# Forrest-Z/my-lidar-graph-slam

Measured on AMD Instinct MI355X. Metric: scans/sec + p50 scan-match ms, 1081-beam vs 1000×1000@5cm grid, 1/2/4/8 GPU, higher is better.
Workload: dtype f64

## Files before the change

### include/lgs_hip.h

```cpp
#ifndef LGS_HIP_H
#define LGS_HIP_H

#include <stddef.h>
#include <stdint.h>

#ifdef __cplusplus
extern "C" {
#endif

#define LGS_ABI_VERSION 2

#define LGS_OK               0
#define LGS_ERR_INVALID_ARG  1
#define LGS_ERR_HIP          2
#define LGS_ERR_NO_DEVICE    3
#define LGS_ERR_OOM          4
#define LGS_ERR_INTERNAL     5

typedef struct lgs_ctx  lgs_ctx;
typedef struct lgs_grid lgs_grid;
typedef struct lgs_scan lgs_scan;

typedef struct { double x, y, theta; } lgs_pose2d;

typedef struct {
    const double* ranges;
    const double* angles;
    int n;
    lgs_pose2d rel_sensor_pose;
    double min_range, max_range;
} lgs_scan_host;

typedef struct {
    int low_resolution;
    double range_x, range_y, range_theta;
    double scan_range_max;
} lgs_rtcsm_params;

typedef struct {
    double usable_range_min, usable_range_max;
    double hit_and_missed_dist, occupancy_threshold;
    int kernel_size;
    double scaling_factor;
    double standard_deviation;
} lgs_cost_ge_params;

typedef struct {
    int pose_found;
    double normalized_cost;
    lgs_pose2d initial_pose;
    lgs_pose2d estimated_pose;
    double covariance[9];
    double score_max;
    double score_threshold;
    int best_win[3];
    int win[3];
    double steps[3];
    lgs_pose2d best_sensor_pose;
    int64_t coarse_blocks;
    int64_t fine_blocks;
    int guard_hits;
    int fixups;
    int slow_path;
} lgs_rtcsm_summary;

int  lgs_ctx_create(int device, lgs_ctx** out);
void lgs_ctx_destroy(lgs_ctx* ctx);
const char* lgs_ctx_last_error(const lgs_ctx* ctx);
int  lgs_ctx_synchronize(lgs_ctx* ctx);
void* lgs_ctx_stream(lgs_ctx* ctx);
int  lgs_abi_version(void);

#define LGS_OPT_GUARD_EPS     1
#define LGS_OPT_FORCE_DENSE   2
#define LGS_OPT_INJECT_INDEX  3
#define LGS_OPT_GUARD_CAP     4
#define LGS_OPT_PROFILE       5
#define LGS_OPT_PROFILE_MASK  7
#define LGS_OPT_SPIN_SYNC     8
#define LGS_OPT_SKIP_MASK     10
#define LGS_OPT_SUPER_PRUNE   9
#define LGS_OPT_RAY_CHUNK_KEYS 13
#define LGS_OPT_LANES_MIN_BATCH 11
#define LGS_OPT_LINSOLVE_SPLIT 17
#define LGS_OPT_HANDOFF_SPIN_US 18
#define LGS_OPT_PEER_COPY     19
#define LGS_OPT_PRUNE_MIN_SUPER 21
#define LGS_OPT_COOP_TILES    22
#define LGS_OPT_SORT_BARRIER_US 23
#define LGS_OPT_FINE_STAGED   24
#define LGS_OPT_SMALL_WINDOW  25
#define LGS_OPT_POST_RECORDS  26
#define LGS_OPT_FUSED_PLANES  27
#define LGS_OPT_PRIORITY_TAIL 28
#define LGS_OPT_HV_FULL       29
#define LGS_OPT_SPLIT_CHUNKS  30
#define LGS_OPT_DEVICE_HITS   31
#define LGS_OPT_SEED_WIDE     32
#define LGS_OPT_ZERO_TILES    33
#define LGS_OPT_DEVICE_TIMING 34
#define LGS_OPT_LEAN_PROJECT  35
#define LGS_OPT_PGCG_GRID_NODES 36
#define LGS_OPT_FAST_ROWS     37
#define LGS_OPT_POISON_WS     15
int  lgs_ctx_set_option(lgs_ctx* ctx, int option, double value);

int  lgs_debug_item_buffer(lgs_ctx* ctx, int item, int which, void* out, size_t cap, size_t* bytes);

int  lgs_debug_libm(lgs_ctx* ctx, int op, const double* x, int n, double* out);

int  lgs_debug_keysort(lgs_ctx* ctx, const unsigned* keys, unsigned* out, long long n, int lo, int bits);

int  lgs_debug_copy_counters(const lgs_ctx* ctx, long long* direct, long long* staged);

int  lgs_debug_offset_checks(lgs_ctx* ctx, int reset, unsigned long long* out);

typedef struct {
    char name[32];
    int64_t launches;
    double total_ms;
    double algo_bytes;
    double dispatch_ms;
} lgs_kernel_stat;
int  lgs_ctx_kernel_stats(lgs_ctx* ctx, lgs_kernel_stat* out, int cap);
int  lgs_ctx_reset_stats(lgs_ctx* ctx);
int  lgs_ctx_match_counters(lgs_ctx* ctx, int64_t* out4);

int  lgs_grid_create(lgs_ctx* ctx, int w, int h, double min_x, double min_y,
                     double resolution, lgs_grid** out);
int  lgs_grid_wrap(lgs_ctx* ctx, double* device_cells, int w, int h, double min_x,
                   double min_y, double resolution, lgs_grid** out);
void lgs_grid_destroy(lgs_grid* grid);
int  lgs_grid_upload(lgs_ctx* ctx, lgs_grid* grid, const double* host_cells);
int  lgs_grid_upload_patches(lgs_ctx* ctx, lgs_grid* grid, const void* const* patches, int npx, int npy,
                             int patch_size, int cell_bytes, int value_offset);
int  lgs_grid_download(lgs_ctx* ctx, const lgs_grid* grid, double* host_cells);
int  lgs_grid_fill(lgs_ctx* ctx, lgs_grid* grid, double value);
int  lgs_grid_info(const lgs_grid* grid, int* w, int* h, double* min_x, double* min_y,
                   double* resolution);
double* lgs_grid_device_ptr(lgs_grid* grid);

int  lgs_grid_precompute_max(lgs_ctx* ctx, const lgs_grid* in, int win, lgs_grid* out);

int  lgs_scan_create(lgs_ctx* ctx, const lgs_scan_host* host, lgs_scan** out);
void lgs_scan_destroy(lgs_scan* scan);
int  lgs_scan_get(const lgs_scan* scan, int* n, double* ranges, double* angles);
int  lgs_scan_interpolate(lgs_ctx* ctx, const lgs_scan* in, double dist_scans, double dist_threshold_empty,
                          lgs_scan** out);

int  lgs_rtcsm_optimize_pose(lgs_ctx* ctx, const lgs_grid* grid, const lgs_grid* coarse,
                             const lgs_rtcsm_params* params,
                             const lgs_cost_ge_params* cost,
                             const lgs_scan* scan, lgs_pose2d initial_pose,
                             double normalized_score_threshold,
                             lgs_rtcsm_summary* out);
int  lgs_rtcsm_optimize_pose_query(lgs_ctx* ctx, const lgs_grid* grid,
                                   const lgs_rtcsm_params* params,
                                   const lgs_cost_ge_params* cost,
                                   const lgs_scan* scan, lgs_pose2d initial_pose,
                                   lgs_rtcsm_summary* out);
int  lgs_rtcsm_optimize_pose_query_batch(lgs_ctx* ctx, const lgs_grid* const* grids,
                                         const lgs_rtcsm_params* params,
                                         const lgs_cost_ge_params* cost,
                                         const lgs_scan* const* scans,
                                         const lgs_pose2d* initial_poses, int n,
                                         lgs_rtcsm_summary* out);
int  lgs_rtcsm_optimize_pose_batch(lgs_ctx* ctx, const lgs_grid* grid, const lgs_grid* coarse,
                                   const lgs_rtcsm_params* params,
                                   const lgs_cost_ge_params* cost,
                                   const lgs_scan* const* scans, const lgs_pose2d* initial_poses,
                                   int n, double normalized_score_threshold,
                                   lgs_rtcsm_summary* out);
int  lgs_rtcsm_dense_scores(lgs_ctx* ctx, const lgs_grid* grid, const lgs_grid* coarse,
                            const lgs_rtcsm_params* params, const lgs_scan* scan,
                            lgs_pose2d initial_pose, double* coarse_scores,
                            double* fine_scores, int* dims);

typedef struct lgs_map lgs_map;

typedef struct {
    double usable_range_min, usable_range_max;
    double prob_hit, prob_miss;
} lgs_builder_params;

typedef struct {
    double resolution;
    int patch_size;
    int num_patches_x, num_patches_y;
    int num_cells_x, num_cells_y;
    double min_x, min_y;
} lgs_map_geometry;

int  lgs_map_create(lgs_ctx* ctx, double resolution, int patch_size, int num_cells_x,
                    int num_cells_y, double center_x, double center_y, lgs_map** out);
void lgs_map_destroy(lgs_map* map);
int  lgs_map_get_geometry(const lgs_map* map, lgs_map_geometry* out);
int  lgs_map_grid(lgs_map* map, lgs_grid** out);
int  lgs_map_update_scan(lgs_ctx* ctx, lgs_map* map, const lgs_scan* scan, lgs_pose2d robot_pose,
                         const lgs_builder_params* params);
int  lgs_map_construct_from_scans(lgs_ctx* ctx, lgs_map* map, const lgs_scan* const* scans,
                                  const lgs_pose2d* robot_poses, int n,
                                  const lgs_builder_params* params);
int  lgs_map_append_scan(lgs_ctx* ctx, lgs_map* local, lgs_map* latest, const lgs_scan* const* scans,
                         const lgs_pose2d* robot_poses, int n, const lgs_builder_params* params);

int  lgs_debug_map_rebuilds(const lgs_map* m, long long* incremental, long long* full);

int  lgs_maps_construct_from_scans(lgs_ctx* ctx, lgs_map* const* maps, const int* idx_min,
                                   const int* idx_max, int n_maps, const lgs_scan* const* scans,
                                   const lgs_pose2d* robot_poses, int n_nodes,
                                   const lgs_builder_params* params);
int  lgs_map_construct_global(lgs_ctx* ctx, double resolution, int patch_size,
                              const lgs_scan* const* scans, const lgs_pose2d* robot_poses, int n,
                              const lgs_builder_params* params, lgs_map** out);
int  lgs_map_render_gray(lgs_ctx* ctx, const lgs_map* map, uint8_t* image);
int  lgs_map_render_gray_region(lgs_ctx* ctx, const lgs_map* map, int x0, int y0, int w, int h,
                                int flip_rows, uint8_t* image);
int  lgs_map_download_patches(lgs_ctx* ctx, const lgs_map* map, uint8_t* flags);
int  lgs_map_actual_size(lgs_ctx* ctx, const lgs_map* map, int* num_allocated, int* out);
int  lgs_map_download(lgs_ctx* ctx, const lgs_map* map, double* cells, uint32_t* hit_count,
                      uint32_t* miss_count);

int  lgs_cost_greedy_endpoint(lgs_ctx* ctx, const lgs_grid* grid,
// ... 265 lines not shown
```

### my-lidar-graph-slam_amd/csrc/k_bb.hip

```cpp
#include "lgs_internal.hpp"

#include <algorithm>
#include <cfloat>
#include <cstring>
#include <chrono>
#include <cstdio>
#include <cstdlib>
#include <thread>
#include <unordered_map>

using namespace lgs;

namespace lgs {
void launch_precompute(lgs_ctx* ctx, const lgs_grid* in, int win, double* out, const PlaneGeom* planes);
void cost_summaries(lgs_ctx* ctx, const lgs_grid* grid, const lgs_cost_ge_params* cost, lgs_scan* const* scans,
                    const lgs_pose2d* best, int n, lgs_rtcsm_summary* out);
}

namespace {

constexpr int kBBMaxH = 12;
constexpr int kBBBatch = 512;

struct BBItem {
// ... 751 lines not shown
        else
            cost_summaries_gx(ctx, gs.data(), cost, sc.data(), bp.data(), (int)order.size(), tmp.data());
        for (size_t k = 0; k < order.size(); ++k) out[order[k]] = tmp[k];
        order.clear();
    }
    std::stable_sort(order.begin(), order.end(), [&](int a, int b) { return grids[a] < grids[b]; });
    for (size_t k0 = 0; k0 < order.size();) {
        size_t k1 = k0;
        while (k1 < order.size() && grids[order[k1]] == grids[order[k0]]) ++k1;
        std::vector<lgs_scan*> sc;
        std::vector<lgs_pose2d> bp;
        std::vector<lgs_rtcsm_summary> tmp;
        for (size_t k = k0; k < k1; ++k) {
            sc.push_back(scans[order[k]]);
            bp.push_back(best[order[k]]);
            tmp.push_back(out[order[k]]);
        }
        cost_summaries(ctx, grids[order[k0]], cost, sc.data(), bp.data(), (int)sc.size(), tmp.data());
        for (size_t k = k0; k < k1; ++k) out[order[k]] = tmp[k - k0];
        k0 = k1;
    }
    lap(3);
    if (timing) {
        int64_t nodes = 0;
        for (int j = 0; j < n; ++j) nodes += out[j].coarse_blocks;
        std::fprintf(stderr, "bb n=%d nodes=%lld: trig+path %.2f ms, levels %.2f ms, replay %.2f ms, cost %.2f ms\n",
                     n, (long long)nodes, t_ms[0], t_ms[1], t_ms[2], t_ms[3]);
    }
    if (!redo.empty()) {
        std::vector<const lgs_grid*> g2;
        std::vector<const double* const*> p2;
        std::vector<lgs_scan*> s2;
        std::vector<lgs_pose2d> i2;
        for (int j : redo) {
            g2.push_back(grids[j]);
            p2.push_back(pyr[j]);
            s2.push_back(scans[j]);
            i2.push_back(init[j]);
        }
        std::vector<lgs_rtcsm_summary> o2(redo.size());
        run_bb(ctx, p, cost, g2.data(), p2.data(), s2.data(), i2.data(), (int)redo.size(), nthr, o2.data(), true, alt);
        for (size_t k = 0; k < redo.size(); ++k) out[redo[k]] = o2[k];
    }
}

void check_bb(const lgs_bb_params* p, const lgs_cost_ge_params* c)
{
    LGS_REQUIRE(p && c, "null argument");
    LGS_REQUIRE(p->node_height_max >= 0 && p->node_height_max <= kBBMaxH, "node_height_max must be in [0, 12]");
    LGS_REQUIRE(p->range_x >= 0 && p->range_y >= 0 && p->range_theta >= 0, "negative search range");
    LGS_REQUIRE(c->kernel_size >= 0, "negative kernel size");
}

std::vector<std::vector<const double*>> pyramids(lgs_ctx* ctx, const lgs_grid* const* maps, int n_maps, int Hm)
{
    for (int k = 0; k < n_maps; ++k) grid_acquire(ctx, maps[k]);
    size_t total = 0;
    for (int m = 0; m < n_maps; ++m) total += (size_t)(Hm + 1) * align256(sizeof(double) * (size_t)maps[m]->w * maps[m]->h);
    char* base = (char*)ctx->ensure(S_BB2, std::max<size_t>(total, 16));
    std::vector<std::vector<const double*>> out((size_t)n_maps);
    size_t off = 0;
    for (int m = 0; m < n_maps; ++m) {
        for (int h = 0; h <= Hm; ++h) {
            double* d = (double*)(base + off);
            off += align256(sizeof(double) * (size_t)maps[m]->w * maps[m]->h);
            launch_precompute(ctx, maps[m], 1 << h, d, nullptr);
            out[m].push_back(d);
        }
    }
    return out;
}

}

extern "C" int lgs_grid_precompute_pyramid(lgs_ctx* ctx, const lgs_grid* in, int node_height_max,
                                           lgs_grid* const* pyramid)
{
    if (!ctx || !in || !pyramid || node_height_max < 0 || node_height_max > kBBMaxH) return LGS_ERR_INVALID_ARG;
    return guarded(ctx, [&] {
        LGS_HIP_CHECK(hipSetDevice(ctx->device));
        for (int h = 0; h <= node_height_max; ++h) {
            LGS_REQUIRE(pyramid[h] && pyramid[h]->w == in->w && pyramid[h]->h == in->h,
                        "pyramid grids must have the input's size");
            launch_precompute(ctx, in, 1 << h, pyramid[h]->d, nullptr);
        }
        ctx->sync();
    });
}

static int bb_batch_run(lgs_ctx* ctx, const lgs_grid* grid, const lgs_grid* const* pyramid,
                        const lgs_bb_params* params, const lgs_cost_ge_params* cost, CostAlt alt,
                        const lgs_scan* const* scans, const lgs_pose2d* initial, int n, double nthr,
                        lgs_rtcsm_summary* out)
{
    if (!ctx || !grid || !pyramid || !scans || !initial || !out || n < 0) return LGS_ERR_INVALID_ARG;
    if (n == 0) return LGS_OK;
    return guarded(ctx, [&] {
        check_bb(params, cost);
        LGS_REQUIRE(!alt || (long long)grid->w * grid->h < (1LL << 30), "square-error or exact cost: map of 2^30 cells or more");
        std::vector<const double*> pyr;
        for (int h = 0; h <= params->node_height_max; ++h) {
            LGS_REQUIRE(pyramid[h] && pyramid[h]->w == grid->w && pyramid[h]->h == grid->h,
                        "pyramid grids must have the map's size");
            pyr.push_back(pyramid[h]->d);
        }
        std::vector<const double* const*> pp((size_t)n, pyr.data());
        std::vector<const lgs_grid*> grids((size_t)n, grid);
        std::vector<lgs_scan*> sc((size_t)n);
        for (int j = 0; j < n; ++j) {
            LGS_REQUIRE(scans[j] && scans[j]->n >= 1, "empty scan");
            sc[j] = const_cast<lgs_scan*>(scans[j]);
        }
        for (int j0 = 0; j0 < n; j0 += kBBBatch) {
            const int m = std::min(kBBBatch, n - j0);
            run_bb(ctx, params, cost, grids.data() + j0, pp.data() + j0, sc.data() + j0, initial + j0, m, nthr,
                   out + j0, false, alt);
        }
    });
}

extern "C" int lgs_bb_optimize_pose_batch(lgs_ctx* ctx, const lgs_grid* grid, const lgs_grid* const* pyramid,
                                          const lgs_bb_params* params, const lgs_cost_ge_params* cost,
                                          const lgs_scan* const* scans, const lgs_pose2d* initial, int n,
                                          double nthr, lgs_rtcsm_summary* out)
{
    return bb_batch_run(ctx, grid, pyramid, params, cost, CostAlt{}, scans, initial, n, nthr, out);
}

extern "C" int lgs_bb_optimize_pose_batch_cost(lgs_ctx* ctx, const lgs_grid* grid, const lgs_grid* const* pyramid,
                                               const lgs_bb_params* params, const lgs_cost_spec* cost,
                                               const lgs_scan* const* scans, const lgs_pose2d* initial, int n,
                                               double nthr, lgs_rtcsm_summary* out)
{
    CostSel sel;
    if (const int rc = cost_select(cost, &sel)) return rc;
    if (!sel.alt) return lgs_bb_optimize_pose_batch(ctx, grid, pyramid, params, sel.ge, scans, initial, n, nthr, out);
    if (!out || n < 0) return LGS_ERR_INVALID_ARG;
    std::vector<lgs_rtcsm_summary> tmp;
    const int rc0 = guarded(ctx, [&] { tmp.resize((size_t)n); });
    if (rc0 != LGS_OK) return rc0;
    const int rc = bb_batch_run(ctx, grid, pyramid, params, sel.ge, sel.alt, scans, initial, n, nthr, tmp.data());
    if (rc == LGS_OK && n > 0) std::memcpy(out, tmp.data(), sizeof(lgs_rtcsm_summary) * (size_t)n);
    return rc;
}

static int bb_query_run(lgs_ctx* ctx, const lgs_grid* grid, const lgs_bb_params* params,
                        const lgs_cost_ge_params* cost, CostAlt alt, const lgs_scan* scan,
                        lgs_pose2d initial, lgs_rtcsm_summary* out)
{
    if (!ctx || !grid || !scan || !out) return LGS_ERR_INVALID_ARG;
    return guarded(ctx, [&] {
        check_bb(params, cost);
        LGS_REQUIRE(scan->n >= 1, "empty scan");
        LGS_REQUIRE(!alt || (long long)grid->w * grid->h < (1LL << 30), "square-error or exact cost: map of 2^30 cells or more");
        auto pyr = pyramids(ctx, &grid, 1, params->node_height_max);
        const double* const* pp = pyr[0].data();
        lgs_scan* s = const_cast<lgs_scan*>(scan);
        run_bb(ctx, params, cost, &grid, &pp, &s, &initial, 1, DBL_MIN, out, false, alt);
    });
}

extern "C" int lgs_bb_optimize_pose_query(lgs_ctx* ctx, const lgs_grid* grid, const lgs_bb_params* params,
                                          const lgs_cost_ge_params* cost, const lgs_scan* scan,
                                          lgs_pose2d initial, lgs_rtcsm_summary* out)
{
    return bb_query_run(ctx, grid, params, cost, CostAlt{}, scan, initial, out);
// ... 116 lines not shown
```

### my-lidar-graph-slam_amd/csrc/k_rtcsm.hip

```cpp
#include "lgs_internal.hpp"
#include "fast_cell.hpp"
#include "sq_cost_stage.hpp"
#include "ge_cost_device.hpp"

#include <algorithm>
#include <cfloat>
#include <cstring>
#include <map>
#include <mutex>
#include <thread>
#include <type_traits>

using namespace lgs;

namespace lgs {
void launch_precompute(lgs_ctx* ctx, const lgs_grid* in, int win, double* out, const PlaneGeom* planes);
void launch_precompute_jobs(lgs_ctx* ctx, const PrecompJob* d_jobs, int njobs, int maxW, int maxH, int win);
bool precompute_planes_ok(const lgs_grid* in, int win);
void precompute_tile_grid(int maxW, int maxH, int win, int njobs, int* gx, int* gy, int* rows);
}

namespace {


typedef _Float16 SuperT;

constexpr int kMaxBatchItems = 64;
constexpr int kPipe = 16;
constexpr int kPad = 4 * kPipe;

struct MatchItem {
    RtcsmPlan pl;
    CostPlan cp;
    const double* grid;
    const double* ranges;
    const double* angles;
    const double* cmap;
    const SuperT* super;
    const int* negflag;
    int pgen;
    int gen;
    RtcsmRecord* rec;
    int* keepc;
    int2* idx;
    int* cbase;
    int* tedge;
    double* cscore;
    uint8_t* cflag;
    int* list;
    int* segcnt;
    int nseg;
    int* dlist;
    int* nsel;
    int frows;
    double* fval;
    int* fpos;
    double* part_c;
    long long* part_k;
    int nparts;
    double* Lp;
    double* Lc;
    double* seedm;
    int nseedm;
    double* sbound;
    double* poses7;
    int4* cidx;
    double* terms;
    const double* ge_tab;
    double4* btab;
    double2* atab;
    int lean;
    int inject;
    int gcap;
    double geps;
    double fox, foy, fh0;
    float finv_lr;
    int fast;
};
typedef const MatchItem* __restrict__ Items;

struct Blk {
    int x, y, z;
};
__device__ __forceinline__ Blk xcd_block()
{
    const int gx = gridDim.x, gy = gridDim.y, gz = gridDim.z;
    const int nwg = gx * gy * gz;
    const int b = blockIdx.x + gx * (blockIdx.y + gy * blockIdx.z);
    const int xcd = b & 7, q = nwg >> 3, r = nwg & 7;
    const int l = (xcd < r ? xcd * (q + 1) : r * (q + 1) + (xcd - r) * q) + (b >> 3);
    return { __builtin_amdgcn_readfirstlane(l % gx), __builtin_amdgcn_readfirstlane((l / gx) % gy),
             __builtin_amdgcn_readfirstlane(l / (gx * gy)) };
}

struct PlaneJob {
    RtcsmPlan pl;
    const unsigned short* planes16;
    SuperT* super;
    unsigned* zt;
    int* negflag;
// ... 3555 lines not shown
}

void bind_workspace(MatchItem& it, char* base, const ItemLayout& L, int frows)
{
    it.idx = (int2*)(base + L.idx);
    it.cbase = (int*)(base + L.cbase);
    it.cscore = (double*)(base + L.cscore);
    it.cflag = (uint8_t*)(base + L.cflag);
    it.list = (int*)(base + L.list);
    it.segcnt = (int*)(base + L.segcnt);
    it.fval = (double*)(base + L.fval);
    it.fpos = (int*)(base + L.fpos);
    it.part_c = (double*)(base + L.part_c);
    it.part_k = (long long*)(base + L.part_k);
    it.sbound = (double*)(base + L.sbound);
    it.poses7 = (double*)(base + L.poses7);
    it.cidx = (int4*)(base + L.cidx);
    it.terms = (double*)(base + L.terms);
    it.Lp = (double*)(base + L.count);
    it.Lc = (double*)(base + L.count + 64);
    it.nsel = (int*)(base + L.count + 64 + 8 * kSeedCands);
    it.seedm = (double*)(base + L.count + 128);
    it.dlist = (int*)(base + L.dlist);
    it.btab = (double4*)(base + L.btab);
    it.atab = (double2*)(base + L.atab);
    static_assert(64 + 8 * kSeedCands + 4 <= 128, "count block layout");
    it.frows = frows;
    it.nseg = (int)((it.pl.K + kSelSeg - 1) / kSelSeg);
}

inline size_t plane_bytes(const RtcsmPlan& pl)
{
    return align256(sizeof(double) * (size_t)pl.low_res * pl.low_res * (size_t)pl.pstride);
}
inline size_t plane16_bytes(const RtcsmPlan& pl)
{
    return align256(sizeof(unsigned short) * (size_t)pl.low_res * pl.low_res * (size_t)pl.pstride) + 256;
}
inline size_t set_bytes(const RtcsmPlan& pl) { return plane_bytes(pl) + plane16_bytes(pl); }
inline size_t super_bytes(const RtcsmPlan& pl)
{
    if (pl.oct) return align256(4 * (size_t)pl.unit8 * pl.low_res * pl.low_res * (size_t)pl.pstrideO);
    return align256(sizeof(SuperT) * (size_t)pl.low_res * pl.low_res * (size_t)pl.pstride4);
}
double* planes_buffer(lgs_ctx* ctx, const RtcsmPlan& pl, int nsets, bool with_super)
{
    const int b = ctx->bank;
    const size_t bytes = set_bytes(pl) * (size_t)nsets;
    double* D = (double*)ctx->ensure(ctx->banked(S_DECIM), bytes);
    const size_t sbytes = super_bytes(pl) * (size_t)nsets;
    SuperT* S = with_super ? (SuperT*)ctx->ensure(ctx->banked(S_SUPER), sbytes) : nullptr;
    const long long key[4] = { pl.low_res, pl.Wq, pl.Hq, pl.M * 16 + pl.oct * 4 + pl.unit8 };
    if (D != ctx->planes_ptr[b] || std::memcmp(key, ctx->planes_key[b], sizeof(key)) != 0 ||
        nsets > ctx->planes_sets[b] || (with_super && (S != ctx->super_ptr[b] || nsets > ctx->super_sets[b]))) {
        LGS_HIP_CHECK(hipMemsetAsync(D, 0, bytes, ctx->stream));
        ctx->planes_ptr[b] = D;
        ctx->planes_sets[b] = nsets;
        std::memcpy(ctx->planes_key[b], key, sizeof(key));
        ctx->super_ptr[b] = nullptr;
        ctx->super_sets[b] = 0;
        if (with_super) {
            LGS_HIP_CHECK(hipMemsetAsync(S, 0, sbytes, ctx->stream));
            ctx->super_ptr[b] = S;
            ctx->super_sets[b] = nsets;
        }
    }
    return D;
}

struct PlaneSet {
    const lgs_grid* fine = nullptr;
    const lgs_grid* coarse = nullptr;
    const double* cmap = nullptr;
    const SuperT* super = nullptr;
    const int* negflag = nullptr;
    int pgen = 0;
    bool half_copy = false;
    unsigned short* planes16 = nullptr;
};

struct SetJobs {
    size_t jobs_off = 0, njobs = 0, pj_off = 0, npj = 0, dj_off = 0, ndj = 0;
    bool hv = false;
};

inline bool hv_mode(const lgs_ctx* ctx, const RtcsmPlan& lp) { return ctx->fused_planes && lp.oct; }
SuperGeom super_geom(const RtcsmPlan& lp)
{
    SuperGeom g{};
    g.M = lp.M;
    g.Wqp = lp.Wqp;
    g.Wq4 = lp.Wq4;
    g.unit8 = lp.unit8;
    g.Hqp = lp.Hqp;
    g.pstride = lp.pstride;
    g.subO = lp.subO;
    g.pstrideO = lp.pstrideO;
    g.X4lo = (lp.M - kSB) >> 2;
    g.ncol = ((lp.M + lp.Wq - 1) >> 2) - g.X4lo + 1;
    g.qlo = (lp.M - kSB) >> 4;
    g.nqt = ((lp.M + lp.Hq - 1) >> 4) - g.qlo + 1;
    g.lr = lp.low_res;
    return g;
}

void zero_tiles(lgs_ctx* ctx, const RtcsmPlan& lp, const std::vector<PlaneSet>& sets, std::vector<PrecompJob>& jobs,
                const std::vector<int>& job_set, std::vector<PlaneJob>& pj, double* D, SuperT* S, bool need_super)
{
    const int b = ctx->bank, ns = (int)sets.size(), lr = lp.low_res;
    std::vector<unsigned char>& pre_ok = ctx->zt_pre[b];
    std::vector<unsigned char>& hv_ok = ctx->zt_hv[b];
    if ((int)pre_ok.size() < ns) pre_ok.resize(ns, 0);
    if ((int)hv_ok.size() < ns) hv_ok.resize(ns, 0);
    const bool want = ctx->zero_tiles && need_super && lr <= 8 && hv_mode(ctx, lp);
    const bool use_pre = want && !jobs.empty();
    const bool use_hv = want;
    std::vector<unsigned char> pre_now(ns, 0), hv_now(ns, 0);
    int maxW = 0, maxH = 0;
    for (auto& ps : sets)
        if (ps.fine) {
            maxW = std::max(maxW, ps.fine->w);
            maxH = std::max(maxH, ps.fine->h);
        }
    int pgx = 0, pgy = 0, prows = 0;
    if (use_pre) precompute_tile_grid(maxW, maxH, lr, (int)jobs.size(), &pgx, &pgy, &prows);
    const SuperGeom g = super_geom(lp);
    const int nq = ctx->hv_full && lp.unit8 == 2 ? 2 : 1;
    const int hgx = hv_grid_x(g, nq);
    const long long pre_words = use_pre ? (long long)pgx * pgy : 0;
    const long long hv_words = use_hv ? (long long)lr * lr * hgx : 0;
    const long long per_set = pre_words + hv_words;
    if (per_set > 0) {
        unsigned* Z = (unsigned*)ctx->ensure(ctx->banked(S_ZTILE), sizeof(unsigned) * (size_t)(per_set * ns));
        const long long key[12] = { (long long)(uintptr_t)D, (long long)(uintptr_t)S, (long long)(uintptr_t)Z,
                                    lr, lp.Wq, lp.Hq, lp.M * 16 + lp.oct * 4 + lp.unit8, lp.pstride,
                                    pgx, (long long)pgy << 8 | prows, hgx, nq };
        if (std::memcmp(key, ctx->zt_key[b], sizeof(key)) != 0) {
            std::memcpy(ctx->zt_key[b], key, sizeof(key));
            std::fill(pre_ok.begin(), pre_ok.end(), 0);
            std::fill(hv_ok.begin(), hv_ok.end(), 0);
        }
        bool clear = false;
        for (size_t k = 0; k < jobs.size() && use_pre; ++k) {
            const int s = job_set[k];
            const bool ok = pre_ok[s] && ctx->zt_dims[b].size() > (size_t)s &&
                            ctx->zt_dims[b][s] == ((long long)jobs[k].W << 32 | jobs[k].H);
            clear |= !ok;
            jobs[k].zt = Z + per_set * s;
            pre_now[s] = 1;
        }
        for (int s = 0; s < ns && use_hv; ++s) {
            clear |= !hv_ok[s];
            pj[s].zt = Z + per_set * s + pre_words;
            hv_now[s] = 1;
        }
        if (clear) LGS_HIP_CHECK(hipMemsetAsync(Z, 0, sizeof(unsigned) * (size_t)(per_set * ns), ctx->stream));
        if (clear) {
            std::fill(pre_ok.begin(), pre_ok.end(), 0);
            std::fill(hv_ok.begin(), hv_ok.end(), 0);
        }
    }
    if ((int)ctx->zt_dims[b].size() < ns) ctx->zt_dims[b].resize(ns, -1);
    for (int s = 0; s < ns; ++s) {
        pre_ok[s] = pre_now[s];
        if (need_super) hv_ok[s] = hv_now[s];
    }
    for (size_t k = 0; k < jobs.size(); ++k)
        ctx->zt_dims[b][job_set[k]] = ((long long)jobs[k].W << 32 | jobs[k].H);
}

void launch_decimate(const double* coarse, const RtcsmPlan& pl, double* D, hipStream_t st);
SetJobs build_sets(lgs_ctx* ctx, const RtcsmPlan& lp, std::vector<PlaneSet>& sets, bool need_super, Upload& up)
{
    const int ns = (int)sets.size();
    hipStream_t st = ctx->stream;
    const int lr = lp.low_res;
    double* D = planes_buffer(ctx, lp, ns, need_super);
    SuperT* S = need_super ? (SuperT*)ctx->ensure(ctx->banked(S_SUPER), super_bytes(lp) * (size_t)ns) : nullptr;
    int* neg = need_super ? (int*)ctx->ensure(ctx->banked(S_NEGFLAG), sizeof(int) * (size_t)ns) : nullptr;
    const size_t pb = plane_bytes(lp) / sizeof(double), sbb = super_bytes(lp) / sizeof(SuperT);
    const size_t ssz = set_bytes(lp) / sizeof(double);
    std::vector<PrecompJob> jobs;
    std::vector<int> job_set;
    std::vector<PlaneJob> pj;
    std::vector<DecimJob> djobs;
    for (int s = 0; s < ns; ++s) {
        PlaneSet& ps = sets[s];
        ps.cmap = D + ssz * (size_t)s;
        PlaneJob j{};
        j.pl = lp;
        ps.half_copy = need_super;
        if (need_super) {
            ps.planes16 = (unsigned short*)(D + ssz * (size_t)s + pb);
            j.planes16 = ps.planes16;
            j.super = S + sbb * (size_t)s;
            ps.super = j.super;
            ps.negflag = neg + s;
            ps.pgen = ctx->next_stamp();
            j.negflag = neg + s;
            j.pgen = ps.pgen;
        }
        if (ps.fine && precompute_planes_ok(ps.fine, lr)) {
            PrecompJob q{};
            q.in = ps.fine->d;
            q.out = D + ssz * (size_t)s;
            q.W = ps.fine->w;
            q.H = ps.fine->h;
            q.pg = PlaneGeom{ lp.M, lp.Wqp, lp.pstride };
            if (need_super && lr <= 8) {
                q.out16 = ps.planes16;
                q.negflag = neg + s;
                q.pgen = ps.pgen;
                ps.half_copy = false;
            }
            jobs.push_back(q);
            job_set.push_back(s);
        } else if (ps.fine) {
            const size_t cells = (size_t)lp.W * lp.H;
            double* plain = (double*)ctx->ensure(S_COARSE_GRID, sizeof(double) * std::max<size_t>(1, cells));
            launch_precompute(ctx, ps.fine, lr, plain, nullptr);
            launch_decimate(plain, lp, D + ssz * (size_t)s, st);
        } else {
            DecimJob dj{ ps.coarse->d, D + ssz * (size_t)s, need_super ? ps.planes16 : nullptr,
                         need_super ? neg + s : nullptr, ps.pgen };
            djobs.push_back(dj);
            ps.half_copy = false;
        }
        if (need_super) pj.push_back(j);
    }
    zero_tiles(ctx, lp, sets, jobs, job_set, pj, D, S, need_super);
    SetJobs sj;
    sj.njobs = jobs.size();
    sj.jobs_off = jobs.empty() ? 0 : up.append(jobs.data(), jobs.size());
    sj.npj = pj.size();
    sj.pj_off = pj.empty() ? 0 : up.append(pj.data(), pj.size());
    sj.ndj = djobs.size();
    sj.dj_off = djobs.empty() ? 0 : up.append(djobs.data(), djobs.size());
    sj.hv = hv_mode(ctx, lp);
    return sj;
}

void launch_sets(lgs_ctx* ctx, const RtcsmPlan& lp, const std::vector<PlaneSet>& sets, const SetJobs& sj,
                 const Upload& up)
{
    int maxW = 0, maxH = 0;
    for (auto& s : sets)
        if (s.fine) {
            maxW = std::max(maxW, s.fine->w);
            maxH = std::max(maxH, s.fine->h);
        }
    if (sj.njobs)
        launch_precompute_jobs(ctx, up.at<PrecompJob>(sj.jobs_off), (int)sj.njobs, maxW, maxH, lp.low_res);
    if (sj.ndj) {
        const int np = lp.low_res * lp.low_res;
        hipLaunchKernelGGL(k_decimate_jobs, dim3((lp.Wq + 255) / 256, lp.Hq, np * (int)sj.ndj), dim3(256), 0,
                           ctx->stream, up.at<DecimJob>(sj.dj_off), lp.W, lp.H, lp.low_res, lp.Wq, lp.M, lp.Wqp,
                           lp.pstride);
        LGS_HIP_CHECK(hipGetLastError());
    }
    for (const auto& s : sets)
        if (s.half_copy) {
            const long long n = (long long)lp.low_res * lp.low_res * lp.pstride;
            hipLaunchKernelGGL(k_planes16, dim3((unsigned)((n + 255) / 256)), dim3(256), 0, ctx->stream, s.cmap,
                               s.planes16, n, const_cast<int*>(s.negflag), s.pgen);
            LGS_HIP_CHECK(hipGetLastError());
        }
    if (sj.npj && sj.hv) {
        const int np = lp.low_res * lp.low_res;
        const SuperGeom g = super_geom(lp);
        const int nq = ctx->hv_full && lp.unit8 == 2 ? 2 : 1;
        dim3 grid(hv_grid_x(g, nq), 1, np * (int)sj.npj);
        const double cq = (double)np * g.ncol * g.nqt * sj.npj;
        const int tok = ctx->timing_begin(K_SUPER_PLANES, cq * (16.0 * 4.0 * 2.0 + 16.0 * 8.0 * g.unit8));
        if (!ctx->skipped(K_SUPER_PLANES))
        {
            if (nq == 2)
                hipLaunchKernelGGL(HIP_KERNEL_NAME(k_super_hv<2>), grid, dim3(256), 0, ctx->stream,
                                   up.at<PlaneJob>(sj.pj_off), np, g, ctx->dts(tok));
            else
                hipLaunchKernelGGL(HIP_KERNEL_NAME(k_super_hv<1>), grid, dim3(256), 0, ctx->stream,
                                   up.at<PlaneJob>(sj.pj_off), np, g, ctx->dts(tok));
        }
        ctx->timing_end(tok);
        LGS_HIP_CHECK(hipGetLastError());
    } else if (sj.npj) {
        const int np = lp.low_res * lp.low_res;
        const bool lone = sj.npj == 1;
        const int spx = lone ? kSPXLone : kSPX;
        dim3 g((lp.Wqp + spx - 1) / spx, (lp.Hqp + kSPY - 1) / kSPY, np * (int)sj.npj);
        const int tok = ctx->timing_begin(K_SUPER_PLANES, 8.0 * 2.0 * (double)np * lp.pstride * sj.npj);
        if (!ctx->skipped(K_SUPER_PLANES)) {
            if (lone)
                hipLaunchKernelGGL(HIP_KERNEL_NAME(k_super_planes<kSPXLone>), g,
                                   dim3((kSPXLone + 3 + 63) / 64 * 64), 0, ctx->stream, up.at<PlaneJob>(sj.pj_off), np);
            else
                hipLaunchKernelGGL(HIP_KERNEL_NAME(k_super_planes<kSPX>), g, dim3(kSPThreads), 0, ctx->stream,
                                   up.at<PlaneJob>(sj.pj_off), np);
        }
        ctx->timing_end(tok);
        LGS_HIP_CHECK(hipGetLastError());
    }
}

void launch_decimate(const double* coarse, const RtcsmPlan& pl, double* D, hipStream_t st)
{
    dim3 gd((pl.Wq + 255) / 256, pl.Hq, pl.low_res * pl.low_res);
    hipLaunchKernelGGL(k_decimate, gd, dim3(256), 0, st, coarse, pl.W, pl.H, pl.low_res, pl.Wq, pl.M, pl.Wqp,
                       pl.pstride, D);
    LGS_HIP_CHECK(hipGetLastError());
}

inline int fine_grid(int n) { return std::max(64, std::min(1024, 8192 / std::max(n, 1))); }
inline size_t pref_bytes(int nseg) { return sizeof(int) * (size_t)(nseg + 1); }

struct ScanOptions {
    bool dense = false;
    const std::vector<int4>* patches = nullptr;
    const std::vector<int2>* host_idx = nullptr;
    const std::vector<int4>* cost_patches = nullptr;
    bool cost_only = false;
};

void enqueue_cost(lgs_ctx* ctx, const BatchShape& B, Items d_items, const std::vector<MatchItem>& items, int n,
                  int inject)
{
    hipStream_t st = ctx->stream;
    double nbeams = 0.0;
    for (auto& it : items) nbeams += it.cp.N;
    if (B.sq) {
        const int tok_ = ctx->timing_begin(K_COST_SQ, 8.0 * 5.0 * 16.0 * nbeams);
        if (!ctx->skipped(K_COST_SQ)) {
            const size_t lds = cost_sq_lds(items);
            sq_allow_lds(k_cost_sq, lds);
            hipLaunchKernelGGL(k_cost_sq, dim3(n), dim3(kSqThreads), lds, st, d_items, (unsigned)lds, ctx->dts(tok_));
        }
// ... 421 lines not shown
        int cells[4];
        host_cost_cells(cp, scan, P7[pb.first], pb.second, cells);
        cpatch.push_back(make_int4(pb.first * cp.N + pb.second, 0, 0, 0));
        cpatch.push_back(make_int4(cells[0], cells[1], cells[2], cells[3]));
    }
    return true;
}

void finish_summary(const RtcsmPlan& pl, const lgs_scan* scan, lgs_pose2d initial, bool pruned,
                    const RtcsmRecord& rec, lgs_rtcsm_summary* out, bool sq = false)
{
    std::memset(out, 0, sizeof(*out));
    out->pose_found = rec.found;
    out->initial_pose = initial;
    out->score_max = rec.score_max;
    out->score_threshold = pl.thr;
    for (int i = 0; i < 3; ++i) out->best_win[i] = rec.best[i];
    out->win[0] = pl.win_x;
    out->win[1] = pl.win_y;
    out->win[2] = pl.win_t;
    out->steps[0] = pl.step_x;
    out->steps[1] = pl.step_y;
    out->steps[2] = pl.step_t;
    const lgs_pose2d best{ pl.sx + rec.best[0] * pl.step_x, pl.sy + rec.best[1] * pl.step_y,
                           pl.st + rec.best[2] * pl.step_t };
    out->best_sensor_pose = best;
    out->normalized_cost = rec.costs[0] / (double)scan->n;
    out->estimated_pose = move_backward(best, scan->rel);
    const double dl = pl.res, da = 1e-2;
    const double g[3] = { 0.5 * (rec.costs[1] - rec.costs[2]) / dl,
                          0.5 * (rec.costs[3] - rec.costs[4]) / dl,
                          0.5 * (rec.costs[5] - rec.costs[6]) / da };
    for (int i = 0; i < 3; ++i)
        for (int j = 0; j < 3; ++j) out->covariance[3 * i + j] = g[i] * g[j];
    out->covariance[0] += 0.01;
    out->covariance[4] += 0.01;
    out->covariance[8] += 0.01;
    if (sq) {
        sq_covariance(rec.costs + 1, out->covariance);
    }
    out->coarse_blocks = pruned ? (int64_t)rec.coarse_evals : pl.K;
    out->fine_blocks = rec.n_eval;
}

void check_args(const lgs_grid* grid, const lgs_rtcsm_params* p, const lgs_cost_ge_params* c, const lgs_scan* s)
{
    LGS_REQUIRE(grid && p && c && s, "null argument");
    LGS_REQUIRE(p->low_resolution >= 1 && p->low_resolution <= 32, "low_resolution must be in [1, 32]");
    LGS_REQUIRE(p->range_x >= 0 && p->range_y >= 0 && p->range_theta >= 0, "negative search range");
    LGS_REQUIRE(s->n >= 1, "empty scan");
    LGS_REQUIRE(s->n <= 16384, "at most 16384 beams per scan (LDS-staged index rows)");
    LGS_REQUIRE(c->kernel_size >= 0, "negative kernel size");
}

void check_coarse(const lgs_grid* grid, const lgs_grid* coarse)
{
    LGS_REQUIRE(coarse, "null coarse map");
    LGS_REQUIRE(grid->w == coarse->w && grid->h == coarse->h && grid->min_x == coarse->min_x &&
                    grid->min_y == coarse->min_y && grid->res == coarse->res,
                "coarse map must have the fine map's geometry (CreateSameSizeMap)");
}

const char* const kSqDomainError = "square-error cost: an angle lies outside the restated sincos domain";
const char* const kGxDomainError = "exact greedy-endpoint cost: an angle lies outside the restated sincos domain";

struct InFlight {
    std::vector<MatchItem> items;
    BatchShape B;
    std::vector<int> gens;
    std::vector<PlaneSet> sets;
    const lgs_grid* const* grids = nullptr;
    lgs_scan* const* scans = nullptr;
    const lgs_pose2d* init = nullptr;
    lgs_rtcsm_summary* out = nullptr;
    RtcsmRecord* h_rec = nullptr;
    RtcsmRecord* d_rec = nullptr;
    int n = 0, bank = 0;
    long long id = 0;
    bool post = false;
    unsigned* flag = nullptr;
    unsigned post_gen = 0;
    bool sq_err = false;
    bool gx_err = false;
};

bool lean_rows(const lgs_ctx* ctx, const BatchShape& B, const std::vector<MatchItem>& items)
{
    const int n = B.n;
    if (!ctx->lean_project || B.small || !B.pruned || !B.oct || n < ctx->lanes_min_batch || !B.wl.cnt) return false;
    if (ctx->skip_mask) return false;
    if (!(B.fine_lanes && B.fine_staged && ctx->fine_staged)) return false;
    if (!(std::min(ctx->seed_wide, kSeedWide) > kSeedCands)) return false;
    for (const auto& it : items)
        if (it.nparts > kSeedWideMaxParts) return false;
    return true;
}

void launch_matches(lgs_ctx* ctx, const lgs_rtcsm_params* params, const lgs_cost_ge_params* cost,
                    const lgs_grid* const* grids, lgs_scan* const* scans, const lgs_pose2d* init, int n,
                    double nthr, std::vector<PlaneSet>& sets, const int* set_of, lgs_rtcsm_summary* out,
                    InFlight& F, CostAlt alt = {})
{
    const lgs_cost_sq_params* sq = alt.sq;
    LGS_HIP_CHECK(hipSetDevice(ctx->device));
    LGS_REQUIRE(n >= 1 && n <= kMaxBatchItems, "batch of 1..64 matches (run_chunked splits larger ones)");
    std::vector<MatchItem> items((size_t)n);
    BatchShape B;
    B.n = n;
    int Nmax = 1;
    for (int j = 0; j < n; ++j) {
        check_args(grids[j], params, cost, scans[j]);
        grid_acquire(ctx, grids[j]);
        LGS_REQUIRE(grids[j]->w == grids[0]->w && grids[j]->h == grids[0]->h && grids[j]->res == grids[0]->res,
                    "the maps of one batch must share their size and resolution");
        int nv = 0;
        scan_valid_indices(ctx, scans[j], params->scan_range_max, &nv);
        MatchItem& it = items[j];
        std::memset(&it, 0, sizeof(it));
        it.pl = make_plan(grids[j], params, scans[j], init[j], nthr, nv);
        LGS_REQUIRE(it.pl.K <= 7LL * 1024 * 1024, "search window too large (> 7M coarse blocks)");
        it.cp = make_cost_plan(grids[j], cost, scans[j]);
        if (sq) {
            it.cp.min_range = std::max(sq->usable_range_min, scans[j]->min_range);
            it.cp.max_range = std::min(sq->usable_range_max, scans[j]->max_range);
        }
        if (alt.gx) it.ge_tab = ctx->ge_table(cost, grids[j]->res);
        B.Tmax = std::max(B.Tmax, it.pl.T);
        B.NvMax = std::max(B.NvMax, nv);
        Nmax = std::max(Nmax, scans[j]->n);
    }
    for (auto& s : sets)
        if (s.coarse) check_coarse(grids[0], s.coarse);
    const RtcsmPlan& p0 = items[0].pl;
    B.P = p0.P;
    B.nsb2 = p0.nsbx * p0.nsby;
    B.low_res = p0.low_res;
    B.cb = coarse_block(p0);
    B.pair = B.nsb2 <= 32;
    B.chunks = B.pair ? 1 : (B.nsb2 + 63) / 64;
    B.oct = p0.oct != 0;
    B.unit8 = p0.unit8;
    B.nsby = p0.nsby;
    B.pruned = uses_super(ctx, B.NvMax, B.nsb2, false);
    B.lr5 = lr5_path(B.NvMax, B.low_res);
    B.fine_lanes = n >= ctx->lanes_min_batch && B.low_res * B.low_res <= 64 &&
                   B.NvMax <= kFineLanesMaxNv;
    B.frows = (B.lr5 && !B.fine_lanes) ? 5 : 1;
    B.fine_staged = B.fine_lanes && B.low_res == 5;
    for (int j = 0; j < n && B.fine_staged; ++j)
        B.fine_staged = grids[j]->w % 2 == 0 && ((uintptr_t)grids[j]->d & 15) == 0 && grids[j]->w <= 8192 &&
                        grids[j]->h <= 8192;
    B.kernel_size = cost->kernel_size;
    B.sq = sq != nullptr;
    B.gx = alt.gx;
    B.nsegMax = (int)(((long long)B.Tmax * B.P + kSelSeg - 1) / kSelSeg);
    B.small = ctx->small_window && !ctx->force_dense && p0.P == 1 && B.low_res >= 2 && B.low_res <= 7 &&
              B.NvMax <= kSmallMaxNv && n <= kTedgeCtrs;
    for (int j = 0; j < n; ++j) B.small = B.small && grids[j]->w >= B.low_res && grids[j]->h >= 1;
    for (auto& s : sets) B.small = B.small && !s.coarse;
    if (B.small) B.pruned = false;
    if (B.pruned && n >= ctx->lanes_min_batch && B.NvMax <= kListMaxNv && B.Tmax < (1 << 24) && B.nsb2 <= 64) {
        int region = 1;
        for (auto& it : items) region = std::max(region, it.pl.T * it.pl.nsbx * it.pl.nsby);
        int* wl = (int*)ctx->ensure(S_KEEP, sizeof(int) * (size_t)n * (16 + (size_t)region + (size_t)B.Tmax));
        B.wl = WorkList{ wl, wl + 16 * (size_t)n, wl + 16 * (size_t)n + (size_t)region * n, region, B.Tmax };
    }
// ... 45 lines not shown
        it.negflag = s.negflag;
        it.pgen = s.pgen;
        it.gen = gens[j] = ctx->generation = ctx->next_stamp();
        it.rec = d_rec + j;
        it.keepc = B.wl.cnt ? B.wl.cnt + 16 * j : sctr ? sctr + j : nullptr;
        it.nparts = item_nparts(B, it.pl, B.pruned);
        it.nseedm = std::min(ctx->seed_wide, kSeedWide);
        it.inject = ctx->inject_index ? 1 : 0;
        it.geps = ctx->guard_eps;
        it.gcap = ctx->guard_cap;
        set_fast_rows(it, ctx->fast_rows);
    }
    const bool lean = lean_rows(ctx, B, items);
    for (auto& it : items) it.lean = lean ? 1 : 0;
    ctx->dbg.assign((size_t)n, lgs_ctx::DbgItem{});
    for (int j = 0; j < n; ++j) {
        const MatchItem& ij = items[j];
        const RtcsmPlan& q = ij.pl;
        const size_t nidx = (size_t)q.T * std::max(q.Nv, 1) + kPad;
        const void* b[8] = { ij.sbound, ij.part_c, ij.part_k, ij.Lp, ij.tedge, ij.cbase, ij.idx, ij.cscore };
        const size_t sz[8] = { sizeof(double) * (size_t)q.T * B.nsb2, sizeof(double) * (size_t)ij.nparts,
                               sizeof(long long) * (size_t)ij.nparts, 64 + sizeof(double) * kSeedCands,
                               sizeof(int) * (size_t)q.T, sizeof(int) * 2 * nidx,
                               sizeof(int2) * (size_t)q.T * q.Nv, sizeof(double) * (size_t)q.K };
        lgs_ctx::DbgItem& d = ctx->dbg[j];
        for (int k = 0; k < 8; ++k) {
            d.buf[k] = b[k];
            d.bytes[k] = sz[k];
        }
        d.buf[8] = ij.cmap;
        d.bytes[8] = ij.cmap ? plane_bytes(q) : 0;
        d.buf[9] = ij.super;
        d.bytes[9] = ij.super ? super_bytes(q) : 0;
        d.gen = ij.gen;
    }
    const size_t items_off = up.append(items.data(), items.size());
    up.flush();
    if (!B.small) launch_sets(ctx, p0, sets, sj, up);
    struct StreamRestore {
        lgs_ctx* c;
        hipStream_t s;
        ~StreamRestore() { c->stream = s; }
    } restore{ ctx, ctx->stream };
    if (!B.small && ctx->prio_tail && ctx->hi) {
        LGS_HIP_CHECK(hipEventRecord(ctx->split_ev[ctx->bank], ctx->stream));
        LGS_HIP_CHECK(hipStreamWaitEvent(ctx->hi, ctx->split_ev[ctx->bank], 0));
        ctx->stream = ctx->hi;
    }
    enqueue_items(ctx, B, up.at<MatchItem>(items_off), items, ScanOptions{});
    F.post = ctx->post_records;
    if (F.post) {
        static_assert(sizeof(RtcsmRecord) % 16 == 0, "k_post copies 16-byte words");
        F.flag = h_flag;
        F.post_gen = (unsigned)ctx->next_stamp();
        *(volatile unsigned*)h_flag = 0u;
        const int n16 = (int)(rec_bytes / 16);
        const int n2 = ctx->dts_dev ? (int)(kDtsBytes / 16) : 0;
        hipLaunchKernelGGL(k_post, dim3(1), dim3(std::min(kPostThreads, (std::max(n16, n2) + 63) / 64 * 64)), 0,
                           ctx->stream, (const uint4*)d_rec, (uint4*)h_rec, (int)(rec_bytes / 16), h_flag, F.post_gen,
                           (const uint4*)ctx->dts_dev, (uint4*)ctx->dts_host, n2);
        LGS_HIP_CHECK(hipGetLastError());
    } else {
        LGS_HIP_CHECK(hipMemcpyAsync(h_rec, d_rec, rec_bytes, hipMemcpyDeviceToHost, ctx->stream));
        if (ctx->dts_dev)
            LGS_HIP_CHECK(hipMemcpyAsync(const_cast<unsigned long long*>(ctx->dts_host), ctx->dts_dev, kDtsBytes,
                                         hipMemcpyDeviceToHost, ctx->stream));
    }
    hipEvent_t& ev = ctx->bank_ev[ctx->bank];
    if (!ev) LGS_HIP_CHECK(hipEventCreateWithFlags(&ev, hipEventDisableTiming));
    LGS_HIP_CHECK(hipEventRecord(ev, ctx->stream));
    if (ctx->stream != restore.s) LGS_HIP_CHECK(hipStreamWaitEvent(restore.s, ev, 0));
    F.items = std::move(items);
    F.B = B;
    F.gens = std::move(gens);
    F.sets = sets;
    F.grids = grids;
    F.scans = scans;
    F.init = init;
    F.out = out;
    F.h_rec = h_rec;
    F.d_rec = d_rec;
    F.n = n;
    F.bank = ctx->bank;
}

void finish_matches(lgs_ctx* ctx, InFlight& F)
{
    ctx->bank = F.bank;
    if (F.post) {
        volatile unsigned* f = F.flag;
        for (unsigned spins = 1; *f != F.post_gen; ++spins) {
            if (spins % 4096) continue;
            const hipError_t e = hipEventQuery(ctx->bank_ev[F.bank]);
            if (e == hipSuccess && *f != F.post_gen) throw Error(LGS_ERR_INTERNAL, "k_post: completion flag lost");
            if (e != hipSuccess && e != hipErrorNotReady) LGS_HIP_CHECK(e);
        }
        std::atomic_thread_fence(std::memory_order_acquire);
    } else {
        ctx->wait_event(ctx->bank_ev[F.bank]);
    }
    ctx->up_busy[F.bank] = false;
    std::vector<MatchItem>& items = F.items;
    const BatchShape& B = F.B;
    const std::vector<int>& gens = F.gens;
    lgs_scan* const* scans = F.scans;
    const lgs_pose2d* init = F.init;
    lgs_rtcsm_summary* out = F.out;
    RtcsmRecord* h_rec = F.h_rec;
    RtcsmRecord* d_rec = F.d_rec;
    const int n = F.n;
    if (ctx->profile) {
        double coarse_bytes = 0.0;
        for (int j = 0; j < n; ++j) coarse_bytes += 8.0 * items[j].pl.Nv * (double)h_rec[j].coarse_evals;
        for (auto& pt : ctx->pending)
            if (pt.coarse_evals && pt.batch == F.id) {
                pt.algo_bytes = coarse_bytes;
                pt.coarse_evals = false;
            }
        ctx->harvest_upto(F.id);
    }
    const long long saved_batch = ctx->timing_batch;
    ctx->timing_batch = F.id;

    for (int j = 0; j < n; ++j) {
        HostRecord rec(h_rec[j], gens[j]);
        const int guard_hits = rec.guard_count + rec.cost_guard_count;
        int fixups = 0, slow = 0;
        bool pruned = B.pruned;
        ScanOptions opt;
        std::vector<int4> patches, cpatch;
        std::vector<int2> hidx;
        for (int iter = 0; iter < 4; ++iter) {
            bool use_hidx = false, full_cost = false;
            bool rerun = false;
            if (!opt.host_idx && !opt.patches &&
                check_projection_guards(ctx, items[j].pl, scans[j], rec, patches, hidx, use_hidx)) {
                if (use_hidx) opt.host_idx = &hidx;
                else opt.patches = &patches;
                rerun = true;
                fixups = 1;
            }
            if (rec.status & REC_DANGEROUS && !opt.dense) {
                opt.dense = true;
                rerun = true;
                slow = 1;
            }
            if (!rerun && !opt.cost_patches && !B.sq && !B.gx) {
                const CostPlan& cp = items[j].cp;
                if (check_cost_guards(ctx, items[j].pl, cp, scans[j], rec, cpatch, full_cost)) {
                    if (full_cost) {
                        double P7[7][3];
                        host_poses7(items[j].pl, rec.best, P7);
                        cpatch.clear();
                        for (int pi = 0; pi < 7; ++pi)
                            for (int b = 0; b < cp.N; ++b) {
                                const double r = scans[j]->h_ranges[b];
                                if (r >= cp.max_range || r <= cp.min_range) continue;
                                int cells[4];
                                host_cost_cells(cp, scans[j], P7[pi], b, cells);
                                cpatch.push_back(make_int4(pi * cp.N + b, 0, 0, 0));
                                cpatch.push_back(make_int4(cells[0], cells[1], cells[2], cells[3]));
                            }
                    }
                    opt.cost_patches = &cpatch;
                    opt.cost_only = true;
                    rerun = true;
                    fixups = 1;
                }
            }
            if (!rerun) break;
            BatchShape B1 = B;
            B1.n = 1;
            B1.Tmax = items[j].pl.T;
            B1.nsegMax = items[j].nseg;
            B1.pruned = pruned = !B.small && uses_super(ctx, B.NvMax, B.nsb2, opt.dense);
            std::vector<MatchItem> one(1, items[j]);
            one[0].nparts = item_nparts(B1, one[0].pl, B1.pruned);
            one[0].lean = 0;
            const int g = one[0].gen = ctx->generation = ctx->next_stamp();
            if ((size_t)j < ctx->dbg.size()) ctx->dbg[j].gen = g;
            Upload u1(ctx);
            const size_t off = u1.append(one.data(), 1);
            u1.flush();
            enqueue_items(ctx, B1, u1.at<MatchItem>(off), one, opt);
            LGS_HIP_CHECK(hipMemcpyAsync(&h_rec[j], d_rec + j, sizeof(RtcsmRecord), hipMemcpyDeviceToHost,
                                         ctx->stream));
            ctx->sync();
            if (ctx->profile) ctx->harvest_upto(F.id);
            rec = HostRecord(h_rec[j], g);
            if (opt.patches || opt.host_idx) rec.guard_count = 0;
        }
        finish_summary(items[j].pl, scans[j], init[j], pruned, rec, &out[j], B.sq);
        if (B.sq && rec.sq_err) F.sq_err = true;
        if (B.gx)
            for (int k = 0; k < 7; ++k) F.gx_err = F.gx_err || rec.gx_err[k] != 0;
        out[j].guard_hits = guard_hits;
        out[j].fixups = fixups;
        out[j].slow_path = slow;
        ctx->count_matches += 1;
        ctx->count_coarse_blocks += out[j].coarse_blocks;
        ctx->count_coarse_blocks_dense += items[j].pl.K;
        ctx->count_pruned += pruned ? 1 : 0;
    }
    ctx->timing_batch = saved_batch;
    ctx->bank = 0;
}

void run_matches(lgs_ctx* ctx, const lgs_rtcsm_params* params, const lgs_cost_ge_params* cost,
                 const lgs_grid* const* grids, lgs_scan* const* scans, const lgs_pose2d* init, int n,
                 double nthr, std::vector<PlaneSet>& sets, const int* set_of, lgs_rtcsm_summary* out,
                 CostAlt alt = {})
{
    InFlight F;
    ctx->bank = 0;
    launch_matches(ctx, params, cost, grids, scans, init, n, nthr, sets, set_of, out, F, alt);
    finish_matches(ctx, F);
    if (F.sq_err) throw Error(LGS_ERR_INTERNAL, kSqDomainError);
    if (F.gx_err) throw Error(LGS_ERR_INTERNAL, kGxDomainError);
}


constexpr int kMaxBatch = kMaxBatchItems;
constexpr int kSplitMin = 16;
void run_chunked(lgs_ctx* ctx, const lgs_rtcsm_params* params, const lgs_cost_ge_params* cost,
                 const lgs_grid* const* grids, lgs_scan* const* scans, const lgs_pose2d* init, int n,
                 double nthr, const std::vector<PlaneSet>& sets_all, const int* set_of, lgs_rtcsm_summary* out,
                 CostAlt alt = {})
{
    InFlight fl[2];
    bool busy[2] = { false, false };
    bool sq_err = false, gx_err = false;
    int c = 0;
    const int step = (ctx->split_chunks && n <= kMaxBatch && n >= 2 * kSplitMin) ? (n + 1) / 2 : kMaxBatch;
    try {
        for (int j0 = 0; j0 < n; j0 += step, ++c) {
            const int m = std::min(step, n - j0);
            std::vector<PlaneSet> sets;
            std::vector<int> so((size_t)m), remap(sets_all.size(), -1);
            for (int k = 0; k < m; ++k) {
                const int s = set_of[j0 + k];
                if (remap[s] < 0) {
                    remap[s] = (int)sets.size();
                    sets.push_back(sets_all[s]);
                }
                so[k] = remap[s];
            }
            const int b = c & 1;
            ctx->bank = b;
            fl[b] = InFlight{};
            launch_matches(ctx, params, cost, grids + j0, scans + j0, init + j0, m, nthr, sets, so.data(), out + j0,
                           fl[b], alt);
            busy[b] = true;
            if (busy[b ^ 1]) {
                finish_matches(ctx, fl[b ^ 1]);
                busy[b ^ 1] = false;
                sq_err = sq_err || fl[b ^ 1].sq_err;
                gx_err = gx_err || fl[b ^ 1].gx_err;
            }
        }
        const int last = (c - 1) & 1;
        if (busy[last]) {
            finish_matches(ctx, fl[last]);
            busy[last] = false;
            sq_err = sq_err || fl[last].sq_err;
            gx_err = gx_err || fl[last].gx_err;
        }
    } catch (...) {
        ctx->bank = 0;
        throw;
    }
    ctx->bank = 0;
    if (sq_err) throw Error(LGS_ERR_INTERNAL, kSqDomainError);
    if (gx_err) throw Error(LGS_ERR_INTERNAL, kGxDomainError);
}

}

namespace lgs {
void cost_summaries(lgs_ctx* ctx, const lgs_grid* grid, const lgs_cost_ge_params* cost, lgs_scan* const* scans,
                    const lgs_pose2d* best, int n, lgs_rtcsm_summary* out)
{
    if (n <= 0) return;
    grid_acquire(ctx, grid);
    int Nmax = 1;
    for (int j = 0; j < n; ++j) Nmax = std::max(Nmax, scans[j]->n);
    const ItemLayout L = item_layout(1, 1, 1, 1, 1, 64, 1, Nmax);
    char* ws = (char*)ctx->ensure(S_BATCH_WS, L.total * (size_t)n);
    RtcsmRecord* d_rec = (RtcsmRecord*)ctx->ensure(S_RECORDS, sizeof(RtcsmRecord) * (size_t)n);
    RtcsmRecord* h_rec = (RtcsmRecord*)ctx->ensure_pinned(sizeof(RtcsmRecord) * (size_t)n);
    std::vector<MatchItem> items((size_t)n);
    std::vector<double> P7((size_t)n * 21);
    std::vector<int> gens((size_t)n);
    scans_to_device(ctx, scans, n);
    for (int j = 0; j < n; ++j) {
        MatchItem& it = items[j];
        std::memset(&it, 0, sizeof(it));
        bind_workspace(it, ws + L.total * (size_t)j, L, 1);
        it.cp = make_cost_plan(grid, cost, scans[j]);
        it.grid = grid->d;
        it.ranges = scans[j]->d_ranges;
        it.angles = scans[j]->d_angles;
        it.rec = d_rec + j;
        it.gen = gens[j] = ctx->generation = ctx->next_stamp();
        const double x = best[j].x, y = best[j].y, th = best[j].theta, dl = grid->res, da = 1e-2;
        const double v[21] = { x, y, th, x + dl, y + 0.0, th + 0.0, x - dl, y - 0.0, th - 0.0,
                               x + 0.0, y + dl, th + 0.0, x - 0.0, y - dl, th - 0.0,
                               x + 0.0, y + 0.0, th + da, x - 0.0, y - 0.0, th - da };
        std::memcpy(&P7[(size_t)j * 21], v, sizeof(v));
    }
    Upload up(ctx);
    const size_t poff = up.append(P7.data(), P7.size());
    const size_t ioff = up.append(items.data(), items.size());
    char* dev = up.prepare();
    for (int j = 0; j < n; ++j) up.host_at<MatchItem>(ioff)[j].poses7 = (double*)(dev + poff) + 21 * (size_t)j;
    up.copy();
    Items d_items = up.at<MatchItem>(ioff);
    const int ks = cost->kernel_size;
    hipLaunchKernelGGL(KCOST(ks), dim3(7, n), dim3(kCostThreads), cost_lds(items), ctx->stream, d_items,
                       ctx->guard_cap,
                       ctx->guard_eps, ctx->inject_index ? 1 : 0, 0, DevTs{});
    LGS_HIP_CHECK(hipGetLastError());
    LGS_HIP_CHECK(hipMemcpyAsync(h_rec, d_rec, sizeof(RtcsmRecord) * (size_t)n, hipMemcpyDeviceToHost, ctx->stream));
    ctx->sync();
    for (int j = 0; j < n; ++j) {
        HostRecord rec(h_rec[j], gens[j]);
        double p7[7][3];
        std::memcpy(p7, &P7[(size_t)j * 21], sizeof(p7));
        std::vector<int4> cpatch;
        bool full = false;
        out[j].guard_hits += rec.cost_guard_count;
        if (check_cost_guards_p7(ctx, p7, items[j].cp, scans[j], rec, cpatch, full)) {
            const CostPlan& cp = items[j].cp;
            if (full) {
                cpatch.clear();
                for (int pi = 0; pi < 7; ++pi)
                    for (int b = 0; b < cp.N; ++b) {
                        const double r = scans[j]->h_ranges[b];
                        if (r >= cp.max_range || r <= cp.min_range) continue;
                        int cells[4];
                        host_cost_cells(cp, scans[j], p7[pi], b, cells);
                        cpatch.push_back(make_int4(pi * cp.N + b, 0, 0, 0));
                        cpatch.push_back(make_int4(cells[0], cells[1], cells[2], cells[3]));
                    }
            }
            const int np = (int)(cpatch.size() / 2);
            int4* dp = (int4*)ctx->ensure(S_PATCH, sizeof(int4) * std::max<size_t>(cpatch.size(), 1));
            LGS_HIP_CHECK(hipMemcpyAsync(dp, cpatch.data(), sizeof(int4) * cpatch.size(), hipMemcpyHostToDevice,
                                         ctx->stream));
            if (np) hipLaunchKernelGGL(k_cost_patch, dim3((np + 255) / 256), dim3(256), 0, ctx->stream,
                                       items[j].cidx, dp, np);
            hipLaunchKernelGGL(KCOST(ks), dim3(7, 1), dim3(kCostThreads), cost_lds(items), ctx->stream, d_items + j,
                               ctx->guard_cap, ctx->guard_eps, 0, 1, DevTs{});
            LGS_HIP_CHECK(hipGetLastError());
            LGS_HIP_CHECK(hipMemcpyAsync(&h_rec[j], d_rec + j, sizeof(RtcsmRecord), hipMemcpyDeviceToHost,
// ... 406 lines not shown
                    ++qi;
                const lgs_loop_query& Q = queries[qi];
                lgs_loop_result& r = results[ci];
                std::memset(&r, 0, sizeof(r));
                const lgs_rtcsm_summary& s = sums[k];
                r.found = s.pose_found;
                r.start_node_index = Q.local_map_node_index;
                r.end_node_index = candidates[ci].node_index;
                r.start_node_pose = Q.local_map_node_pose;
                r.estimated_pose = s.estimated_pose;
                r.score = s.score_max;
                r.normalized_cost = s.normalized_cost;
                if (s.pose_found) r.relative_pose = inverse_compound(Q.local_map_node_pose, s.estimated_pose);
                std::memcpy(r.covariance, s.covariance, sizeof(r.covariance));
            }
        }
    });
}

extern "C" int lgs_loop_detect_rtcsm(lgs_ctx* ctx, const lgs_rtcsm_params* params,
                                     const lgs_cost_ge_params* cost, double score_threshold,
                                     const lgs_loop_query* queries, int num_queries,
                                     const lgs_loop_candidate* candidates, int num_candidates,
                                     lgs_loop_result* results)
{
    return loop_detect_rtcsm_run(ctx, params, cost, CostAlt{}, score_threshold, queries, num_queries, candidates,
                                 num_candidates, results);
}

extern "C" int lgs_loop_detect_rtcsm_cost(lgs_ctx* ctx, const lgs_rtcsm_params* params, const lgs_cost_spec* cost,
                                          double score_threshold, const lgs_loop_query* queries, int num_queries,
                                          const lgs_loop_candidate* candidates, int num_candidates,
                                          lgs_loop_result* results)
{
    CostSel sel;
    if (const int rc = cost_select(cost, &sel)) return rc;
    if (!sel.alt)
        return lgs_loop_detect_rtcsm(ctx, params, sel.ge, score_threshold, queries, num_queries, candidates,
                                     num_candidates, results);
    if (num_candidates < 0 || (num_candidates > 0 && !results)) return LGS_ERR_INVALID_ARG;
    std::vector<lgs_loop_result> tmp;
    const int rc0 = guarded(ctx, [&] { tmp.resize((size_t)num_candidates); });
    if (rc0 != LGS_OK) return rc0;
    const int rc = loop_detect_rtcsm_run(ctx, params, sel.ge, sel.alt, score_threshold, queries, num_queries,
                                         candidates, num_candidates, tmp.data());
    if (rc == LGS_OK && num_candidates > 0) std::memcpy(results, tmp.data(), sizeof(lgs_loop_result) * tmp.size());
    return rc;
}

namespace {

bool peer_access(int dev, int peer)
{
    if (dev == peer) return true;
    static std::mutex mu;
    static std::map<std::pair<int, int>, bool> known;
    std::lock_guard<std::mutex> lock(mu);
    const auto key = std::make_pair(dev, peer);
    auto it = known.find(key);
    if (it != known.end()) return it->second;
    int can = 0;
    bool ok = hipDeviceCanAccessPeer(&can, dev, peer) == hipSuccess && can;
    if (ok) {
        int cur = 0;
        hipGetDevice(&cur);
        hipSetDevice(dev);
        const hipError_t e = hipDeviceEnablePeerAccess(peer, 0);
        ok = e == hipSuccess || e == hipErrorPeerAccessAlreadyEnabled;
        (void)hipGetLastError();
        hipSetDevice(cur);
    }
    known[key] = ok;
    return ok;
}

lgs_grid* clone_grid(lgs_ctx* ctx, const lgs_grid* src)
{
    lgs_grid* g = nullptr;
    const int rc = lgs_grid_create(ctx, src->w, src->h, src->min_x, src->min_y, src->res, &g);
    if (rc != LGS_OK) throw Error(rc, ctx->last_error);
    const size_t bytes = sizeof(double) * (size_t)src->w * (size_t)src->h;
    try {
        if (bytes) {
            if (src->writer) src->writer->wait();
            if (!ctx->peer_staged && peer_access(ctx->device, src->device)) {
                LGS_HIP_CHECK(hipMemcpyPeerAsync(g->d, ctx->device, src->d, src->device, bytes, ctx->stream));
                ctx->sync();
                ++ctx->copies_direct;
            } else {
                void* pin = nullptr;
                LGS_HIP_CHECK(hipHostMalloc(&pin, bytes));
                hipError_t e = hipMemcpy(pin, src->d, bytes, hipMemcpyDeviceToHost);
                if (e == hipSuccess) e = hipMemcpyAsync(g->d, pin, bytes, hipMemcpyHostToDevice, ctx->stream);
                if (e == hipSuccess) e = hipStreamSynchronize(ctx->stream);
                hipHostFree(pin);
                LGS_HIP_CHECK(e);
                ++ctx->copies_staged;
            }
        }
    } catch (...) {
        lgs_grid_destroy(g);
        throw;
    }
    return g;
}

lgs_scan* clone_scan(lgs_ctx* ctx, const lgs_scan* src)
{
    lgs_scan_host h{};
    h.n = src->n;
    h.ranges = src->h_ranges.data();
    h.angles = src->h_angles.data();
    h.rel_sensor_pose = src->rel;
    h.min_range = src->min_range;
    h.max_range = src->max_range;
    lgs_scan* s = nullptr;
    const int rc = lgs_scan_create(ctx, &h, &s);
    if (rc != LGS_OK) throw Error(rc, ctx->last_error);
    return s;
}

struct LoopShard {
    lgs_ctx* ctx = nullptr;
    int lo = 0, hi = 0;
    std::vector<lgs_loop_query> qs;
    std::vector<lgs_loop_candidate> cs;
    std::vector<lgs_grid*> grids;
    std::vector<lgs_scan*> scans;
    int status = LGS_OK;
    std::string error;

    ~LoopShard()
    {
        for (lgs_grid* g : grids) lgs_grid_destroy(g);
        for (lgs_scan* s : scans) lgs_scan_destroy(s);
    }
    const lgs_grid* own(const lgs_grid* g, std::vector<std::pair<const lgs_grid*, lgs_grid*>>& memo)
    {
        if (!g || g->ctx == ctx) return g;
        for (auto& m : memo)
            if (m.first == g) return m.second;
        grids.push_back(clone_grid(ctx, g));
        memo.push_back({ g, grids.back() });
        return grids.back();
    }
    void prepare(const lgs_loop_query* queries, int num_queries, const lgs_loop_candidate* candidates)
    {
        std::vector<std::pair<const lgs_grid*, lgs_grid*>> memo;
        for (int q = 0; q < num_queries; ++q) {
            const lgs_loop_query& Q = queries[q];
            const int a = std::max(Q.first_candidate, lo), b = std::min(Q.first_candidate + Q.num_candidates, hi);
            if (a >= b) continue;
            lgs_loop_query c = Q;
            c.map = own(Q.map, memo);
            c.coarse = own(Q.coarse, memo);
            c.first_candidate = (int)cs.size();
            c.num_candidates = b - a;
            qs.push_back(c);
            for (int i = a; i < b; ++i) {
                lgs_loop_candidate k = candidates[i];
                if (k.scan->ctx != ctx) {
                    scans.push_back(clone_scan(ctx, k.scan));
                    k.scan = scans.back();
                }
                cs.push_back(k);
            }
// ... 130 lines not shown
```

### my-lidar-graph-slam_amd/csrc/lgs_core.hip

```cpp
#include "lgs_internal.hpp"

#include <atomic>
#include <condition_variable>
#include <cstring>
#include <mutex>
#include <thread>

#include <pthread.h>

using namespace lgs;

void* lgs_ctx::ensure(int slot, size_t bytes)
{
    if (bytes == 0) bytes = 16;
    if (buf_bytes[slot] >= bytes) return buf[slot];
    if (buf[slot]) {
        LGS_HIP_CHECK(hipStreamSynchronize(stream));
        LGS_HIP_CHECK(hipFree(buf[slot]));
        buf[slot] = nullptr;
        buf_bytes[slot] = 0;
    }
    size_t want = bytes + bytes / 4;
    void* p = nullptr;
    hipError_t e = hipMalloc(&p, want);
// ... 419 lines not shown
    int n = 0;
    for (int k = 0; k < K_NUM_KERNELS; ++k) {
        if (ctx->stat_launches[k] == 0) continue;
        if (out && n < cap) {
            std::memset(&out[n], 0, sizeof(out[n]));
            std::strncpy(out[n].name, kKernelNames[k], sizeof(out[n].name) - 1);
            out[n].launches = ctx->stat_launches[k];
            out[n].total_ms = ctx->stat_ms[k];
            out[n].algo_bytes = ctx->stat_bytes[k];
            out[n].dispatch_ms = ctx->stat_disp_ms[k];
        }
        ++n;
    }
    return n;
}

extern "C" size_t lgs_cost_spec_size(void) { return sizeof(lgs_cost_spec); }

extern "C" int lgs_ctx_reset_stats(lgs_ctx* ctx)
{
    if (!ctx) return LGS_ERR_INVALID_ARG;
    return guarded(ctx, [&] {
        ctx->sync();
        ctx->harvest();
        for (int k = 0; k < K_NUM_KERNELS; ++k) {
            ctx->stat_launches[k] = 0;
            ctx->stat_ms[k] = 0;
            ctx->stat_bytes[k] = 0;
            ctx->stat_disp_ms[k] = 0;
        }
        ctx->count_matches = ctx->count_coarse_blocks = ctx->count_coarse_blocks_dense = ctx->count_pruned = 0;
    });
}

extern "C" int lgs_ctx_match_counters(lgs_ctx* ctx, int64_t* out4)
{
    if (!ctx || !out4) return LGS_ERR_INVALID_ARG;
    out4[0] = ctx->count_matches;
    out4[1] = ctx->count_coarse_blocks;
    out4[2] = ctx->count_coarse_blocks_dense;
    out4[3] = ctx->count_pruned;
    return LGS_OK;
}

extern "C" void* lgs_ctx_stream(lgs_ctx* ctx) { return ctx ? (void*)ctx->stream : nullptr; }

extern "C" int lgs_ctx_set_option(lgs_ctx* ctx, int option, double value)
{
    if (!ctx) return LGS_ERR_INVALID_ARG;
    switch (option) {
    case LGS_OPT_GUARD_EPS: ctx->guard_eps = value; return LGS_OK;
    case LGS_OPT_FORCE_DENSE: ctx->force_dense = value != 0.0; return LGS_OK;
    case LGS_OPT_INJECT_INDEX: ctx->inject_index = value != 0.0; return LGS_OK;
    case LGS_OPT_PROFILE:
        ctx->profile = value != 0.0;
        ctx->profile_mask = ~0u;
        return LGS_OK;
    case LGS_OPT_SPIN_SYNC: ctx->spin_sync = value != 0.0; return LGS_OK;
    case LGS_OPT_PROFILE_MASK:
        ctx->profile_mask = (unsigned)value;
        ctx->profile = ctx->profile_mask != 0;
        return LGS_OK;
    case LGS_OPT_SUPER_PRUNE: ctx->super_prune = value != 0.0; return LGS_OK;
    case LGS_OPT_LANES_MIN_BATCH: ctx->lanes_min_batch = (int)value; return LGS_OK;
    case LGS_OPT_RAY_CHUNK_KEYS:
        if (!(value >= 1.0)) return LGS_ERR_INVALID_ARG;
        ctx->ray_chunk_keys = (long long)std::min(value, (double)(1LL << 30));
        return LGS_OK;
    case LGS_OPT_SKIP_MASK: ctx->skip_mask = (unsigned)value; return LGS_OK;
    case LGS_OPT_POISON_WS: ctx->poison_ws = value != 0.0; return LGS_OK;
    case LGS_OPT_PEER_COPY: ctx->peer_staged = value != 0.0; return LGS_OK;
    case LGS_OPT_PRUNE_MIN_SUPER: ctx->prune_min_super = (int)value; return LGS_OK;
    case LGS_OPT_COOP_TILES: ctx->coop_tiles = (long long)value; return LGS_OK;
    case LGS_OPT_FINE_STAGED: ctx->fine_staged = value != 0.0; return LGS_OK;
    case LGS_OPT_SMALL_WINDOW: ctx->small_window = value != 0.0; return LGS_OK;
    case LGS_OPT_POST_RECORDS: ctx->post_records = value != 0.0; return LGS_OK;
    case LGS_OPT_FUSED_PLANES: ctx->fused_planes = value != 0.0; return LGS_OK;
    case LGS_OPT_PRIORITY_TAIL: ctx->prio_tail = value != 0.0; return LGS_OK;
    case LGS_OPT_DEVICE_TIMING: ctx->dev_timing = value != 0.0; return LGS_OK;
    case LGS_OPT_HV_FULL: ctx->hv_full = value != 0.0; return LGS_OK;
    case LGS_OPT_SPLIT_CHUNKS: ctx->split_chunks = value != 0.0; return LGS_OK;
    case LGS_OPT_DEVICE_HITS: ctx->device_hits = value != 0.0; return LGS_OK;
    case LGS_OPT_ZERO_TILES: ctx->zero_tiles = value != 0.0; return LGS_OK;
    case LGS_OPT_LEAN_PROJECT: ctx->lean_project = value != 0.0; return LGS_OK;
    case LGS_OPT_FAST_ROWS: ctx->fast_rows = value != 0.0; return LGS_OK;
    case LGS_OPT_PGCG_GRID_NODES:
        if (!(value >= 0.0)) return LGS_ERR_INVALID_ARG;
        ctx->pg_grid_nodes = (int)std::min(value, 2147483647.0);
        return LGS_OK;
    case LGS_OPT_SEED_WIDE:
        if (!(value >= 0.0 && value <= 16.0)) return LGS_ERR_INVALID_ARG;
        ctx->seed_wide = (int)value;
        return LGS_OK;
    case LGS_OPT_SORT_BARRIER_US:
        if (value < 0) return LGS_ERR_INVALID_ARG;
        ctx->sort_barrier_us = (long long)value;
        return LGS_OK;
    case LGS_OPT_LINSOLVE_SPLIT: ctx->linsolve_split = value != 0.0; return LGS_OK;
    case LGS_OPT_HANDOFF_SPIN_US:
        if (value < 0.0) return LGS_ERR_INVALID_ARG;
        ctx->handoff_spin_us = (long long)value;
        return LGS_OK;
    case LGS_OPT_GUARD_CAP:
        ctx->guard_cap = (int)value;
        if (ctx->guard_cap < 0) ctx->guard_cap = 0;
        if (ctx->guard_cap > kGuardInline) ctx->guard_cap = kGuardInline;
        return LGS_OK;
    default: ctx->last_error = "unknown option"; return LGS_ERR_INVALID_ARG;
    }
}

__global__ void k_fill(double* __restrict__ d, size_t n, double v)
{
    size_t i = (size_t)blockIdx.x * blockDim.x + threadIdx.x;
    size_t stride = (size_t)gridDim.x * blockDim.x;
    for (; i < n; i += stride) d[i] = v;
}

extern "C" int lgs_grid_create(lgs_ctx* ctx, int w, int h, double min_x, double min_y,
                               double res, lgs_grid** out)
{
    if (!ctx || !out) return LGS_ERR_INVALID_ARG;
    *out = nullptr;
    return guarded(ctx, [&] {
        LGS_REQUIRE(w >= 0 && h >= 0 && res > 0.0, "invalid grid geometry");
        LGS_HIP_CHECK(hipSetDevice(ctx->device));
        lgs_grid* g = new lgs_grid();
        g->ctx = ctx;
        g->device = ctx->device;
        g->w = w;
        g->h = h;
        g->min_x = min_x;
        g->min_y = min_y;
        g->res = res;
        g->owned = true;
        size_t bytes = (size_t)w * (size_t)h * sizeof(double);
        if (bytes == 0) bytes = sizeof(double);
        if (hipMalloc(&g->d, bytes) != hipSuccess) {
            delete g;
            throw Error(LGS_ERR_OOM, "hipMalloc failed for grid");
        }
        LGS_HIP_CHECK(hipMemsetAsync(g->d, 0, bytes, ctx->stream));
        ctx->sync();
        *out = g;
    });
}

extern "C" int lgs_grid_wrap(lgs_ctx* ctx, double* dev, int w, int h, double min_x,
                             double min_y, double res, lgs_grid** out)
{
    if (!ctx || !out) return LGS_ERR_INVALID_ARG;
    *out = nullptr;
    return guarded(ctx, [&] {
        LGS_REQUIRE(dev != nullptr && w >= 0 && h >= 0 && res > 0.0, "invalid grid view");
        lgs_grid* g = new lgs_grid();
        g->ctx = ctx;
        g->device = ctx->device;
        g->d = dev;
        g->w = w;
        g->h = h;
        g->min_x = min_x;
        g->min_y = min_y;
        g->res = res;
        g->owned = false;
        *out = g;
    });
}

extern "C" void lgs_grid_destroy(lgs_grid* g)
{
    if (!g || g->map_view) return;
    if (g->owned && g->d) {
        hipSetDevice(g->device);
        hipFree(g->d);
    }
    delete g;
}

extern "C" int lgs_grid_upload(lgs_ctx* ctx, lgs_grid* g, const double* host)
{
    if (!ctx || !g || !host) return LGS_ERR_INVALID_ARG;
    return guarded(ctx, [&] {
        LGS_REQUIRE(!g->map_view, "cannot upload into a map's grid view");
        size_t bytes = (size_t)g->w * (size_t)g->h * sizeof(double);
        if (!bytes) return;
        grid_acquire(ctx, g);
        LGS_HIP_CHECK(hipMemcpyAsync(g->d, host, bytes, hipMemcpyHostToDevice, ctx->stream));
        ctx->sync();
    });
}

namespace {
__global__ __launch_bounds__(256) void k_patch_ingest(double* __restrict__ grid, int W, int H, int ps, int npx,
                                                      const int* __restrict__ slot,
                                                      const unsigned char* __restrict__ cells, int cell_bytes,
                                                      int value_offset)
{
    const int x = blockIdx.x * blockDim.x + threadIdx.x;
    if (x >= W) return;
    for (int y = blockIdx.y; y < H; y += gridDim.y) {
        const int s = slot[(y / ps) * npx + x / ps];
        double v = 0.0;
        if (s >= 0) {
            const size_t c = (size_t)s * ps * ps + (size_t)(y % ps) * ps + (x % ps);
            v = *(const double*)(cells + c * cell_bytes + value_offset);
        }
        grid[(size_t)y * W + x] = v;
    }
}
}

extern "C" int lgs_grid_upload_patches(lgs_ctx* ctx, lgs_grid* g, const void* const* patches, int npx, int npy,
                                       int ps, int cell_bytes, int value_offset)
{
    if (!ctx || !g || (!patches && npx * npy > 0)) return LGS_ERR_INVALID_ARG;
    return guarded(ctx, [&] {
        LGS_REQUIRE(!g->map_view, "cannot upload into a map's grid view");
        LGS_REQUIRE(npx >= 0 && npy >= 0 && ps >= 1, "invalid patch geometry");
        LGS_REQUIRE((long long)npx * ps == g->w && (long long)npy * ps == g->h,
                    "grid size must be npx*patch_size x npy*patch_size");
        LGS_REQUIRE(cell_bytes >= 8 && cell_bytes % 8 == 0 && value_offset >= 0 && value_offset % 8 == 0 &&
                        value_offset + 8 <= cell_bytes,
                    "cell_bytes / value_offset must describe an aligned fp64 inside each cell");
        if (!g->w || !g->h) return;
        LGS_HIP_CHECK(hipSetDevice(ctx->device));
        grid_acquire(ctx, g);
        const int np = npx * npy;
        const size_t patch_bytes = (size_t)ps * ps * cell_bytes;
        const size_t b_slot = ((size_t)np * sizeof(int) + 15) / 16 * 16;
        std::vector<int> slot(np);
        std::vector<int> order;
        for (int p = 0; p < np; ++p) {
            slot[p] = patches[p] ? (int)order.size() : -1;
            if (patches[p]) order.push_back(p);
        }
        const int na = (int)order.size();
        const size_t total = b_slot + (size_t)na * patch_bytes;
        char* h = (char*)ctx->ensure_pinned_in(total);
        char* d = (char*)ctx->ensure(S_INGEST, total);
        std::memcpy(h, slot.data(), (size_t)np * sizeof(int));
        LGS_HIP_CHECK(hipMemcpyAsync(d, h, b_slot, hipMemcpyHostToDevice, ctx->stream));
        constexpr size_t kChunkBytes = 2u << 20;
        const int per_chunk = (int)std::max<size_t>(1, kChunkBytes / patch_bytes);
        for (int c0 = 0; c0 < na; c0 += per_chunk) {
            const int c1 = std::min(na, c0 + per_chunk);
            host_parallel_for(c1 - c0, 1, [&](int k) {
                std::memcpy(h + b_slot + (size_t)(c0 + k) * patch_bytes, patches[order[c0 + k]], patch_bytes);
            });
            LGS_HIP_CHECK(hipMemcpyAsync(d + b_slot + (size_t)c0 * patch_bytes, h + b_slot + (size_t)c0 * patch_bytes,
                                         (size_t)(c1 - c0) * patch_bytes, hipMemcpyHostToDevice, ctx->stream));
        }
        hipLaunchKernelGGL(k_patch_ingest, dim3((g->w + 255) / 256, std::min(g->h, 65535)), dim3(256), 0, ctx->stream,
                           g->d, g->w, g->h, ps, npx, (const int*)d, (const unsigned char*)(d + b_slot), cell_bytes, value_offset);
        LGS_HIP_CHECK(hipGetLastError());
        ctx->sync();
    });
}

extern "C" int lgs_grid_download(lgs_ctx* ctx, const lgs_grid* g, double* host)
{
    if (!ctx || !g || !host) return LGS_ERR_INVALID_ARG;
    return guarded(ctx, [&] {
        size_t bytes = (size_t)g->w * (size_t)g->h * sizeof(double);
        if (!bytes) return;
        grid_acquire(ctx, g);
        LGS_HIP_CHECK(hipMemcpyAsync(host, g->d, bytes, hipMemcpyDeviceToHost, ctx->stream));
        ctx->sync();
    });
}

extern "C" int lgs_grid_fill(lgs_ctx* ctx, lgs_grid* g, double v)
{
    if (!ctx || !g) return LGS_ERR_INVALID_ARG;
    return guarded(ctx, [&] {
        size_t n = (size_t)g->w * (size_t)g->h;
        if (!n) return;
        unsigned blocks = (unsigned)std::min<size_t>((n + 255) / 256, 4096);
        hipLaunchKernelGGL(k_fill, dim3(blocks), dim3(256), 0, ctx->stream, g->d, n, v);
        LGS_HIP_CHECK(hipGetLastError());
    });
}

extern "C" int lgs_grid_info(const lgs_grid* g, int* w, int* h, double* min_x, double* min_y,
                             double* res)
{
    if (!g) return LGS_ERR_INVALID_ARG;
    if (w) *w = g->w;
    if (h) *h = g->h;
    if (min_x) *min_x = g->min_x;
    if (min_y) *min_y = g->min_y;
    if (res) *res = g->res;
    return LGS_OK;
}

extern "C" double* lgs_grid_device_ptr(lgs_grid* g) { return g ? g->d : nullptr; }

namespace {

constexpr int kTileX = 64;
constexpr int kTileY = 32;
constexpr int kMaxWinTiled = 32;

__device__ __forceinline__ int win_start(int i, int n, int w) { return (n >= w) ? min(i, n - w) : 0; }

__device__ __forceinline__ double dmax(double a, double b) { return (a < b) ? b : a; }

__device__ __forceinline__ void precompute_tile(const double* __restrict__ in, double* __restrict__ out, int W,
                                                int H, int w, const PlaneGeom& pg, int bx, int by)
{
    extern __shared__ double lds[];
    const int x0 = bx * kTileX, y0 = by * kTileY;
    const int x1 = min(x0 + kTileX, W), y1 = min(y0 + kTileY, H);
    const int sx0 = win_start(x0, W, w), sy0 = win_start(y0, H, w);
    const int sx1 = win_start(x1 - 1, W, w) + w, sy1 = win_start(y1 - 1, H, w) + w;
    const int fw = sx1 - sx0, fh = sy1 - sy0;
    double* tile = lds;
    double* m1 = lds + fh * fw;
    const int tid = threadIdx.x;
    for (int k0 = tid; k0 < fh * fw; k0 += 8 * (int)blockDim.x) {
        double v[8];
#pragma unroll
        for (int j = 0; j < 8; ++j) {
            const int k = k0 + j * (int)blockDim.x;
            const int yy = sy0 + k / fw, xx = sx0 + k % fw;
            v[j] = (k < fh * fw && xx < W && yy < H) ? in[(size_t)yy * W + xx] : 0.0;
        }
#pragma unroll
        for (int j = 0; j < 8; ++j) {
            const int k = k0 + j * (int)blockDim.x;
            if (k < fh * fw) tile[k] = v[j];
        }
    }
    __syncthreads();
    const int oh = y1 - y0;
    for (int k = tid; k < oh * fw; k += blockDim.x) {
        const int oy = k / fw, cx = k % fw;
        const int s = win_start(y0 + oy, H, w) - sy0;
        double m = tile[s * fw + cx];
        for (int j = 1; j < w; ++j) m = dmax(m, tile[(s + j) * fw + cx]);
        m1[oy * fw + cx] = m;
    }
    __syncthreads();
    const int ow = x1 - x0;
    for (int k = tid; k < oh * ow; k += blockDim.x) {
        const int oy = k / ow, ox = k % ow;
        const int s = win_start(x0 + ox, W, w) - sx0;
        double m = m1[oy * fw + s];
        for (int j = 1; j < w; ++j) m = dmax(m, m1[oy * fw + s + j]);
        const int x = x0 + ox, y = y0 + oy;
        if (pg.Wqp > 0) {
            const int qx = x / w, qy = y / w, rx = x - qx * w, ry = y - qy * w;
            out[(ry * w + rx) * pg.pstride + (long long)(qy + pg.M) * pg.Wqp + qx + pg.M] = m;
        } else {
            out[(size_t)y * W + x] = m;
        }
    }
}

__global__ __launch_bounds__(256) void k_precompute_tiled(const double* __restrict__ in,
                                                          double* __restrict__ out, int W,
                                                          int H, int w, PlaneGeom pg)
{
    precompute_tile(in, out, W, H, w, pg, blockIdx.x, blockIdx.y);
}

#ifndef LGS_PTY_BATCH
#define LGS_PTY_BATCH 8
#endif
#ifndef LGS_PTY_LONE
#define LGS_PTY_LONE 4
#endif
constexpr int pqx_of(int LR) { return ((257 - LR) / LR) & ~1; }
template <int LR>
constexpr int pqx() { return pqx_of(LR); }
typedef double d2a16 __attribute__((ext_vector_type(2)));
template <int LR, int kPTY = 16>
__global__ __launch_bounds__(256) void k_precompute_planes(const PrecompJob* __restrict__ jobs, DevTs dts)
{
    const DtsScope dts_scope(dts);
    const int gx = gridDim.x, gy = gridDim.y, nwg = gx * gy * gridDim.z;
    const int b = blockIdx.x + gx * (blockIdx.y + gy * blockIdx.z);
    const int xcd = b & 7, q = nwg >> 3, r = nwg & 7;
    const int l = (xcd < r ? xcd * (q + 1) : r * (q + 1) + (xcd - r) * q) + (b >> 3);
#ifdef LGS_NO_XCD
    const int bx = blockIdx.x, by = blockIdx.y, bz = blockIdx.z;
    (void)l;
#else
    const int bx = __builtin_amdgcn_readfirstlane(l % gx), by = __builtin_amdgcn_readfirstlane((l / gx) % gy),
              bz = __builtin_amdgcn_readfirstlane(l / (gx * gy));
#endif
    const PrecompJob& j = jobs[bz];
    const int W = j.W, H = j.H;
    constexpr int kPQX = pqx<LR>();
    const int x0 = bx * kPQX * LR, y0 = by * kPTY;
    if (x0 >= W || y0 >= H) return;
    const int x1 = min(x0 + kPQX * LR, W), y1 = min(y0 + kPTY, H);
    const int sx0 = win_start(x0, W, LR), sy0 = win_start(y0, H, LR);
    const int sx1 = win_start(x1 - 1, W, LR) + LR;
    const int fw = sx1 - sx0;
    const int oh = y1 - y0;
    constexpr int FW = kPQX * LR + LR - 1;
    static_assert(FW <= 256, "one footprint column per thread");
    constexpr int FH = kPTY + LR - 1;
    __shared__ double m1[kPTY][FW];
    const double* __restrict__ in = j.in;
    const int tid = threadIdx.x;
    int nz = 0;
    for (int c = tid; c < fw; c += 256) {
        const int xx = sx0 + c;
        double v[FH];
#pragma unroll
        for (int k = 0; k < FH; ++k) {
            const int yy = sy0 + k;
            v[k] = (xx < W && yy < H) ? gload(in + ((size_t)yy * W + xx)) : 0.0;
        }
#pragma unroll
        for (int k = 0; k < FH; ++k) nz |= __double_as_longlong(v[k]) != 0;
        double wm[kPTY];
#pragma unroll
        for (int k = 0; k < kPTY; ++k) {
            double m = v[k];
#pragma unroll
            for (int i = 1; i < LR; ++i) m = dmax(m, v[k + i]);
            wm[k] = m;
        }
        const int d = y0 - sy0, st = max(0, H - LR - sy0);
        if (d == 0 && st >= kPTY - 1) {
#pragma unroll
            for (int oy = 0; oy < kPTY; ++oy)
                if (oy < oh) m1[oy][c] = wm[oy];
        } else {
#pragma unroll
            for (int oy = 0; oy < kPTY; ++oy) {
                const int s = min(oy + d, st);
                double m = wm[0];
#pragma unroll
                for (int k = 1; k < kPTY; ++k) m = (k == s) ? wm[k] : m;
                if (oy < oh) m1[oy][c] = m;
            }
        }
    }
    unsigned* zw = j.zt ? j.zt + (by * gx + bx) : nullptr;
    if (zw) {
        const unsigned zprev = *zw;
        const int anynz = __syncthreads_or(nz);
        if (!anynz && zprev == 1u) return;
        if (tid == 0 && zprev != (anynz ? 0u : 1u)) *zw = anynz ? 0u : 1u;
    } else {
        __syncthreads();
    }
    const PlaneGeom& pg = j.pg;
    const int nq = (x1 - x0) / LR;
    const int np = (nq + 1) >> 1;
    double* __restrict__ out = j.out;
    for (int k = tid; k < oh * LR * (kPQX / 2); k += 256) {
        const int oy = k / (LR * (kPQX / 2)), rem = k % (LR * (kPQX / 2));
        const int rx = rem / (kPQX / 2), p = rem % (kPQX / 2);
        if (p >= np) continue;
        const int qxl = 2 * p;
        const int xa = x0 + qxl * LR + rx;
        const double* ca = &m1[oy][win_start(xa, W, LR) - sx0];
        double ma = ca[0];
#pragma unroll
        for (int i = 1; i < LR; ++i) ma = dmax(ma, ca[i]);
        const int y = y0 + oy, qy = y / LR, ry = y - qy * LR;
        const long long o = (ry * LR + rx) * pg.pstride + (long long)(qy + pg.M) * pg.Wqp + (x0 / LR + qxl) + pg.M;
        double* dst = out + o;
        if (qxl + 1 < nq) {
            const int xb = xa + LR;
            const double* cb = &m1[oy][win_start(xb, W, LR) - sx0];
            double mb = cb[0];
#pragma unroll
            for (int i = 1; i < LR; ++i) mb = dmax(mb, cb[i]);
            d2a16 v;
            v.x = ma;
            v.y = mb;
            gstore((d2a16*)dst, v);
            if (j.out16) {
                gstore((unsigned*)(j.out16 + o),
                       (unsigned)half_round_up_bits(ma) | ((unsigned)half_round_up_bits(mb) << 16));
                if (!(ma >= 0.0) || !(mb >= 0.0)) gstore(j.negflag, j.pgen);
            }
        } else {
            gstore(dst, ma);
            if (j.out16) {
                gstore(j.out16 + o, half_round_up_bits(ma));
                if (!(ma >= 0.0)) gstore(j.negflag, j.pgen);
            }
        }
    }
}

#ifndef LGS_PTY_SUB
#define LGS_PTY_SUB 2
#endif
template <int LR, int kPTY, int kSub>
__global__ __launch_bounds__(256) void k_precompute_planes_s(const PrecompJob* __restrict__ jobs, int gyt, DevTs dts)
{
    const DtsScope dts_scope(dts);
    const int gx = gridDim.x, gy = gridDim.y, nwg = gx * gy * gridDim.z;
    const int b = blockIdx.x + gx * (blockIdx.y + gy * blockIdx.z);
    const int xcd = b & 7, q = nwg >> 3, r = nwg & 7;
    const int l = (xcd < r ? xcd * (q + 1) : r * (q + 1) + (xcd - r) * q) + (b >> 3);
    const int bx = __builtin_amdgcn_readfirstlane(l % gx), bys = __builtin_amdgcn_readfirstlane((l / gx) % gy),
              bz = __builtin_amdgcn_readfirstlane(l / (gx * gy));
    const PrecompJob& j = jobs[bz];
    const int W = j.W, H = j.H;
    constexpr int kPQX = pqx<LR>();
    constexpr int FW = kPQX * LR + LR - 1;
    static_assert(FW <= 256, "one footprint column per thread");
    constexpr int FH = kPTY + LR - 1;
    const int x0 = bx * kPQX * LR;
    if (x0 >= W) return;
    const int x1 = min(x0 + kPQX * LR, W);
    const int sx0 = win_start(x0, W, LR);
    const int fw = win_start(x1 - 1, W, LR) + LR - sx0;
    __shared__ double m1[kPTY][FW];
    const double* __restrict__ in = j.in;
    const int tid = threadIdx.x;
    const int xx = sx0 + tid;
    const bool col = tid < fw, cin = col && xx < W;
    const int nq = (x1 - x0) / LR, np = (nq + 1) >> 1;
    const PlaneGeom& pg = j.pg;
    double* __restrict__ out = j.out;
    double v[FH];
    const int by0 = bys * kSub;
    int sy0 = win_start(by0 * kPTY, H, LR);
    if (by0 >= gyt || by0 * kPTY >= H) return;
#pragma unroll
    for (int k = 0; k < FH; ++k) {
        const int yy = sy0 + k;
        v[k] = (cin && yy < H) ? gload(in + ((size_t)yy * W + xx)) : 0.0;
    }
    for (int s = 0; s < kSub; ++s) {
        const int by = by0 + s, y0 = by * kPTY;
        if (by >= gyt || y0 >= H) break;
        const int y1 = min(y0 + kPTY, H), oh = y1 - y0;
        int nz = 0;
#pragma unroll
        for (int k = 0; k < FH; ++k) nz |= __double_as_longlong(v[k]) != 0;
        double wm[kPTY];
#pragma unroll
        for (int k = 0; k < kPTY; ++k) {
            double m = v[k];
#pragma unroll
            for (int i = 1; i < LR; ++i) m = dmax(m, v[k + i]);
            wm[k] = m;
        }
        if (s > 0) __syncthreads();
        const int d = y0 - sy0, st = max(0, H - LR - sy0);
        if (col) {
            if (d == 0 && st >= kPTY - 1) {
#pragma unroll
                for (int oy = 0; oy < kPTY; ++oy)
                    if (oy < oh) m1[oy][tid] = wm[oy];
            } else {
#pragma unroll
                for (int oy = 0; oy < kPTY; ++oy) {
                    const int sr = min(oy + d, st);
                    double m = wm[0];
#pragma unroll
                    for (int k = 1; k < kPTY; ++k) m = (k == sr) ? wm[k] : m;
                    if (oy < oh) m1[oy][tid] = m;
                }
            }
        }
        const int nby = by + 1;
        if (s + 1 < kSub && nby < gyt && nby * kPTY < H) {
            const int nsy0 = win_start(nby * kPTY, H, LR);
            if (nsy0 == sy0 + kPTY) {
#pragma unroll
                for (int k = 0; k < LR - 1; ++k) v[k] = v[k + kPTY];
#pragma unroll
                for (int k = LR - 1; k < FH; ++k) {
                    const int yy = nsy0 + k;
                    v[k] = (cin && yy < H) ? gload(in + ((size_t)yy * W + xx)) : 0.0;
                }
            } else {
#pragma unroll
                for (int k = 0; k < FH; ++k) {
                    const int yy = nsy0 + k;
                    v[k] = (cin && yy < H) ? gload(in + ((size_t)yy * W + xx)) : 0.0;
                }
            }
            sy0 = nsy0;
        }
        unsigned* zw = j.zt ? j.zt + (by * gx + bx) : nullptr;
        if (zw) {
            const unsigned zprev = *zw;
            const int anynz = __syncthreads_or(nz);
            if (tid == 0 && zprev != (anynz ? 0u : 1u)) *zw = anynz ? 0u : 1u;
            if (!anynz && zprev == 1u) continue;
        } else {
            __syncthreads();
        }
        for (int k = tid; k < oh * LR * (kPQX / 2); k += 256) {
            const int oy = k / (LR * (kPQX / 2)), rem = k % (LR * (kPQX / 2));
            const int rx = rem / (kPQX / 2), p = rem % (kPQX / 2);
            if (p >= np) continue;
            const int qxl = 2 * p;
            const int xa = x0 + qxl * LR + rx;
            const double* ca = &m1[oy][win_start(xa, W, LR) - sx0];
            double ma = ca[0];
#pragma unroll
            for (int i = 1; i < LR; ++i) ma = dmax(ma, ca[i]);
            const int y = y0 + oy, qy = y / LR, ry = y - qy * LR;
            const long long o = (ry * LR + rx) * pg.pstride + (long long)(qy + pg.M) * pg.Wqp + (x0 / LR + qxl) + pg.M;
            double* dst = out + o;
            if (qxl + 1 < nq) {
                const int xb = xa + LR;
                const double* cb = &m1[oy][win_start(xb, W, LR) - sx0];
                double mb = cb[0];
#pragma unroll
                for (int i = 1; i < LR; ++i) mb = dmax(mb, cb[i]);
                d2a16 vv;
                vv.x = ma;
                vv.y = mb;
                gstore((d2a16*)dst, vv);
                if (j.out16) {
                    gstore((unsigned*)(j.out16 + o),
                           (unsigned)half_round_up_bits(ma) | ((unsigned)half_round_up_bits(mb) << 16));
                    if (!(ma >= 0.0) || !(mb >= 0.0)) gstore(j.negflag, j.pgen);
                }
            } else {
                gstore(dst, ma);
                if (j.out16) {
                    gstore(j.out16 + o, half_round_up_bits(ma));
                    if (!(ma >= 0.0)) gstore(j.negflag, j.pgen);
                }
            }
        }
    }
}

__global__ __launch_bounds__(256) void k_precompute_jobs(const PrecompJob* __restrict__ jobs, int w)
{
    const int gx = gridDim.x, gy = gridDim.y, nwg = gx * gy * gridDim.z;
    const int b = blockIdx.x + gx * (blockIdx.y + gy * blockIdx.z);
    const int xcd = b & 7, q = nwg >> 3, r = nwg & 7;
    const int l = (xcd < r ? xcd * (q + 1) : r * (q + 1) + (xcd - r) * q) + (b >> 3);
#ifdef LGS_NO_XCD
    const int bx = blockIdx.x, by = blockIdx.y, bz = blockIdx.z;
    (void)l;
#else
    const int bx = __builtin_amdgcn_readfirstlane(l % gx), by = __builtin_amdgcn_readfirstlane((l / gx) % gy),
              bz = __builtin_amdgcn_readfirstlane(l / (gx * gy));
#endif
    const PrecompJob& j = jobs[bz];
    if (bx * kTileX >= j.W || by * kTileY >= j.H) return;
    precompute_tile(j.in, j.out, j.W, j.H, w, j.pg, bx, by);
}

__global__ void k_precompute_sep_y(const double* __restrict__ in, double* __restrict__ out, int W, int H, int w)
{
    const int x = blockIdx.x * blockDim.x + threadIdx.x;
    const int y = blockIdx.y;
    if (x >= W) return;
    const int s = win_start(y, H, w);
    double m = 0.0;
    for (int j = 0; j < w; ++j) {
        const double v = (s + j < H) ? in[(size_t)(s + j) * W + x] : 0.0;
        m = (j == 0) ? v : dmax(m, v);
    }
    out[(size_t)y * W + x] = m;
}

__global__ void k_precompute_sep_x(const double* __restrict__ in, double* __restrict__ out, int W, int H, int w)
{
    const int x = blockIdx.x * blockDim.x + threadIdx.x;
    const int y = blockIdx.y;
    if (x >= W) return;
    const int s = win_start(x, W, w);
    const double* row = in + (size_t)y * W;
    double m = 0.0;
    for (int j = 0; j < w; ++j) {
        const double v = (s + j < W) ? row[s + j] : 0.0;
        m = (j == 0) ? v : dmax(m, v);
    }
    out[(size_t)y * W + x] = m;
}

}

namespace lgs {
bool precompute_planes_ok(const lgs_grid* in, int win)
{
    return win >= 1 && win <= kMaxWinTiled && in->w % win == 0 && in->h % win == 0;
}

void launch_precompute(lgs_ctx* ctx, const lgs_grid* in, int win, double* out, const PlaneGeom* planes)
{
    LGS_REQUIRE(!planes || precompute_planes_ok(in, win), "phase-plane precompute needs W, H multiples of the window");
    const PlaneGeom pg = planes ? *planes : PlaneGeom{ 0, 0, 0 };
    if (in->w == 0 || in->h == 0) return;
    const int tok = ctx->timing_begin(K_PRECOMPUTE, 32.0 * (double)in->w * (double)in->h);
    if (ctx->skipped(K_PRECOMPUTE)) {
    } else if (win <= kMaxWinTiled) {
        const int fw = kTileX + win - 1, fh = kTileY + win - 1;
        const size_t lds = (size_t)(fh * fw + kTileY * fw) * sizeof(double);
        dim3 grid((in->w + kTileX - 1) / kTileX, (in->h + kTileY - 1) / kTileY);
        hipLaunchKernelGGL(k_precompute_tiled, grid, dim3(256), lds, ctx->stream, in->d, out,
                           in->w, in->h, win, pg);
    } else {
        LGS_REQUIRE(!planes, "phase-plane precompute: window must be <= 32");
        double* tmp = (double*)ctx->ensure(S_PRECOMP_TMP, sizeof(double) * (size_t)in->w * in->h);
        dim3 grid((in->w + 255) / 256, in->h);
        hipLaunchKernelGGL(k_precompute_sep_y, grid, dim3(256), 0, ctx->stream, in->d, tmp, in->w, in->h, win);
        hipLaunchKernelGGL(k_precompute_sep_x, grid, dim3(256), 0, ctx->stream, tmp, out, in->w, in->h, win);
    }
    ctx->timing_end(tok);
    LGS_HIP_CHECK(hipGetLastError());
}
void precompute_tile_grid(int maxW, int maxH, int win, int njobs, int* gx, int* gy, int* rows)
{
    const int q = pqx_of(win) * win;
    *rows = njobs == 1 ? LGS_PTY_LONE : LGS_PTY_BATCH;
    *gx = (maxW + q - 1) / q;
    *gy = (maxH + *rows - 1) / *rows;
}
void launch_precompute_jobs(lgs_ctx* ctx, const PrecompJob* d_jobs, int njobs, int maxW, int maxH, int win)
{
    LGS_REQUIRE(win >= 1 && win <= kMaxWinTiled, "batched precompute: window must be in [1, 32]");
    if (njobs == 0 || maxW == 0 || maxH == 0) return;
    const int tok = ctx->timing_begin(K_PRECOMPUTE, 32.0 * (double)maxW * (double)maxH * njobs);
    if (ctx->skipped(K_PRECOMPUTE)) {
    } else if (win <= 8) {
        switch (win) {
#define LGS_PP_CASE(L) case L: \
            if (njobs == 1) \
                hipLaunchKernelGGL(HIP_KERNEL_NAME(k_precompute_planes<L, LGS_PTY_LONE>), \
                    dim3((maxW + pqx<L>() * L - 1) / (pqx<L>() * L), (maxH + LGS_PTY_LONE - 1) / LGS_PTY_LONE, njobs), \
                    dim3(256), 0, ctx->stream, d_jobs, ctx->dts(tok)); \
            else if (LGS_PTY_SUB > 1) { \
                const int gyt = (maxH + LGS_PTY_BATCH - 1) / LGS_PTY_BATCH; \
                hipLaunchKernelGGL(HIP_KERNEL_NAME(k_precompute_planes_s<L, LGS_PTY_BATCH, LGS_PTY_SUB>), \
                    dim3((maxW + pqx<L>() * L - 1) / (pqx<L>() * L), (gyt + LGS_PTY_SUB - 1) / LGS_PTY_SUB, njobs), \
                    dim3(256), 0, ctx->stream, d_jobs, gyt, ctx->dts(tok)); \
            } else \
                hipLaunchKernelGGL(HIP_KERNEL_NAME(k_precompute_planes<L, LGS_PTY_BATCH>), \
                    dim3((maxW + pqx<L>() * L - 1) / (pqx<L>() * L), (maxH + LGS_PTY_BATCH - 1) / LGS_PTY_BATCH, njobs), dim3(256), 0, ctx->stream, \
                    d_jobs, ctx->dts(tok)); \
            break;
        LGS_PP_CASE(1) LGS_PP_CASE(2) LGS_PP_CASE(3) LGS_PP_CASE(4) LGS_PP_CASE(5) LGS_PP_CASE(6)
        LGS_PP_CASE(7) LGS_PP_CASE(8)
#undef LGS_PP_CASE
        }
    } else {
        const int fw = kTileX + win - 1, fh = kTileY + win - 1;
        const size_t lds = (size_t)(fh * fw + kTileY * fw) * sizeof(double);
        dim3 grid((maxW + kTileX - 1) / kTileX, (maxH + kTileY - 1) / kTileY, njobs);
        hipLaunchKernelGGL(k_precompute_jobs, grid, dim3(256), lds, ctx->stream, d_jobs, win);
    }
    ctx->timing_end(tok);
    LGS_HIP_CHECK(hipGetLastError());
}
}

extern "C" int lgs_grid_precompute_max(lgs_ctx* ctx, const lgs_grid* in, int win, lgs_grid* out)
{
    if (!ctx || !in || !out) return LGS_ERR_INVALID_ARG;
    return guarded(ctx, [&] {
        LGS_REQUIRE(win >= 1, "window must be >= 1");
        LGS_REQUIRE(out->w == in->w && out->h == in->h, "precompute output geometry mismatch");
        LGS_REQUIRE(out->d != in->d, "precompute cannot run in place");
        grid_acquire(ctx, in);
        out->min_x = in->min_x;
        out->min_y = in->min_y;
        out->res = in->res;
        launch_precompute(ctx, in, win, out->d, nullptr);
    });
}

namespace {
constexpr size_t kScanPoolBytes = size_t(64) << 20;
struct ScanPool {
    std::mutex mu;
    std::vector<std::vector<void*>> bins;
    size_t held = 0;
};
ScanPool& scan_pool(int device)
{
    static std::mutex mu;
    static std::vector<std::unique_ptr<ScanPool>> pools;
    std::lock_guard<std::mutex> g(mu);
    if ((int)pools.size() <= device) pools.resize((size_t)device + 1);
    if (!pools[device]) pools[device].reset(new ScanPool());
    return *pools[device];
}
int scan_bin(size_t bytes)
{
    int b = 8;
    while ((size_t(1) << b) < bytes) ++b;
    return b;
}
void* scan_buffer_get(int device, size_t bytes)
{
    const int b = scan_bin(bytes);
    ScanPool& P = scan_pool(device);
    {
        std::lock_guard<std::mutex> g(P.mu);
        if ((int)P.bins.size() > b && !P.bins[b].empty()) {
            void* p = P.bins[b].back();
            P.bins[b].pop_back();
            P.held -= size_t(1) << b;
            return p;
        }
    }
    void* p = nullptr;
    if (hipMalloc(&p, size_t(1) << b) != hipSuccess) throw Error(LGS_ERR_OOM, "hipMalloc failed for scan");
    return p;
}
void scan_buffer_put(int device, void* p, size_t bytes)
{
    const int b = scan_bin(bytes);
    ScanPool& P = scan_pool(device);
    {
        std::lock_guard<std::mutex> g(P.mu);
        if (P.held + (size_t(1) << b) <= kScanPoolBytes) {
            if ((int)P.bins.size() <= b) P.bins.resize((size_t)b + 1);
            P.bins[b].push_back(p);
            P.held += size_t(1) << b;
            return;
        }
    }
    hipSetDevice(device);
    hipFree(p);
}
}

extern "C" int lgs_scan_create(lgs_ctx* ctx, const lgs_scan_host* hs, lgs_scan** out)
{
    if (!ctx || !hs || !out) return LGS_ERR_INVALID_ARG;
    *out = nullptr;
    return guarded(ctx, [&] {
        LGS_REQUIRE(hs->n >= 1 && hs->ranges && hs->angles, "scan must have >= 1 beam");
        LGS_HIP_CHECK(hipSetDevice(ctx->device));
        lgs_scan* s = new lgs_scan();
        std::unique_ptr<lgs_scan> own(s);
        static std::atomic<unsigned long long> uids{ 0 };
        s->uid = uids.fetch_add(1, std::memory_order_relaxed) + 1;
        s->ctx = ctx;
        s->device = ctx->device;
        s->n = hs->n;
        s->rel = hs->rel_sensor_pose;
        s->min_range = hs->min_range;
        s->max_range = hs->max_range;
        s->h_ranges.assign(hs->ranges, hs->ranges + hs->n);
        s->h_angles.assign(hs->angles, hs->angles + hs->n);
        double m = hs->ranges[0];
        for (int i = 1; i < hs->n; ++i)
            if (m < hs->ranges[i]) m = hs->ranges[i];
// ... 277 lines not shown
```

### my-lidar-graph-slam_amd/csrc/lgs_internal.hpp

```cpp
#pragma once

#include <hip/hip_runtime.h>

#include <climits>
#include <cmath>
#include <cstdint>
#include <cstring>
#include <functional>
#include <stdexcept>
#include <string>
#include <memory>
#include <map>
#include <mutex>
#include <atomic>
#include <condition_variable>
#include <utility>
#include <vector>

#include "lgs_hip.h"

namespace lgs {

struct Error : std::runtime_error {
    int code;
    Error(int c, const std::string& m) : std::runtime_error(m), code(c) {}
};

#define LGS_HIP_CHECK(expr)                                                              \
    do {                                                                                 \
        hipError_t e_ = (expr);                                                          \
        if (e_ != hipSuccess)                                                            \
            throw ::lgs::Error(LGS_ERR_HIP, std::string(#expr) + ": " + hipGetErrorString(e_)); \
    } while (0)

#define LGS_REQUIRE(cond, msg)                                                           \
    do {                                                                                 \
        if (!(cond))                                                                     \
            throw ::lgs::Error(LGS_ERR_INVALID_ARG, msg);                                \
    } while (0)

enum Slot {
    S_IDX = 0,
    S_CSCORE,
    S_CFLAG,
    S_SEL,
    S_LIST,
    S_FVAL,
    S_FPOS,
    S_PART_C,
    S_PART_K,
    S_CUB_TEMP,
    S_COUNT,
    S_RECORDS,
    S_POSES7,
    S_COST_IDX,
    S_COST_TERM,
    S_PATCH,
    S_INGEST,
    S_DENSE_FINE,
    S_COARSE_GRID,
    S_DECIM,
    S_CINFO,
    S_TEDGE,
    S_RAY0, S_RAY1, S_RAY2, S_RAY3, S_RAY4, S_RAY5, S_RAY6, S_RAY7,
    S_RAY8,
    S_LS0, S_LS1,
    S_LIN0, S_LIN1,
    S_LIN2,
    S_LIN3,
    S_SUPER,
    S_SBOUND,
    S_UPLOAD,
    S_BATCH_WS,
    S_NEGFLAG,
    S_BB0, S_BB1, S_BB2, S_BB3, S_BB4, S_BB5,
    S_PRECOMP_TMP,
    S_KEEP,
    S_COLL,
    S_ZTILE,
    S_GS0, S_GS1,
    S_HC0, S_HC1,
    S_PG0, S_PG1,
    S_PG2, S_PG3,
    S_BATCH_WS_B, S_RECORDS_B, S_UPLOAD_B, S_DECIM_B, S_SUPER_B, S_NEGFLAG_B, S_TEDGE_B, S_ZTILE_B,
    S_NUM_SLOTS
};

constexpr int kGuardInline = 64;
constexpr int kTedgeCtrs = 64;

struct GuardRec { int t, v, ix, iy; };
struct CostGuardRec { int pose_which, beam, ix, iy; };

struct RtcsmRecord {
    int status;
    int found;
    unsigned long long guard_word;
    unsigned long long cost_guard_word;
    long long n_eval;
    int best[3];
    int sq_err;
    double score_max;
    double L;
    double costs[7];
    unsigned long long coarse_evals;
    int gx_err[8];
    GuardRec guard[kGuardInline];
    CostGuardRec cost_guard[kGuardInline];
};

enum RecordStatus { REC_DANGEROUS = 1 };

struct RtcsmPlan {
    double sx, sy, st;
    double step_x, step_y, step_t;
    double min_x, min_y, res;
    double thr;
    int W, H;
    int win_x, win_y, win_t;
    int T, ncx, ncy, P;
    int low_res;
    int Nv;
    int N;
    double rmax;
    int Wq, Hq, M, Wqp, Hqp;
    long long pstride;
    long long K;
    int nsbx, nsby;
    double sb_mult;
    int Wq4, Hq4;
    long long sub4, pstride4;
    long long sb_off;
    int oct, Qo, unit8;
    long long subO, pstrideO;
};

struct PlaneGeom {
    int M, Wqp;
    long long pstride;
};

struct PrecompJob {
    const double* in;
    double* out;
    int W, H;
    PlaneGeom pg;
    unsigned short* out16;
    int* negflag;
    int pgen;
    unsigned* zt;
};

__device__ __forceinline__ unsigned short half_round_up_bits_cvt(double m)
{
    const _Float16 h = (_Float16)(float)m;
    unsigned short b = __builtin_bit_cast(unsigned short, h);
    if ((double)(float)h < m) b = (m > 0.0) ? (unsigned short)(b + 1) : (unsigned short)(b - 1);
    if (m == 0.0 || m != m) b = 0;
    return b;
}
__device__ __forceinline__ unsigned short half_round_up_bits(double m)
{
    const unsigned long long b = __builtin_bit_cast(unsigned long long, m);
    const unsigned hi = (unsigned)(b >> 32), lo = (unsigned)b;
    const unsigned e = (hi >> 20) & 0x7FFu;
    if ((hi >> 31) == 0u && e >= 1009u && e < 2047u) {
        if (e > 1038u) return 0x7C00u;
        unsigned h = ((e - 1008u) << 10) | ((hi >> 10) & 0x3FFu);
        h += ((hi & 0x3FFu) | lo) != 0u;
        return (unsigned short)h;
    }
    return half_round_up_bits_cvt(m);
}

struct CostPlan {
    double min_range, max_range;
    double hit_and_missed_dist, occupancy_threshold;
    double variance, scaling_factor;
    double min_x, min_y, res;
    int W, H, kernel_size, N;
};

}

#ifdef LGS_PROBE
#define LGS_PROBE_DECL unsigned long long lgs_probe_t[16]; int lgs_probe_n = 0
#define LGS_PROBE_MARK() do { if (threadIdx.x == 0) lgs_probe_t[lgs_probe_n < 16 ? lgs_probe_n++ : 15] = wall_clock64(); } while (0)
#define LGS_PROBE_PRINT(name) do { if (threadIdx.x == 0 && blockIdx.x == 0 && blockIdx.y == 0) { \
    printf("probe %s:", name); for (int i_ = 1; i_ < lgs_probe_n; ++i_) printf(" %.2f", 0.01 * (double)(lgs_probe_t[i_] - lgs_probe_t[i_ - 1])); \
    printf(" us\n"); } } while (0)
#else
#define LGS_PROBE_DECL do { } while (0)
#define LGS_PROBE_MARK() do { } while (0)
#define LGS_PROBE_PRINT(name) do { } while (0)
#endif

namespace lgs {
enum KernelId { K_PROJECT = 0, K_COARSE, K_SEED, K_SELECT, K_FINE, K_REPLAY, K_COST, K_PRECOMPUTE,
                K_LINSOLVE, K_RAY_EMIT, K_RAY_APPLY, K_SUPER, K_SUPER_PLANES, K_BB_SCORE, K_BB_EXPAND,
                K_COARSE_AUX,
                K_MATCH_SMALL,
                K_GS_SCORE,
                K_COST_SQ,
                K_COST_GX,
                K_NUM_KERNELS };
extern const char* const kKernelNames[K_NUM_KERNELS];
struct PendingTiming {
    int kernel;
    hipEvent_t a, b;
    double algo_bytes;
    bool coarse_evals = false;
    long long batch = 0;
    const unsigned long long* hw = nullptr;
    unsigned long long tag = 0;
};

constexpr int kDtsSub = 8;
constexpr int kDtsEvery = 31;
constexpr int kDtsSlots = 32;
constexpr unsigned long long kDtsMask = (1ull << 40) - 1ull;
struct DevTs {
    unsigned long long* w;
    unsigned long long tag;
};
__device__ __forceinline__ void dts_begin(const DevTs& d)
{
    if (d.w && threadIdx.x == 0 && threadIdx.y == 0) {
        const unsigned b = blockIdx.x + gridDim.x * (blockIdx.y + gridDim.y * blockIdx.z);
        if (b < (unsigned)kDtsSub) {
            const unsigned long long t = __builtin_amdgcn_s_memrealtime() & kDtsMask;
            __hip_atomic_fetch_max(d.w + 2 * b, d.tag | (kDtsMask - t), __ATOMIC_RELAXED, __HIP_MEMORY_SCOPE_AGENT);
        }
    }
}
__device__ __forceinline__ void dts_end(const DevTs& d)
{
    if (d.w && threadIdx.x == 0 && threadIdx.y == 0) {
        const unsigned b = blockIdx.x + gridDim.x * (blockIdx.y + gridDim.y * blockIdx.z);
        const unsigned nwg = gridDim.x * gridDim.y * gridDim.z;
        if (b + (unsigned)kDtsSub >= nwg || b % (unsigned)kDtsEvery == 0u) {
            const unsigned long long t = __builtin_amdgcn_s_memrealtime() & kDtsMask;
            const unsigned sub = (b + b / (unsigned)kDtsEvery) & (unsigned)(kDtsSub - 1);
            __hip_atomic_fetch_max(d.w + 2 * sub + 1, d.tag | t, __ATOMIC_RELAXED, __HIP_MEMORY_SCOPE_AGENT);
        }
    }
}
struct DtsScope {
    const DevTs d;
    __device__ explicit DtsScope(const DevTs& x) : d(x) { dts_begin(d); }
    __device__ ~DtsScope() { dts_end(d); }
};
}

struct lgs_ctx {
    int device = 0;
    hipStream_t stream = nullptr;
    std::string last_error;
    double guard_eps = 1e-9;
    bool force_dense = false;
    bool inject_index = false;
    int guard_cap = lgs::kGuardInline;
    bool super_prune = true;
    bool linsolve_split = true;
    long long handoff_spin_us = 200000;
#ifndef LGS_FINE_STAGED_DEFAULT
#define LGS_FINE_STAGED_DEFAULT 1
#endif
    bool fine_staged = LGS_FINE_STAGED_DEFAULT;
    long long coop_tiles = -1;
    long long sort_barrier_us = 50000;
    long long handoff_fallbacks = 0;
    bool peer_staged = false;
    int prune_min_super = 1;
    bool small_window = true;
    bool fused_planes = true;
    int seed_wide = 12;
    bool lean_project = true;
    bool fast_rows = true;
    bool zero_tiles = true;
    bool device_hits = true;
    bool split_chunks = false;
    bool hv_full = false;
    bool prio_tail = false;
    hipStream_t hi = nullptr;
    hipEvent_t split_ev[2] = {};
    bool post_records = true;
    long long copies_direct = 0, copies_staged = 0;
    int lanes_min_batch = 2;
    long long ray_chunk_keys = 1LL << 28;
    int next_stamp();
    unsigned skip_mask = 0;
    bool skipped(int kernel) const { return (skip_mask >> kernel) & 1u; }
    bool poison_ws = false;
    struct DbgItem {
        const void* buf[10];
        size_t bytes[10];
        int gen;
    };
    std::vector<DbgItem> dbg;
    int generation = 0;
    void* buf[lgs::S_NUM_SLOTS] = {};
    size_t buf_bytes[lgs::S_NUM_SLOTS] = {};
    void* pinned = nullptr;
    size_t pinned_bytes = 0;
    void* pinned_up = nullptr;
    size_t pinned_up_bytes = 0;
    void* pinned_up_b = nullptr;
    size_t pinned_up_b_bytes = 0;
    bool up_busy[2] = { false, false };
    void* pinned_rec[2] = {};
    size_t pinned_rec_bytes[2] = {};
    int bank = 0;
    size_t tedge_zeroed[2] = {};
    int* tedge_buffer(size_t n);
    int* small_counters(size_t n);
    int banked(int slot) const
    {
        if (!bank) return slot;
        switch (slot) {
        case lgs::S_BATCH_WS: return lgs::S_BATCH_WS_B;
        case lgs::S_RECORDS: return lgs::S_RECORDS_B;
        case lgs::S_UPLOAD: return lgs::S_UPLOAD_B;
        case lgs::S_DECIM: return lgs::S_DECIM_B;
        case lgs::S_SUPER: return lgs::S_SUPER_B;
        case lgs::S_NEGFLAG: return lgs::S_NEGFLAG_B;
        case lgs::S_TEDGE: return lgs::S_TEDGE_B;
        case lgs::S_ZTILE: return lgs::S_ZTILE_B;
        default: return slot;
        }
    }
    void* ensure_pinned_rec(size_t bytes);
    void* pinned_scan[2] = {};
    size_t pinned_scan_bytes[2] = {};
    hipEvent_t scan_ev[2] = {};
    bool scan_ev_live[2] = {};
    void* pinned_in = nullptr;
    size_t pinned_in_bytes = 0;
    void* pinned_pg = nullptr;
    size_t pinned_pg_bytes = 0;
    void* ensure_pinned_pg(size_t bytes);
    std::shared_ptr<void> pg_cache;
    long long pg_solves = 0, pg_iterations = 0, pg_patterns = 0, pg_grid_solves = 0;
    int pg_grid_nodes = 1280;
    hipEvent_t pg_ev[2] = {};
    long long pglm_optimizes = 0, pglm_steps = 0, pglm_pose_uploads = 0, pglm_pose_downloads = 0, pglm_incidence_builds = 0;
    void* planes_ptr[2] = {};
    int planes_sets[2] = {};
    void* super_ptr[2] = {};
    int super_sets[2] = {};
    long long planes_key[2][4] = { { -1, -1, -1, -1 }, { -1, -1, -1, -1 } };
    long long zt_key[2][12] = {};
    std::vector<unsigned char> zt_pre[2], zt_hv[2];
    std::vector<long long> zt_dims[2];
    double* zero = nullptr;
    bool profile = false;
    unsigned profile_mask = ~0u;
    std::vector<lgs::PendingTiming> pending;
    std::vector<hipEvent_t> event_pool;
    int64_t stat_launches[lgs::K_NUM_KERNELS] = {};
    double stat_ms[lgs::K_NUM_KERNELS] = {};
    double stat_bytes[lgs::K_NUM_KERNELS] = {};
    double stat_disp_ms[lgs::K_NUM_KERNELS] = {};
    int64_t count_matches = 0, count_coarse_blocks = 0, count_coarse_blocks_dense = 0, count_pruned = 0;

    int timing_begin(int kernel, double algo_bytes);
    void timing_end(int token);
    bool dev_timing = false;
    unsigned long long* dts_buf[2] = {};
    unsigned long long* dts_dev = nullptr;
    const unsigned long long* dts_host = nullptr;
    int dts_used = 0;
    unsigned dts_gen = 0;
    lgs::DevTs dts(int token) const
    {
        if (token < 0 || !pending[(size_t)token].hw) return lgs::DevTs{ nullptr, 0ull };
        const size_t slot = (size_t)(pending[(size_t)token].hw - dts_host) / (2 * lgs::kDtsSub);
        return lgs::DevTs{ dts_dev + slot * 2 * lgs::kDtsSub, pending[(size_t)token].tag };
    }
    void harvest();
    void harvest_upto(long long b);
    long long timing_batch = 0;
    hipEvent_t bank_ev[2] = {};
    void wait_event(hipEvent_t ev);

    bool spin_sync = true;
    void sync();

    struct GeTable {
        int K;
        double sd, res;
        std::vector<double> host;
        double* dev;
    };
    std::vector<GeTable> ge_tables;
    const double* ge_table(const lgs_cost_ge_params* cost, double res);

    void* ensure(int slot, size_t bytes);
    std::vector<void*> aux;
    std::vector<size_t> aux_bytes;
    void* ensure_aux(int i, size_t bytes);
    void* ensure_pinned(size_t bytes);
    void* ensure_pinned_up(size_t bytes);
    void* ensure_pinned_in(size_t bytes);
    void release();
};

namespace lgs {
struct WriterEvent {
    hipEvent_t ev = nullptr;
    std::atomic<hipStream_t> st{ nullptr };
    unsigned* flag = nullptr;
    std::atomic<unsigned> gen{ 0 };
    std::mutex mu;
    WriterEvent() = default;
    WriterEvent(const WriterEvent&) = delete;
    WriterEvent& operator=(const WriterEvent&) = delete;
    ~WriterEvent()
    {
        if (ev) hipEventDestroy(ev);
        if (flag) hipHostFree(flag);
    }
    bool done() const { return __atomic_load_n(flag, __ATOMIC_ACQUIRE) == gen.load(std::memory_order_acquire); }
    void wait()
    {
        for (unsigned spins = 1; !done(); ++spins) {
            if (spins % 4096) continue;
            const hipError_t e = hipStreamQuery(st.load(std::memory_order_acquire));
            if (e == hipSuccess && !done()) throw Error(LGS_ERR_INTERNAL, "map writer: completion word lost");
            if (e != hipSuccess && e != hipErrorNotReady) LGS_HIP_CHECK(e);
        }
    }
    void order_after(hipStream_t reader)
    {
        std::lock_guard<std::mutex> lk(mu);
        if (done()) return;
        if (!ev) LGS_HIP_CHECK(hipEventCreateWithFlags(&ev, hipEventDisableTiming));
        LGS_HIP_CHECK(hipEventRecord(ev, st.load(std::memory_order_acquire)));
        LGS_HIP_CHECK(hipStreamWaitEvent(reader, ev, 0));
    }
};
}

struct lgs_grid {
    lgs_ctx* ctx = nullptr;
    int device = 0;
    double* d = nullptr;
    int w = 0, h = 0;
    double min_x = 0, min_y = 0, res = 0;
    bool owned = false;
    bool map_view = false;
    std::shared_ptr<lgs::WriterEvent> writer;
};

namespace lgs {
struct CopyFence {
    std::mutex mu;
    std::condition_variable cv;
    int state = 0;
    void set(int s)
    {
        {
            std::lock_guard<std::mutex> g(mu);
            state = s;
        }
        cv.notify_all();
    }
    int wait()
    {
        std::unique_lock<std::mutex> g(mu);
        cv.wait(g, [&] { return state != 0; });
        return state;
    }
};
}

#ifndef LGS_GLOBAL_GATHER
#define LGS_GLOBAL_GATHER 1
#endif
#ifdef __HIP_DEVICE_COMPILE__
template <class T>
__device__ __forceinline__ T gload(const T* p)
{
#if LGS_GLOBAL_GATHER
    return *(const __attribute__((address_space(1))) T*)p;
#else
    return *p;
#endif
}
template <class T>
__device__ __forceinline__ void gstore(T* p, T v)
{
#if LGS_GLOBAL_GATHER
    *(__attribute__((address_space(1))) T*)p = v;
#else
    *p = v;
#endif
}
#else
template <class T>
__device__ __forceinline__ T gload(const T* p)
{
    return *p;
}
template <class T>
__device__ __forceinline__ void gstore(T* p, T v)
{
    *p = v;
}
#endif

struct lgs_scan {
    lgs_ctx* ctx = nullptr;
    int device = 0;
    unsigned long long uid = 0;
    double* d_ranges = nullptr;
    double* d_angles = nullptr;
    std::mutex dev_mu;
    const lgs_ctx* dev_ctx = nullptr;
    std::shared_ptr<lgs::CopyFence> dev_fence;
    std::atomic<bool> dev_done{ false };
    int n = 0;
    lgs_pose2d rel{0, 0, 0};
    double min_range = 0, max_range = 0;
    double max_elem = 0;
    std::vector<double> h_ranges, h_angles;
    mutable std::mutex cache_mu;
    std::map<uint64_t, std::vector<int>> vidx_by_rmax;
    mutable std::shared_ptr<const void> hits_cache;
    mutable double hits_key[5] = { NAN, NAN, NAN, NAN, NAN };
};

extern "C" void sincos(double x, double* s, double* c);

namespace lgs {

inline void ref_sincos(double x, double& s, double& c) { ::sincos(x, &s, &c); }

inline lgs_pose2d compound(lgs_pose2d s, lgs_pose2d d)
{
    double sinT, cosT;
    ref_sincos(s.theta, sinT, cosT);
    return { cosT * d.x - sinT * d.y + s.x, sinT * d.x + cosT * d.y + s.y, s.theta + d.theta };
}
inline lgs_pose2d move_backward(lgs_pose2d e, lgs_pose2d d)
{
    const double theta = e.theta - d.theta;
    double sinT, cosT;
    ref_sincos(theta, sinT, cosT);
    return { e.x - cosT * d.x + sinT * d.y, e.y - sinT * d.x - cosT * d.y, theta };
}
inline lgs_pose2d inverse_compound(lgs_pose2d s, lgs_pose2d e)
{
    double sinT, cosT;
    ref_sincos(s.theta, sinT, cosT);
    const double dx = e.x - s.x, dy = e.y - s.y;
    return { cosT * dx + sinT * dy, -sinT * dx + cosT * dy, e.theta - s.theta };
}

const int* scan_valid_indices(lgs_ctx* ctx, lgs_scan* scan, double scan_range_max, int* nv);
struct Upload;
void scans_to_device(lgs_ctx* ctx, const lgs_scan* const* scans, int n, Upload* up = nullptr);
using ForeignScans = std::vector<std::pair<lgs_scan*, std::shared_ptr<CopyFence>>>;
void wait_foreign_scans(ForeignScans& f);
void abandon_scan_copies(lgs_ctx* ctx, const std::shared_ptr<CopyFence>& fence, const std::vector<lgs_scan*>& scans);
void fetch_async(lgs_ctx* ctx, void* dst, const void* src, size_t bytes);
struct FetchSeg {
    const unsigned char* src;
    unsigned char* dst;
    unsigned long long bytes;
};
constexpr int kFetchSegs = 8;
struct FetchList {
    FetchSeg s[kFetchSegs];
};
FetchSeg fetch_seg(void* dst, const void* src, size_t bytes);
void fetch_list(lgs_ctx* ctx, const std::vector<FetchSeg>& segs);
constexpr size_t kFetchMaxBytes = size_t(1) << 20;
void sincos_batch(const double* x, long long n, double* s, double* c);
void cells_of_points(const double* xy, long long n2, double mx, double my, double res, int* out);
inline void scan_to_device(lgs_ctx* ctx, const lgs_scan* s) { scans_to_device(ctx, &s, 1); }

inline void grid_acquire(lgs_ctx* ctx, const lgs_grid* g)
{
    if (g && g->writer && g->writer->st.load(std::memory_order_acquire) != ctx->stream)
        g->writer->order_after(ctx->stream);
}

struct Upload {
    lgs_ctx* ctx;
    std::vector<char> host;
    char* dev = nullptr;
    std::vector<FetchSeg> extra;
    std::shared_ptr<CopyFence> fence;
    std::vector<lgs_scan*> fence_scans;
    ForeignScans foreign;
    explicit Upload(lgs_ctx* c) : ctx(c) {}
    Upload(const Upload&) = delete;
    Upload& operator=(const Upload&) = delete;
    ~Upload()
    {
        if (!extra.empty()) {
            try {
                fetch_list(ctx, extra);
            } catch (...) {
                if (fence) abandon_scan_copies(ctx, fence, fence_scans);
                fence.reset();
            }
        }
        if (fence) fence->set(1);
    }
    template <class T>
    size_t append(const T* p, size_t n)
    {
        const size_t off = (host.size() + 255) & ~(size_t)255;
        host.resize(off + sizeof(T) * n);
        std::memcpy(host.data() + off, p, sizeof(T) * n);
        return off;
    }
    char* prepare()
    {
        dev = (char*)ctx->ensure(ctx->banked(S_UPLOAD), std::max<size_t>(host.size(), 16));
        return dev;
    }
    void copy()
    {
        const size_t b = std::max<size_t>(host.size(), 16);
        if (ctx->up_busy[ctx->bank]) ctx->sync();
        char* pin = (char*)ctx->ensure_pinned_up(b);
        std::memcpy(pin, host.data(), host.size());
        std::vector<FetchSeg> segs;
        try {
            if (host.size() <= kFetchMaxBytes)
                segs.push_back(fetch_seg(dev, pin, host.size()));
            else
                LGS_HIP_CHECK(hipMemcpyAsync(dev, pin, host.size(), hipMemcpyHostToDevice, ctx->stream));
            segs.insert(segs.end(), extra.begin(), extra.end());
            extra.clear();
            fetch_list(ctx, segs);
        } catch (...) {
            extra.clear();
            if (fence) abandon_scan_copies(ctx, fence, fence_scans);
            fence.reset();
            fence_scans.clear();
            ctx->up_busy[ctx->bank] = true;
            throw;
        }
        ctx->up_busy[ctx->bank] = true;
        if (fence) fence->set(1);
        fence.reset();
        fence_scans.clear();
        if (!foreign.empty()) wait_foreign_scans(foreign);
    }
    void flush()
    {
        prepare();
        copy();
    }
    template <class T>
    T* host_at(size_t off) { return (T*)(host.data() + off); }
    template <class T>
    const T* at(size_t off) const { return (const T*)(dev + off); }
};

template <class F>
int guarded(lgs_ctx* ctx, F&& f)
{
    try {
        f();
// ... 81 lines not shown
```

### my-lidar-graph-slam_amd/lgs_amd/abi.py

```python
from __future__ import annotations

import ctypes as C
import os
from typing import Optional, Sequence

import numpy as np

_HERE = os.path.dirname(os.path.abspath(__file__))
LIB_PATH = os.path.join(_HERE, "liblgs_hip.so")

LGS_OK = 0
LGS_OPT_GUARD_EPS = 1
LGS_OPT_FORCE_DENSE = 2
LGS_OPT_INJECT_INDEX = 3
LGS_OPT_GUARD_CAP = 4
LGS_OPT_PROFILE = 5
LGS_OPT_PROFILE_MASK = 7
LGS_OPT_SPIN_SYNC = 8
LGS_OPT_SUPER_PRUNE = 9
LGS_OPT_LANES_MIN_BATCH = 11
LGS_OPT_RAY_CHUNK_KEYS = 13
LGS_OPT_POISON_WS = 15
LGS_OPT_SKIP_MASK = 10
LGS_OPT_LINSOLVE_SPLIT = 17
LGS_OPT_HANDOFF_SPIN_US = 18
LGS_OPT_PEER_COPY = 19
LGS_OPT_PRUNE_MIN_SUPER = 21
LGS_OPT_COOP_TILES = 22
LGS_OPT_SORT_BARRIER_US = 23
LGS_OPT_FINE_STAGED = 24
LGS_OPT_SMALL_WINDOW = 25
LGS_OPT_POST_RECORDS = 26
LGS_OPT_FUSED_PLANES = 27
LGS_OPT_PRIORITY_TAIL = 28
LGS_OPT_HV_FULL = 29
LGS_OPT_SPLIT_CHUNKS = 30
LGS_OPT_DEVICE_HITS = 31
LGS_OPT_SEED_WIDE = 32
LGS_OPT_ZERO_TILES = 33
LGS_OPT_DEVICE_TIMING = 34
LGS_OPT_LEAN_PROJECT = 35
LGS_OPT_PGCG_GRID_NODES = 36
LGS_OPT_FAST_ROWS = 37
KERNEL_IDS = ["k_project", "k_coarse", "k_seed", "k_select", "k_fine", "k_replay", "k_cost", "k_precompute",
              "k_linsolve", "k_ray_emit", "k_ray_apply", "k_super", "k_super_planes", "k_bb_score",
              "k_bb_expand", "k_coarse_aux", "k_match_small", "k_gs_score",
              "k_cost_sq", "k_cost_gx"]


class Pose2D(C.Structure):
    _fields_ = [("x", C.c_double), ("y", C.c_double), ("theta", C.c_double)]

    def tuple(self):
        return (self.x, self.y, self.theta)


class ScanHost(C.Structure):
    _fields_ = [
        ("ranges", C.POINTER(C.c_double)),
        ("angles", C.POINTER(C.c_double)),
        ("n", C.c_int),
        ("rel_sensor_pose", Pose2D),
        ("min_range", C.c_double),
        ("max_range", C.c_double),
    ]


class RtcsmParams(C.Structure):
    _fields_ = [
        ("low_resolution", C.c_int),
        ("range_x", C.c_double),
        ("range_y", C.c_double),
        ("range_theta", C.c_double),
        ("scan_range_max", C.c_double),
    ]


class CostGEParams(C.Structure):
    _fields_ = [
        ("usable_range_min", C.c_double),
        ("usable_range_max", C.c_double),
        ("hit_and_missed_dist", C.c_double),
        ("occupancy_threshold", C.c_double),
        ("kernel_size", C.c_int),
        ("scaling_factor", C.c_double),
        ("standard_deviation", C.c_double),
    ]


class RtcsmSummary(C.Structure):
    _fields_ = [
        ("pose_found", C.c_int),
        ("normalized_cost", C.c_double),
        ("initial_pose", Pose2D),
        ("estimated_pose", Pose2D),
        ("covariance", C.c_double * 9),
        ("score_max", C.c_double),
        ("score_threshold", C.c_double),
        ("best_win", C.c_int * 3),
        ("win", C.c_int * 3),
        ("steps", C.c_double * 3),
        ("best_sensor_pose", Pose2D),
        ("coarse_blocks", C.c_int64),
        ("fine_blocks", C.c_int64),
        ("guard_hits", C.c_int),
        ("fixups", C.c_int),
        ("slow_path", C.c_int),
    ]


class BBParams(C.Structure):
    _fields_ = [("node_height_max", C.c_int), ("range_x", C.c_double), ("range_y", C.c_double),
                ("range_theta", C.c_double), ("scan_range_max", C.c_double),
                ("score_usable_range_min", C.c_double), ("score_usable_range_max", C.c_double)]


class GSParams(C.Structure):
    _fields_ = [("range_x", C.c_double), ("range_y", C.c_double), ("range_theta", C.c_double),
                ("step_x", C.c_double), ("step_y", C.c_double), ("step_theta", C.c_double),
                ("score_usable_range_min", C.c_double), ("score_usable_range_max", C.c_double)]


class HCParams(C.Structure):
    _fields_ = [("linear_step", C.c_double), ("angular_step", C.c_double), ("max_iterations", C.c_int),
                ("max_num_of_refinements", C.c_int)]
# ... 53 lines not shown
                    npx=self.num_patches_x, npy=self.num_patches_y)

    def res(self):
        return self.resolution


class LinsolveParams(C.Structure):
    _fields_ = [("num_iterations_max", C.c_int), ("convergence_threshold", C.c_double),
                ("usable_range_min", C.c_double), ("usable_range_max", C.c_double),
                ("translation_regularizer", C.c_double), ("rotation_regularizer", C.c_double),
                ("cost_usable_range_min", C.c_double), ("cost_usable_range_max", C.c_double)]


class LinsolveSummary(C.Structure):
    _fields_ = [("pose_found", C.c_int), ("iterations", C.c_int), ("normalized_cost", C.c_double),
                ("initial_pose", Pose2D), ("estimated_pose", Pose2D), ("covariance", C.c_double * 9),
                ("sensor_pose", Pose2D), ("best_sensor_pose", Pose2D), ("cost", C.c_double)]


class LoopQuery(C.Structure):
    _fields_ = [("map", C.c_void_p), ("coarse", C.c_void_p), ("local_map_node_pose", Pose2D),
                ("local_map_node_index", C.c_int), ("first_candidate", C.c_int), ("num_candidates", C.c_int)]


class LoopCandidate(C.Structure):
    _fields_ = [("scan", C.c_void_p), ("node_pose", Pose2D), ("node_index", C.c_int), ("pad", C.c_int)]


class LoopResult(C.Structure):
    _fields_ = [("found", C.c_int), ("start_node_index", C.c_int), ("end_node_index", C.c_int), ("pad", C.c_int),
                ("relative_pose", Pose2D), ("start_node_pose", Pose2D), ("estimated_pose", Pose2D),
                ("covariance", C.c_double * 9), ("score", C.c_double), ("normalized_cost", C.c_double)]


LOOP_RESULT_DOUBLES = 22


class KernelStat(C.Structure):
    _fields_ = [("name", C.c_char * 32), ("launches", C.c_int64), ("total_ms", C.c_double),
                ("algo_bytes", C.c_double), ("dispatch_ms", C.c_double)]


_P = C.c_void_p
class PgEdge(C.Structure):
    _fields_ = [("start_node_index", C.c_int), ("end_node_index", C.c_int), ("relative_pose", Pose2D),
                ("information", C.c_double * 9)]


class PgLmParams(C.Structure):
    _fields_ = [("num_iterations_max", C.c_int), ("error_tolerance", C.c_double), ("loss_kind", C.c_int),
                ("loss_scale", C.c_double)]


def pg_edges(edges):
    arr = (PgEdge * max(1, len(edges)))()
    for k, (s, e, z, info) in enumerate(edges):
        arr[k].start_node_index, arr[k].end_node_index = s, e
        arr[k].relative_pose = Pose2D(*z)
        arr[k].information[:] = [float(v) for v in np.asarray(info, dtype=np.float64).reshape(9)]
    return arr


_PROTOS = [
    ("lgs_abi_version", C.c_int, []),
    ("lgs_ctx_create", C.c_int, [C.c_int, C.POINTER(_P)]),
    ("lgs_ctx_destroy", None, [_P]),
    ("lgs_ctx_last_error", C.c_char_p, [_P]),
    ("lgs_ctx_synchronize", C.c_int, [_P]),
    ("lgs_ctx_stream", _P, [_P]),
    ("lgs_ctx_set_option", C.c_int, [_P, C.c_int, C.c_double]),
    ("lgs_ctx_kernel_stats", C.c_int, [_P, C.POINTER(KernelStat), C.c_int]),
    ("lgs_ctx_reset_stats", C.c_int, [_P]),
    ("lgs_ctx_match_counters", C.c_int, [_P, C.POINTER(C.c_int64)]),
    ("lgs_grid_create", C.c_int, [_P, C.c_int, C.c_int, C.c_double, C.c_double, C.c_double, C.POINTER(_P)]),
    ("lgs_grid_wrap", C.c_int, [_P, _P, C.c_int, C.c_int, C.c_double, C.c_double, C.c_double, C.POINTER(_P)]),
    ("lgs_grid_destroy", None, [_P]),
    ("lgs_grid_upload", C.c_int, [_P, _P, C.POINTER(C.c_double)]),
    ("lgs_grid_upload_patches", C.c_int, [_P, _P, C.POINTER(_P), C.c_int, C.c_int, C.c_int, C.c_int, C.c_int]),
    ("lgs_grid_download", C.c_int, [_P, _P, C.POINTER(C.c_double)]),
    ("lgs_grid_fill", C.c_int, [_P, _P, C.c_double]),
    ("lgs_grid_info", C.c_int, [_P, C.POINTER(C.c_int), C.POINTER(C.c_int), C.POINTER(C.c_double),
                                 C.POINTER(C.c_double), C.POINTER(C.c_double)]),
    ("lgs_grid_device_ptr", _P, [_P]),
    ("lgs_grid_precompute_max", C.c_int, [_P, _P, C.c_int, _P]),
    ("lgs_scan_create", C.c_int, [_P, C.POINTER(ScanHost), C.POINTER(_P)]),
    ("lgs_scan_destroy", None, [_P]),
    ("lgs_rtcsm_optimize_pose", C.c_int, [_P, _P, _P, C.POINTER(RtcsmParams), C.POINTER(CostGEParams), _P,
                                          Pose2D, C.c_double, C.POINTER(RtcsmSummary)]),
    ("lgs_rtcsm_optimize_pose_query", C.c_int, [_P, _P, C.POINTER(RtcsmParams), C.POINTER(CostGEParams), _P,
                                                Pose2D, C.POINTER(RtcsmSummary)]),
    ("lgs_rtcsm_optimize_pose_query_batch", C.c_int, [_P, C.POINTER(_P), C.POINTER(RtcsmParams),
                                                      C.POINTER(CostGEParams), C.POINTER(_P), C.POINTER(Pose2D),
                                                      C.c_int, C.POINTER(RtcsmSummary)]),
    ("lgs_rtcsm_optimize_pose_batch", C.c_int, [_P, _P, _P, C.POINTER(RtcsmParams), C.POINTER(CostGEParams),
                                                C.POINTER(_P), C.POINTER(Pose2D), C.c_int, C.c_double,
                                                C.POINTER(RtcsmSummary)]),
    ("lgs_rtcsm_dense_scores", C.c_int, [_P, _P, _P, C.POINTER(RtcsmParams), _P, Pose2D,
                                         C.POINTER(C.c_double), C.POINTER(C.c_double), C.POINTER(C.c_int)]),
    ("lgs_cost_greedy_endpoint", C.c_int, [_P, _P, C.POINTER(CostGEParams), _P, Pose2D,
                                           C.POINTER(C.c_double)]),
    ("lgs_scan_get", C.c_int, [_P, C.POINTER(C.c_int), C.POINTER(C.c_double), C.POINTER(C.c_double)]),
    ("lgs_scan_interpolate", C.c_int, [_P, _P, C.c_double, C.c_double, C.POINTER(_P)]),
    ("lgs_map_create", C.c_int, [_P, C.c_double, C.c_int, C.c_int, C.c_int, C.c_double, C.c_double,
                                 C.POINTER(_P)]),
    ("lgs_map_destroy", None, [_P]),
    ("lgs_map_get_geometry", C.c_int, [_P, C.POINTER(MapGeometry)]),
    ("lgs_map_grid", C.c_int, [_P, C.POINTER(_P)]),
    ("lgs_map_update_scan", C.c_int, [_P, _P, _P, Pose2D, C.POINTER(BuilderParams)]),
    ("lgs_map_construct_from_scans", C.c_int, [_P, _P, C.POINTER(_P), C.POINTER(Pose2D), C.c_int,
                                               C.POINTER(BuilderParams)]),
    ("lgs_map_append_scan", C.c_int, [_P, _P, _P, C.POINTER(_P), C.POINTER(Pose2D), C.c_int,
                                      C.POINTER(BuilderParams)]),
    ("lgs_maps_construct_from_scans", C.c_int, [_P, C.POINTER(_P), C.POINTER(C.c_int), C.POINTER(C.c_int),
                                                C.c_int, C.POINTER(_P), C.POINTER(Pose2D), C.c_int,
                                                C.POINTER(BuilderParams)]),
    ("lgs_map_construct_global", C.c_int, [_P, C.c_double, C.c_int, C.POINTER(_P), C.POINTER(Pose2D), C.c_int,
                                           C.POINTER(BuilderParams), C.POINTER(_P)]),
    ("lgs_map_render_gray", C.c_int, [_P, _P, C.POINTER(C.c_uint8)]),
    ("lgs_map_render_gray_region", C.c_int, [_P, _P, C.c_int, C.c_int, C.c_int, C.c_int, C.c_int,
                                             C.POINTER(C.c_uint8)]),
    ("lgs_map_download_patches", C.c_int, [_P, _P, C.POINTER(C.c_uint8)]),
    ("lgs_map_actual_size", C.c_int, [_P, _P, C.POINTER(C.c_int), C.POINTER(C.c_int)]),
    ("lgs_map_download", C.c_int, [_P, _P, C.POINTER(C.c_double), C.POINTER(C.c_uint32),
                                   C.POINTER(C.c_uint32)]),
    ("lgs_grid_precompute_pyramid", C.c_int, [_P, _P, C.c_int, C.POINTER(_P)]),
    ("lgs_bb_optimize_pose_batch", C.c_int, [_P, _P, C.POINTER(_P), C.POINTER(BBParams), C.POINTER(CostGEParams),
                                             C.POINTER(_P), C.POINTER(Pose2D), C.c_int, C.c_double,
                                             C.POINTER(RtcsmSummary)]),
    ("lgs_bb_optimize_pose_query", C.c_int, [_P, _P, C.POINTER(BBParams), C.POINTER(CostGEParams), _P, Pose2D,
                                             C.POINTER(RtcsmSummary)]),
    ("lgs_loop_detect_bb", C.c_int, [_P, C.POINTER(BBParams), C.POINTER(CostGEParams), C.c_double,
                                     C.POINTER(LoopQuery), C.c_int, C.POINTER(LoopCandidate), C.c_int,
                                     C.POINTER(LoopResult)]),
    ("lgs_gs_steps", C.c_int, [C.c_double, C.c_double, C.POINTER(C.c_double), C.c_int]),
    ("lgs_gs_optimize_pose_batch", C.c_int, [_P, _P, C.POINTER(GSParams), C.POINTER(CostGEParams), C.POINTER(_P),
                                             C.POINTER(Pose2D), C.c_int, C.c_double, C.POINTER(RtcsmSummary)]),
    ("lgs_gs_optimize_pose_query", C.c_int, [_P, _P, C.POINTER(GSParams), C.POINTER(CostGEParams), _P, Pose2D,
                                             C.POINTER(RtcsmSummary)]),
    ("lgs_gs_dense_scores", C.c_int, [_P, _P, C.POINTER(GSParams), _P, Pose2D, C.POINTER(C.c_double),
                                      C.c_longlong]),
    ("lgs_loop_detect_gs", C.c_int, [_P, C.POINTER(GSParams), C.POINTER(CostGEParams), C.c_double,
                                     C.POINTER(LoopQuery), C.c_int, C.POINTER(LoopCandidate), C.c_int,
                                     C.POINTER(LoopResult)]),
    ("lgs_hc_term_table", C.c_int, [C.POINTER(CostGEParams), C.c_double, C.POINTER(C.c_double),
                                    C.POINTER(C.c_double), C.c_int]),
    ("lgs_hc_optimize_pose_query", C.c_int, [_P, _P, C.POINTER(HCParams), C.POINTER(CostGEParams), _P, Pose2D,
                                             C.POINTER(HCSummary)]),
    ("lgs_hc_optimize_pose_batch", C.c_int, [_P, C.POINTER(_P), C.POINTER(HCParams), C.POINTER(CostGEParams),
                                             C.POINTER(_P), C.POINTER(Pose2D), C.c_int, C.POINTER(HCSummary)]),
    ("lgs_hc_trace", C.c_int, [_P, _P, C.POINTER(HCParams), C.POINTER(CostGEParams), _P, Pose2D,
                               C.POINTER(C.c_int), C.POINTER(C.c_double), C.c_int]),
    ("lgs_cost_ge_exact", C.c_int, [_P, _P, C.POINTER(CostGEParams), _P, C.POINTER(Pose2D), C.c_int,
                                    C.POINTER(C.c_double)]),
    ("lgs_loop_detect_rtcsm", C.c_int, [_P, C.POINTER(RtcsmParams), C.POINTER(CostGEParams), C.c_double,
                                        C.POINTER(LoopQuery), C.c_int, C.POINTER(LoopCandidate), C.c_int,
                                        C.POINTER(LoopResult)]),
    ("lgs_loop_detect_rtcsm_multi", C.c_int, [C.POINTER(_P), C.c_int, C.POINTER(RtcsmParams),
                                              C.POINTER(CostGEParams), C.c_double, C.POINTER(LoopQuery), C.c_int,
                                              C.POINTER(LoopCandidate), C.c_int, C.POINTER(LoopResult)]),
    ("lgs_cost_spec_size", C.c_size_t, []),
    ("lgs_rtcsm_optimize_pose_cost", C.c_int, [_P, _P, _P, C.POINTER(RtcsmParams), C.POINTER(CostSpec), _P,
                                               Pose2D, C.c_double, C.POINTER(RtcsmSummary)]),
    ("lgs_rtcsm_optimize_pose_query_cost", C.c_int, [_P, _P, C.POINTER(RtcsmParams), C.POINTER(CostSpec), _P,
                                                     Pose2D, C.POINTER(RtcsmSummary)]),
    ("lgs_rtcsm_optimize_pose_query_batch_cost", C.c_int, [_P, C.POINTER(_P), C.POINTER(RtcsmParams),
                                                           C.POINTER(CostSpec), C.POINTER(_P), C.POINTER(Pose2D),
# ... 662 lines not shown

    def construct_maps(self, maps, ranges, scans, poses, bp: "BuilderParams"):
        nm, n = len(maps), len(scans)
        mh = (_P * nm)(*[m.h for m in maps])
        lo = (C.c_int * nm)(*[int(a) for a, _ in ranges])
        hi = (C.c_int * nm)(*[int(b) for _, b in ranges])
        arr = (_P * n)(*[s.h for s in scans])
        ps = (Pose2D * n)(*[Pose2D(*p) for p in poses])
        self.check(self.lib.lgs_maps_construct_from_scans(self.h, mh, lo, hi, nm, arr, ps, n, C.byref(bp)),
                   "maps_construct_from_scans")

    def construct_global_map(self, res: float, patch_size: int, scans, poses, bp: "BuilderParams") -> "Map":
        n = len(scans)
        arr = (_P * n)(*[s.h for s in scans])
        ps = (Pose2D * n)(*[Pose2D(*p) for p in poses])
        h = _P()
        self.check(self.lib.lgs_map_construct_global(self.h, res, patch_size, arr, ps, n, C.byref(bp), C.byref(h)),
                   "map_construct_global")
        return Map(self, h)

    DEBUG_BUFFERS = {"sbound": (0, np.float64), "part_c": (1, np.float64), "part_k": (2, np.int64),
                     "L": (3, np.float64), "tedge": (4, np.int32), "cbase": (5, np.int32), "idx": (6, np.int32),
                     "cscore": (7, np.float64), "planes": (8, np.float64), "super": (9, np.float16)}

    def debug_buffer(self, name: str, item: int = 0) -> np.ndarray:
        which, dt = self.DEBUG_BUFFERS[name]
        n = C.c_size_t()
        self.check(self.lib.lgs_debug_item_buffer(self.h, item, which, None, 0, C.byref(n)), "debug_item_buffer")
        out = np.zeros(n.value // np.dtype(dt).itemsize, dtype=dt)
        self.check(self.lib.lgs_debug_item_buffer(self.h, item, which, out.ctypes.data_as(_P), out.nbytes,
                                                  C.byref(n)),
                   "debug_item_buffer")
        return out

    def debug_libm(self, op: int, x) -> np.ndarray:
        x = np.ascontiguousarray(x, dtype=np.float64)
        out = np.zeros((len(x), 2) if op == 0 else len(x), dtype=np.float64)
        self.check(self.lib.lgs_debug_libm(self.h, op, x.ctypes.data_as(_P), len(x), out.ctypes.data_as(_P)),
                   "debug_libm")
        return out

    def copy_counters(self) -> dict:
        a, b = C.c_longlong(), C.c_longlong()
        self.check(self.lib.lgs_debug_copy_counters(self.h, C.byref(a), C.byref(b)), "debug_copy_counters")
        return {"direct": a.value, "staged": b.value}

    def offset_checks(self, reset: bool = True) -> dict:
        out = (C.c_ulonglong * 4)()
        self.check(self.lib.lgs_debug_offset_checks(self.h, 1 if reset else 0, out), "debug_offset_checks")
        return {"checked": out[0], "violations": out[1], "first": out[2], "first_base": out[3]}

    def debug_keysort(self, keys, lo: int, bits: int) -> np.ndarray:
        k = np.ascontiguousarray(keys, dtype=np.uint32)
        out = np.zeros_like(k)
        self.check(self.lib.lgs_debug_keysort(self.h, k.ctypes.data_as(_P), out.ctypes.data_as(_P), len(k), lo, bits),
                   "debug_keysort")
        return out

    def cost_greedy_endpoint(self, grid, cost: CostGEParams, scan, pose) -> float:
        v = C.c_double()
        self.check(self.lib.lgs_cost_greedy_endpoint(self.h, grid.h, C.byref(cost), scan.h, Pose2D(*pose),
                                                     C.byref(v)), "cost_greedy_endpoint")
        return v.value


class Grid:
    def __init__(self, ctx: Context, h, w, hh, min_x, min_y, res, owned=True, map_view=None):
        self.ctx, self.h = ctx, h
        self.map_view = map_view
        self.w, self.hgt = w, hh
        self.min_x, self.min_y, self.res = min_x, min_y, res
        self.owned = owned

    def upload(self, cells: np.ndarray):
        cells = np.ascontiguousarray(cells, dtype=np.float64)
        assert cells.shape == (self.hgt, self.w)
        self.ctx.check(self.ctx.lib.lgs_grid_upload(self.ctx.h, self.h, dptr(cells)), "grid_upload")

    def download(self) -> np.ndarray:
        out = np.zeros((self.hgt, self.w))
        self.ctx.check(self.ctx.lib.lgs_grid_download(self.ctx.h, self.h, dptr(out)), "grid_download")
        return out

    def device_ptr(self) -> int:
        return self.ctx.lib.lgs_grid_device_ptr(self.h)

    def close(self):
        if self.h:
            if self.map_view is None:
                self.ctx.lib.lgs_grid_destroy(self.h)
            self.h = None

    def __del__(self):
        try:
            self.close()
        except Exception:
            pass


class Map:

    def __init__(self, ctx: Context, h):
        self.ctx, self.h = ctx, h

    def geometry(self) -> dict:
        g = MapGeometry()
        self.ctx.check(self.ctx.lib.lgs_map_get_geometry(self.h, C.byref(g)), "map_geometry")
        return g.dict()

    def grid(self) -> "Grid":
        gh = _P()
        self.ctx.check(self.ctx.lib.lgs_map_grid(self.h, C.byref(gh)), "map_grid")
        mg = MapGeometry()
        self.ctx.check(self.ctx.lib.lgs_map_get_geometry(self.h, C.byref(mg)), "map_geometry")
        return Grid(self.ctx, gh, mg.num_cells_x, mg.num_cells_y, mg.min_x, mg.min_y, mg.resolution,
                    owned=False, map_view=self)

    def update_scan(self, scan: "Scan", robot_pose, bp: BuilderParams):
        self.ctx.check(self.ctx.lib.lgs_map_update_scan(self.ctx.h, self.h, scan.h, Pose2D(*robot_pose),
                                                        C.byref(bp)), "map_update_scan")

    def construct(self, scans, poses, bp: BuilderParams):
        n = len(scans)
        arr = (_P * n)(*[s.h for s in scans])
        ps = (Pose2D * n)(*[Pose2D(*p) for p in poses])
        self.ctx.check(self.ctx.lib.lgs_map_construct_from_scans(self.ctx.h, self.h, arr, ps, n, C.byref(bp)),
                       "map_construct_from_scans")

    def append_scan(self, latest: "Map", scans, poses, bp: BuilderParams):
        n = len(scans)
        arr = (_P * n)(*[s.h for s in scans])
        ps = (Pose2D * n)(*[Pose2D(*p) for p in poses])
        self.ctx.check(self.ctx.lib.lgs_map_append_scan(self.ctx.h, self.h, latest.h, arr, ps, n, C.byref(bp)),
                       "map_append_scan")

    def rebuilds(self) -> dict:
        a, b = C.c_longlong(), C.c_longlong()
        self.ctx.check(self.ctx.lib.lgs_debug_map_rebuilds(self.h, C.byref(a), C.byref(b)), "debug_map_rebuilds")
        return {"incremental": a.value, "full": b.value}

    def render_gray(self) -> np.ndarray:
        g = self.geometry()
        img = np.zeros((g["h"], g["w"]), dtype=np.uint8)
        if img.size:
            self.ctx.check(self.ctx.lib.lgs_map_render_gray(self.ctx.h, self.h,
                                                            img.ctypes.data_as(C.POINTER(C.c_uint8))),
                           "map_render_gray")
        return img

    def render_gray_region(self, x0, y0, w, h, flip=True) -> np.ndarray:
        img = np.zeros((h, w), dtype=np.uint8)
        self.ctx.check(self.ctx.lib.lgs_map_render_gray_region(self.ctx.h, self.h, x0, y0, w, h, int(flip),
                                                               img.ctypes.data_as(C.POINTER(C.c_uint8))),
                       "map_render_gray_region")
        return img

    def patches(self) -> np.ndarray:
        g = self.geometry()
        f = np.zeros((g["npy"], g["npx"]), dtype=np.uint8)
        if f.size:
            self.ctx.check(self.ctx.lib.lgs_map_download_patches(self.ctx.h, self.h,
                                                                 f.ctypes.data_as(C.POINTER(C.c_uint8))),
                           "map_download_patches")
        return f

    def actual_size(self):
        n = C.c_int()
        out = (C.c_int * 12)()
# ... 43 lines not shown
```

Baseline: 102,600.

## Add per-grid occupancy bitmap to skip loading empty tiles in plane precompute

Builds a 16x16-block occupancy bitmap for each grid on upload and patch ingest, and invalidates it on any other write path. The plane precompute kernels read this bitmap and skip global loads for tiles whose footprint is entirely zero, aiming to cut memory traffic over sparse maps. An optional verification mode records any tile wrongly marked empty, and the occupancy kernel variant also raises its launch-bounds occupancy hint. The cost is an extra summarise kernel plus memset per upload, extra bitmap memory, and correctness depends on every writer invalidating the bitmap.

```diff
diff --git a/include/lgs_hip.h b/include/lgs_hip.h
--- a/include/lgs_hip.h
+++ b/include/lgs_hip.h
@@ -102,6 +102,7 @@
 #define LGS_OPT_LEAN_PROJECT  35
 #define LGS_OPT_PGCG_GRID_NODES 36
 #define LGS_OPT_FAST_ROWS     37
+#define LGS_OPT_GRID_OCCUPANCY 38
 #define LGS_OPT_POISON_WS     15
 int  lgs_ctx_set_option(lgs_ctx* ctx, int option, double value);
 
@@ -139,6 +140,9 @@
 int  lgs_grid_info(const lgs_grid* grid, int* w, int* h, double* min_x, double* min_y,
                    double* resolution);
 double* lgs_grid_device_ptr(lgs_grid* grid);
+const double* lgs_grid_device_cells(const lgs_grid* grid);
+int  lgs_grid_occupancy_info(lgs_ctx* ctx, const lgs_grid* grid, int* valid, int* block_w, int* block_h,
+                             int64_t* blocks_set);
 
 int  lgs_grid_precompute_max(lgs_ctx* ctx, const lgs_grid* in, int win, lgs_grid* out);
 
diff --git a/my-lidar-graph-slam_amd/csrc/k_bb.hip b/my-lidar-graph-slam_amd/csrc/k_bb.hip
--- a/my-lidar-graph-slam_amd/csrc/k_bb.hip
+++ b/my-lidar-graph-slam_amd/csrc/k_bb.hip
@@ -857,6 +857,7 @@
         for (int h = 0; h <= node_height_max; ++h) {
             LGS_REQUIRE(pyramid[h] && pyramid[h]->w == in->w && pyramid[h]->h == in->h,
                         "pyramid grids must have the input's size");
+            grid_touch(pyramid[h]);
             launch_precompute(ctx, in, 1 << h, pyramid[h]->d, nullptr);
         }
         ctx->sync();
diff --git a/my-lidar-graph-slam_amd/csrc/k_rtcsm.hip b/my-lidar-graph-slam_amd/csrc/k_rtcsm.hip
--- a/my-lidar-graph-slam_amd/csrc/k_rtcsm.hip
+++ b/my-lidar-graph-slam_amd/csrc/k_rtcsm.hip
@@ -15,7 +15,7 @@
 
 namespace lgs {
 void launch_precompute(lgs_ctx* ctx, const lgs_grid* in, int win, double* out, const PlaneGeom* planes);
-void launch_precompute_jobs(lgs_ctx* ctx, const PrecompJob* d_jobs, int njobs, int maxW, int maxH, int win);
+void launch_precompute_jobs(lgs_ctx* ctx, const PrecompJob* d_jobs, int njobs, int maxW, int maxH, int win, bool occ);
 bool precompute_planes_ok(const lgs_grid* in, int win);
 void precompute_tile_grid(int maxW, int maxH, int win, int njobs, int* gx, int* gy, int* rows);
 }
@@ -3737,6 +3737,9 @@
 struct SetJobs {
     size_t jobs_off = 0, njobs = 0, pj_off = 0, npj = 0, dj_off = 0, ndj = 0;
     bool hv = false;
+    unsigned long long* occ_err = nullptr;
+    int occ_n = 0;
+    bool occ = false;
 };
 
 inline bool hv_mode(const lgs_ctx* ctx, const RtcsmPlan& lp) { return ctx->fused_planes && lp.oct; }
@@ -3839,6 +3842,7 @@
     std::vector<int> job_set;
     std::vector<PlaneJob> pj;
     std::vector<DecimJob> djobs;
+    unsigned long long* occ_err = nullptr;
     for (int s = 0; s < ns; ++s) {
         PlaneSet& ps = sets[s];
         ps.cmap = D + ssz * (size_t)s;
@@ -3862,6 +3866,15 @@
             q.W = ps.fine->w;
             q.H = ps.fine->h;
             q.pg = PlaneGeom{ lp.M, lp.Wqp, lp.pstride };
+            q.occ = ctx->grid_occupancy ? grid_occ(ps.fine) : nullptr;
+            q.occ_ws = occ::row_words(q.W);
+            if (q.occ && ctx->grid_occupancy == 2 && lr <= 8) {
+                if (!occ_err) {
+                    occ_err = (unsigned long long*)ctx->ensure(ctx->banked(S_OCC_ERR), sizeof(unsigned long long) * (size_t)ns);
+                    LGS_HIP_CHECK(hipMemsetAsync(occ_err, 0, sizeof(unsigned long long) * (size_t)ns, st));
+                }
+                q.occ_err = occ_err + s;
+            }
             if (need_super && lr <= 8) {
                 q.out16 = ps.planes16;
                 q.negflag = neg + s;
@@ -3892,6 +3905,9 @@
     sj.ndj = djobs.size();
     sj.dj_off = djobs.empty() ? 0 : up.append(djobs.data(), djobs.size());
     sj.hv = hv_mode(ctx, lp);
+    sj.occ_err = occ_err;
+    sj.occ_n = ns;
+    for (const PrecompJob& q : jobs) sj.occ = sj.occ || q.occ;
     return sj;
 }
 
@@ -3905,7 +3921,7 @@
             maxH = std::max(maxH, s.fine->h);
         }
     if (sj.njobs)
-        launch_precompute_jobs(ctx, up.at<PrecompJob>(sj.jobs_off), (int)sj.njobs, maxW, maxH, lp.low_res);
+        launch_precompute_jobs(ctx, up.at<PrecompJob>(sj.jobs_off), (int)sj.njobs, maxW, maxH, lp.low_res, sj.occ);
     if (sj.ndj) {
         const int np = lp.low_res * lp.low_res;
         hipLaunchKernelGGL(k_decimate_jobs, dim3((lp.Wq + 255) / 256, lp.Hq, np * (int)sj.ndj), dim3(256), 0,
@@ -4493,6 +4509,9 @@
     unsigned post_gen = 0;
     bool sq_err = false;
     bool gx_err = false;
+    unsigned long long* occ_err = nullptr;
+    int occ_n = 0;
+    std::string occ_msg;
 };
 
 bool lean_rows(const lgs_ctx* ctx, const BatchShape& B, const std::vector<MatchItem>& items)
@@ -4704,6 +4723,8 @@
     F.d_rec = d_rec;
     F.n = n;
     F.bank = ctx->bank;
+    F.occ_err = sj.occ_err;
+    F.occ_n = sj.occ_n;
 }
 
 void finish_matches(lgs_ctx* ctx, InFlight& F)
@@ -4722,6 +4743,21 @@
         ctx->wait_event(ctx->bank_ev[F.bank]);
     }
     ctx->up_busy[F.bank] = false;
+    if (F.occ_err) {
+        std::vector<unsigned long long> e((size_t)F.occ_n);
+        LGS_HIP_CHECK(hipMemcpyAsync(e.data(), F.occ_err, sizeof(unsigned long long) * e.size(), hipMemcpyDeviceToHost,
+                                     ctx->stream));
+        LGS_HIP_CHECK(hipStreamSynchronize(ctx->stream));
+        for (int s = 0; s < F.occ_n && F.occ_msg.empty(); ++s)
+            if (e[s]) {
+                int item = 0;
+                while (item < F.n && F.sets[s].fine != F.grids[item]) ++item;
+                F.occ_msg = "occupancy bitmap of the grid of match " + std::to_string(item) +
+                            " of its chunk calls precompute tile (" + std::to_string((unsigned)e[s]) + ", " +
+                            std::to_string((unsigned)(e[s] >> 32) & 0x7FFFFFFFu) +
+                            ") empty, but a cell of its footprint is not +0: a write of the cells went unrecorded";
+            }
+    }
     std::vector<MatchItem>& items = F.items;
     const BatchShape& B = F.B;
     const std::vector<int>& gens = F.gens;
@@ -4837,6 +4873,7 @@
     ctx->bank = 0;
     launch_matches(ctx, params, cost, grids, scans, init, n, nthr, sets, set_of, out, F, alt);
     finish_matches(ctx, F);
+    if (!F.occ_msg.empty()) throw Error(LGS_ERR_INTERNAL, F.occ_msg);
     if (F.sq_err) throw Error(LGS_ERR_INTERNAL, kSqDomainError);
     if (F.gx_err) throw Error(LGS_ERR_INTERNAL, kGxDomainError);
 }
@@ -4852,6 +4889,7 @@
     InFlight fl[2];
     bool busy[2] = { false, false };
     bool sq_err = false, gx_err = false;
+    std::string occ_msg;
     int c = 0;
     const int step = (ctx->split_chunks && n <= kMaxBatch && n >= 2 * kSplitMin) ? (n + 1) / 2 : kMaxBatch;
     try {
@@ -4877,6 +4915,7 @@
                 finish_matches(ctx, fl[b ^ 1]);
                 busy[b ^ 1] = false;
                 sq_err = sq_err || fl[b ^ 1].sq_err;
+                if (occ_msg.empty()) occ_msg = fl[b ^ 1].occ_msg;
                 gx_err = gx_err || fl[b ^ 1].gx_err;
             }
         }
@@ -4885,6 +4924,7 @@
             finish_matches(ctx, fl[last]);
             busy[last] = false;
             sq_err = sq_err || fl[last].sq_err;
+            if (occ_msg.empty()) occ_msg = fl[last].occ_msg;
             gx_err = gx_err || fl[last].gx_err;
         }
     } catch (...) {
@@ -4892,6 +4932,7 @@
         throw;
     }
     ctx->bank = 0;
+    if (!occ_msg.empty()) throw Error(LGS_ERR_INTERNAL, occ_msg);
     if (sq_err) throw Error(LGS_ERR_INTERNAL, kSqDomainError);
     if (gx_err) throw Error(LGS_ERR_INTERNAL, kGxDomainError);
 }
@@ -5464,6 +5505,7 @@
     const size_t bytes = sizeof(double) * (size_t)src->w * (size_t)src->h;
     try {
         if (bytes) {
+            grid_touch(g);
             if (src->writer) src->writer->wait();
             if (!ctx->peer_staged && peer_access(ctx->device, src->device)) {
                 LGS_HIP_CHECK(hipMemcpyPeerAsync(g->d, ctx->device, src->d, src->device, bytes, ctx->stream));
diff --git a/my-lidar-graph-slam_amd/csrc/lgs_core.hip b/my-lidar-graph-slam_amd/csrc/lgs_core.hip
--- a/my-lidar-graph-slam_amd/csrc/lgs_core.hip
+++ b/my-lidar-graph-slam_amd/csrc/lgs_core.hip
@@ -525,6 +525,10 @@
     case LGS_OPT_SPLIT_CHUNKS: ctx->split_chunks = value != 0.0; return LGS_OK;
     case LGS_OPT_DEVICE_HITS: ctx->device_hits = value != 0.0; return LGS_OK;
     case LGS_OPT_ZERO_TILES: ctx->zero_tiles = value != 0.0; return LGS_OK;
+    case LGS_OPT_GRID_OCCUPANCY:
+        if (!(value == 0.0 || value == 1.0 || value == 2.0)) return LGS_ERR_INVALID_ARG;
+        ctx->grid_occupancy = (int)value;
+        return LGS_OK;
     case LGS_OPT_LEAN_PROJECT: ctx->lean_project = value != 0.0; return LGS_OK;
     case LGS_OPT_FAST_ROWS: ctx->fast_rows = value != 0.0; return LGS_OK;
     case LGS_OPT_PGCG_GRID_NODES:
@@ -560,6 +564,48 @@
     for (; i < n; i += stride) d[i] = v;
 }
 
+namespace {
+__global__ __launch_bounds__(256) void k_grid_occupancy(const double* __restrict__ cells, int W, int H,
+                                                        unsigned* __restrict__ bits, int ws)
+{
+    const int x = blockIdx.x * 256 + threadIdx.x;
+    const int nby = occ::blocks(H);
+    const long long* __restrict__ c64 = (const long long*)cells;
+    for (int r = blockIdx.y; r < nby; r += gridDim.y) {
+        const int y0 = r << occ::kShift;
+        long long v[occ::kBlock];
+#pragma unroll
+        for (int k = 0; k < occ::kBlock; ++k) v[k] = (x < W && y0 + k < H) ? c64[(size_t)(y0 + k) * W + x] : 0;
+        long long any = 0;
+#pragma unroll
+        for (int k = 0; k < occ::kBlock; ++k) any |= v[k];
+        const unsigned long long m = __ballot(any != 0);
+        if ((threadIdx.x & 63) == 0 && m) {
+            unsigned b4 = 0;
+#pragma unroll
+            for (int q = 0; q < 64 / occ::kBlock; ++q)
+                if ((m >> (occ::kBlock * q)) & ((1ull << occ::kBlock) - 1)) b4 |= 1u << q;
+            const int c = x >> occ::kShift;
+            atomicOr(&bits[(size_t)r * ws + (c >> 5)], b4 << (c & 31));
+        }
+    }
+}
+
+size_t occ_bytes(const lgs_grid* g) { return sizeof(unsigned) * std::max<size_t>(1, occ::words(g->w, g->h)); }
+
+bool grid_summarise(lgs_ctx* ctx, lgs_grid* g)
+{
+    if (!g->occ || g->occ_never) return false;
+    LGS_HIP_CHECK(hipMemsetAsync(g->occ, 0, occ_bytes(g), ctx->stream));
+    if (g->w && g->h) {
+        hipLaunchKernelGGL(k_grid_occupancy, dim3((g->w + 255) / 256, std::min(occ::blocks(g->h), 65535)), dim3(256), 0,
+                           ctx->stream, g->d, g->w, g->h, g->occ, occ::row_words(g->w));
+        LGS_HIP_CHECK(hipGetLastError());
+    }
+    return true;
+}
+}
+
 extern "C" int lgs_grid_create(lgs_ctx* ctx, int w, int h, double min_x, double min_y,
                                double res, lgs_grid** out)
 {
@@ -583,8 +629,15 @@
             delete g;
             throw Error(LGS_ERR_OOM, "hipMalloc failed for grid");
         }
+        if (hipMalloc((void**)&g->occ, occ_bytes(g)) != hipSuccess) {
+            hipFree(g->d);
+            delete g;
+            throw Error(LGS_ERR_OOM, "hipMalloc failed for grid");
+        }
         LGS_HIP_CHECK(hipMemsetAsync(g->d, 0, bytes, ctx->stream));
+        LGS_HIP_CHECK(hipMemsetAsync(g->occ, 0, occ_bytes(g), ctx->stream));
         ctx->sync();
+        g->occ_valid.store(true, std::memory_order_release);
         *out = g;
     });
 }
@@ -616,6 +669,7 @@
     if (g->owned && g->d) {
         hipSetDevice(g->device);
         hipFree(g->d);
+        if (g->occ) hipFree(g->occ);
     }
     delete g;
 }
@@ -628,8 +682,11 @@
         size_t bytes = (size_t)g->w * (size_t)g->h * sizeof(double);
         if (!bytes) return;
         grid_acquire(ctx, g);
+        grid_touch(g);
         LGS_HIP_CHECK(hipMemcpyAsync(g->d, host, bytes, hipMemcpyHostToDevice, ctx->stream));
+        const bool summarised = grid_summarise(ctx, g);
         ctx->sync();
+        if (summarised) g->occ_valid.store(true, std::memory_order_release);
     });
 }
 
@@ -668,6 +725,7 @@
         if (!g->w || !g->h) return;
         LGS_HIP_CHECK(hipSetDevice(ctx->device));
         grid_acquire(ctx, g);
+        grid_touch(g);
         const int np = npx * npy;
         const size_t patch_bytes = (size_t)ps * ps * cell_bytes;
         const size_t b_slot = ((size_t)np * sizeof(int) + 15) / 16 * 16;
@@ -696,7 +754,9 @@
         hipLaunchKernelGGL(k_patch_ingest, dim3((g->w + 255) / 256, std::min(g->h, 65535)), dim3(256), 0, ctx->stream,
                            g->d, g->w, g->h, ps, npx, (const int*)d, (const unsigned char*)(d + b_slot), cell_bytes, value_offset);
         LGS_HIP_CHECK(hipGetLastError());
+        const bool summarised = grid_summarise(ctx, g);
         ctx->sync();
+        if (summarised) g->occ_valid.store(true, std::memory_order_release);
     });
 }
 
@@ -718,6 +778,7 @@
     return guarded(ctx, [&] {
         size_t n = (size_t)g->w * (size_t)g->h;
         if (!n) return;
+        grid_touch(g);
         unsigned blocks = (unsigned)std::min<size_t>((n + 255) / 256, 4096);
         hipLaunchKernelGGL(k_fill, dim3(blocks), dim3(256), 0, ctx->stream, g->d, n, v);
         LGS_HIP_CHECK(hipGetLastError());
@@ -736,7 +797,39 @@
     return LGS_OK;
 }
 
-extern "C" double* lgs_grid_device_ptr(lgs_grid* g) { return g ? g->d : nullptr; }
+extern "C" double* lgs_grid_device_ptr(lgs_grid* g)
+{
+    if (!g) return nullptr;
+    g->occ_never = true;
+    grid_touch(g);
+    return g->d;
+}
+
+extern "C" const double* lgs_grid_device_cells(const lgs_grid* g) { return g ? g->d : nullptr; }
+
+extern "C" int lgs_grid_occupancy_info(lgs_ctx* ctx, const lgs_grid* g, int* valid, int* block_w, int* block_h,
+                                       int64_t* blocks_set)
+{
+    if (!ctx || !g) return LGS_ERR_INVALID_ARG;
+    return guarded(ctx, [&] {
+        const unsigned* bits = grid_occ(g);
+        if (valid) *valid = bits ? 1 : 0;
+        if (block_w) *block_w = occ::kBlock;
+        if (block_h) *block_h = occ::kBlock;
+        if (!blocks_set) return;
+        *blocks_set = 0;
+        if (!bits) return;
+        LGS_HIP_CHECK(hipSetDevice(ctx->device));
+        std::vector<unsigned> h(occ::words(g->w, g->h));
+        if (h.empty()) return;
+        grid_acquire(ctx, g);
+        LGS_HIP_CHECK(hipMemcpyAsync(h.data(), bits, sizeof(unsigned) * h.size(), hipMemcpyDeviceToHost, ctx->stream));
+        ctx->sync();
+        int64_t n = 0;
+        for (unsigned w : h) n += __builtin_popcount(w);
+        *blocks_set = n;
+    });
+}
 
 namespace {
 
@@ -848,6 +941,11 @@
     __shared__ double m1[kPTY][FW];
     const double* __restrict__ in = j.in;
     const int tid = threadIdx.x;
+    static_assert(FW <= 32 * occ::kBlock && FH <= occ::kBlock + 1, "occ::any2: two words, two block rows");
+    const bool occ_empty = j.occ && !occ::any2(j.occ, j.occ_ws, occ::cols(sx0, min(sx1, W)), sy0, min(sy0 + FH, H));
+    const bool ld = !occ_empty || j.occ_err;
+    unsigned* zw = j.zt ? j.zt + (by * gx + bx) : nullptr;
+    if (!ld && zw && *zw == 1u) return;
     int nz = 0;
     for (int c = tid; c < fw; c += 256) {
         const int xx = sx0 + c;
@@ -855,7 +953,7 @@
 #pragma unroll
         for (int k = 0; k < FH; ++k) {
             const int yy = sy0 + k;
-            v[k] = (xx < W && yy < H) ? gload(in + ((size_t)yy * W + xx)) : 0.0;
+            v[k] = (ld && xx < W && yy < H) ? gload(in + ((size_t)yy * W + xx)) : 0.0;
         }
 #pragma unroll
         for (int k = 0; k < FH; ++k) nz |= __double_as_longlong(v[k]) != 0;
@@ -883,12 +981,15 @@
             }
         }
     }
-    unsigned* zw = j.zt ? j.zt + (by * gx + bx) : nullptr;
-    if (zw) {
-        const unsigned zprev = *zw;
+    if (zw || j.occ_err) {
+        const unsigned zprev = zw ? *zw : 0u;
         const int anynz = __syncthreads_or(nz);
-        if (!anynz && zprev == 1u) return;
-        if (tid == 0 && zprev != (anynz ? 0u : 1u)) *zw = anynz ? 0u : 1u;
+        if (j.occ_err && occ_empty && anynz && tid == 0)
+            *j.occ_err = 1ull << 63 | (unsigned long long)by << 32 | (unsigned)bx;
+        if (zw) {
+            if (!anynz && zprev == 1u) return;
+            if (tid == 0 && zprev != (anynz ? 0u : 1u)) *zw = anynz ? 0u : 1u;
+        }
     } else {
         __syncthreads();
     }
@@ -937,8 +1038,11 @@
 #ifndef LGS_PTY_SUB
 #define LGS_PTY_SUB 2
 #endif
-template <int LR, int kPTY, int kSub>
-__global__ __launch_bounds__(256) void k_precompute_planes_s(const PrecompJob* __restrict__ jobs, int gyt, DevTs dts)
+#ifndef LGS_OCC_WAVES
+#define LGS_OCC_WAVES 7
+#endif
+template <int LR, int kPTY, int kSub, bool kOcc>
+__global__ __launch_bounds__(256, (kOcc ? LGS_OCC_WAVES : 1)) void k_precompute_planes_s(const PrecompJob* __restrict__ jobs, int gyt, DevTs dts)
 {
     const DtsScope dts_scope(dts);
     const int gx = gridDim.x, gy = gridDim.y, nwg = gx * gy * gridDim.z;
@@ -970,70 +1074,91 @@
     const int by0 = bys * kSub;
     int sy0 = win_start(by0 * kPTY, H, LR);
     if (by0 >= gyt || by0 * kPTY >= H) return;
-#pragma unroll
-    for (int k = 0; k < FH; ++k) {
-        const int yy = sy0 + k;
-        v[k] = (cin && yy < H) ? gload(in + ((size_t)yy * W + xx)) : 0.0;
+    static_assert(FW <= 32 * occ::kBlock && FH <= occ::kBlock + 1, "occ::any2: two words, two block rows");
+    const unsigned* __restrict__ obits = kOcc ? j.occ : nullptr;
+    const int ows = j.occ_ws;
+    const bool verify = kOcc && j.occ_err != nullptr;
+    const occ::Cols ocols = occ::cols(sx0, min(sx0 + fw, W));
+    auto tile_empty = [&](int fy0) { return obits && !occ::any2(obits, ows, ocols, fy0, min(fy0 + FH, H)); };
+    bool empty = tile_empty(sy0);
+    {
+        const bool ld = cin && (!empty || verify);
+#pragma unroll
+        for (int k = 0; k < FH; ++k) {
+            const int yy = sy0 + k;
+            v[k] = (ld && yy < H) ? gload(in + ((size_t)yy * W + xx)) : 0.0;
+        }
     }
     for (int s = 0; s < kSub; ++s) {
         const int by = by0 + s, y0 = by * kPTY;
         if (by >= gyt || y0 >= H) break;
         const int y1 = min(y0 + kPTY, H), oh = y1 - y0;
+        unsigned* zw = j.zt ? j.zt + (by * gx + bx) : nullptr;
+        const bool occ_empty = empty;
+        const bool skip = occ_empty && !verify && zw && *zw == 1u;
         int nz = 0;
-#pragma unroll
-        for (int k = 0; k < FH; ++k) nz |= __double_as_longlong(v[k]) != 0;
-        double wm[kPTY];
-#pragma unroll
-        for (int k = 0; k < kPTY; ++k) {
-            double m = v[k];
-#pragma unroll
-            for (int i = 1; i < LR; ++i) m = dmax(m, v[k + i]);
-            wm[k] = m;
-        }
-        if (s > 0) __syncthreads();
-        const int d = y0 - sy0, st = max(0, H - LR - sy0);
-        if (col) {
-            if (d == 0 && st >= kPTY - 1) {
-#pragma unroll
-                for (int oy = 0; oy < kPTY; ++oy)
-                    if (oy < oh) m1[oy][tid] = wm[oy];
-            } else {
-#pragma unroll
-                for (int oy = 0; oy < kPTY; ++oy) {
-                    const int sr = min(oy + d, st);
-                    double m = wm[0];
-#pragma unroll
-                    for (int k = 1; k < kPTY; ++k) m = (k == sr) ? wm[k] : m;
-                    if (oy < oh) m1[oy][tid] = m;
+        if (!skip) {
+#pragma unroll
+            for (int k = 0; k < FH; ++k) nz |= __double_as_longlong(v[k]) != 0;
+            double wm[kPTY];
+#pragma unroll
+            for (int k = 0; k < kPTY; ++k) {
+                double m = v[k];
+#pragma unroll
+                for (int i = 1; i < LR; ++i) m = dmax(m, v[k + i]);
+                wm[k] = m;
+            }
+            if (s > 0) __syncthreads();
+            const int d = y0 - sy0, st = max(0, H - LR - sy0);
+            if (col) {
+                if (d == 0 && st >= kPTY - 1) {
+#pragma unroll
+                    for (int oy = 0; oy < kPTY; ++oy)
+                        if (oy < oh) m1[oy][tid] = wm[oy];
+                } else {
+#pragma unroll
+                    for (int oy = 0; oy < kPTY; ++oy) {
+                        const int sr = min(oy + d, st);
+                        double m = wm[0];
+#pragma unroll
+                        for (int k = 1; k < kPTY; ++k) m = (k == sr) ? wm[k] : m;
+                        if (oy < oh) m1[oy][tid] = m;
+                    }
                 }
             }
         }
         const int nby = by + 1;
         if (s + 1 < kSub && nby < gyt && nby * kPTY < H) {
             const int nsy0 = win_start(nby * kPTY, H, LR);
+            empty = tile_empty(nsy0);
+            const bool ld = cin && (!empty || verify);
             if (nsy0 == sy0 + kPTY) {
 #pragma unroll
                 for (int k = 0; k < LR - 1; ++k) v[k] = v[k + kPTY];
 #pragma unroll
                 for (int k = LR - 1; k < FH; ++k) {
                     const int yy = nsy0 + k;
-                    v[k] = (cin && yy < H) ? gload(in + ((size_t)yy * W + xx)) : 0.0;
+                    v[k] = (ld && yy < H) ? gload(in + ((size_t)yy * W + xx)) : 0.0;
                 }
             } else {
 #pragma unroll
                 for (int k = 0; k < FH; ++k) {
                     const int yy = nsy0 + k;
-                    v[k] = (cin && yy < H) ? gload(in + ((size_t)yy * W + xx)) : 0.0;
+                    v[k] = (ld && yy < H) ? gload(in + ((size_t)yy * W + xx)) : 0.0;
                 }
             }
             sy0 = nsy0;
         }
-        unsigned* zw = j.zt ? j.zt + (by * gx + bx) : nullptr;
-        if (zw) {
-            const unsigned zprev = *zw;
+        if (skip) continue;
+        if (zw || verify) {
+            const unsigned zprev = zw ? *zw : 0u;
             const int anynz = __syncthreads_or(nz);
-            if (tid == 0 && zprev != (anynz ? 0u : 1u)) *zw = anynz ? 0u : 1u;
-            if (!anynz && zprev == 1u) continue;
+            if (verify && occ_empty && anynz && tid == 0)
+                *j.occ_err = 1ull << 63 | (unsigned long long)by << 32 | (unsigned)bx;
+            if (zw) {
+                if (tid == 0 && zprev != (anynz ? 0u : 1u)) *zw = anynz ? 0u : 1u;
+                if (!anynz && zprev == 1u) continue;
+            }
         } else {
             __syncthreads();
         }
@@ -1161,7 +1286,7 @@
     *gx = (maxW + q - 1) / q;
     *gy = (maxH + *rows - 1) / *rows;
 }
-void launch_precompute_jobs(lgs_ctx* ctx, const PrecompJob* d_jobs, int njobs, int maxW, int maxH, int win)
+void launch_precompute_jobs(lgs_ctx* ctx, const PrecompJob* d_jobs, int njobs, int maxW, int maxH, int win, bool occ)
 {
     LGS_REQUIRE(win >= 1 && win <= kMaxWinTiled, "batched precompute: window must be in [1, 32]");
     if (njobs == 0 || maxW == 0 || maxH == 0) return;
@@ -1176,9 +1301,13 @@
                     dim3(256), 0, ctx->stream, d_jobs, ctx->dts(tok)); \
             else if (LGS_PTY_SUB > 1) { \
                 const int gyt = (maxH + LGS_PTY_BATCH - 1) / LGS_PTY_BATCH; \
-                hipLaunchKernelGGL(HIP_KERNEL_NAME(k_precompute_planes_s<L, LGS_PTY_BATCH, LGS_PTY_SUB>), \
-                    dim3((maxW + pqx<L>() * L - 1) / (pqx<L>() * L), (gyt + LGS_PTY_SUB - 1) / LGS_PTY_SUB, njobs), \
-                    dim3(256), 0, ctx->stream, d_jobs, gyt, ctx->dts(tok)); \
+                const dim3 gs((maxW + pqx<L>() * L - 1) / (pqx<L>() * L), (gyt + LGS_PTY_SUB - 1) / LGS_PTY_SUB, njobs); \
+                if (occ)  \
+                    hipLaunchKernelGGL(HIP_KERNEL_NAME(k_precompute_planes_s<L, LGS_PTY_BATCH, LGS_PTY_SUB, true>), gs, \
+                        dim3(256), 0, ctx->stream, d_jobs, gyt, ctx->dts(tok)); \
+                else \
+                    hipLaunchKernelGGL(HIP_KERNEL_NAME(k_precompute_planes_s<L, LGS_PTY_BATCH, LGS_PTY_SUB, false>), gs, \
+                        dim3(256), 0, ctx->stream, d_jobs, gyt, ctx->dts(tok)); \
             } else \
                 hipLaunchKernelGGL(HIP_KERNEL_NAME(k_precompute_planes<L, LGS_PTY_BATCH>), \
                     dim3((maxW + pqx<L>() * L - 1) / (pqx<L>() * L), (maxH + LGS_PTY_BATCH - 1) / LGS_PTY_BATCH, njobs), dim3(256), 0, ctx->stream, \
@@ -1210,6 +1339,7 @@
         out->min_x = in->min_x;
         out->min_y = in->min_y;
         out->res = in->res;
+        grid_touch(out);
         launch_precompute(ctx, in, win, out->d, nullptr);
     });
 }
diff --git a/my-lidar-graph-slam_amd/csrc/lgs_internal.hpp b/my-lidar-graph-slam_amd/csrc/lgs_internal.hpp
--- a/my-lidar-graph-slam_amd/csrc/lgs_internal.hpp
+++ b/my-lidar-graph-slam_amd/csrc/lgs_internal.hpp
@@ -18,6 +18,7 @@
 #include <vector>
 
 #include "lgs_hip.h"
+#include "occupancy.hpp"
 
 namespace lgs {
 
@@ -78,11 +79,12 @@
     S_KEEP,
     S_COLL,
     S_ZTILE,
+    S_OCC_ERR,
     S_GS0, S_GS1,
     S_HC0, S_HC1,
     S_PG0, S_PG1,
     S_PG2, S_PG3,
-    S_BATCH_WS_B, S_RECORDS_B, S_UPLOAD_B, S_DECIM_B, S_SUPER_B, S_NEGFLAG_B, S_TEDGE_B, S_ZTILE_B,
+    S_BATCH_WS_B, S_RECORDS_B, S_UPLOAD_B, S_DECIM_B, S_SUPER_B, S_NEGFLAG_B, S_TEDGE_B, S_ZTILE_B, S_OCC_ERR_B,
     S_NUM_SLOTS
 };
 
@@ -149,6 +151,9 @@
     int* negflag;
     int pgen;
     unsigned* zt;
+    const unsigned* occ;
+    int occ_ws;
+    unsigned long long* occ_err;
 };
 
 __device__ __forceinline__ unsigned short half_round_up_bits_cvt(double m)
@@ -277,6 +282,7 @@
     int seed_wide = 12;
     bool lean_project = true;
     bool fast_rows = true;
+    int grid_occupancy = 1;
     bool zero_tiles = true;
     bool device_hits = true;
     bool split_chunks = false;
@@ -326,6 +332,7 @@
         case lgs::S_NEGFLAG: return lgs::S_NEGFLAG_B;
         case lgs::S_TEDGE: return lgs::S_TEDGE_B;
         case lgs::S_ZTILE: return lgs::S_ZTILE_B;
+        case lgs::S_OCC_ERR: return lgs::S_OCC_ERR_B;
         default: return slot;
         }
     }
@@ -450,6 +457,9 @@
     bool owned = false;
     bool map_view = false;
     std::shared_ptr<lgs::WriterEvent> writer;
+    unsigned* occ = nullptr;
+    std::atomic<bool> occ_valid{ false };
+    bool occ_never = false;
 };
 
 namespace lgs {
@@ -584,6 +594,15 @@
 {
     if (g && g->writer && g->writer->st.load(std::memory_order_acquire) != ctx->stream)
         g->writer->order_after(ctx->stream);
+}
+
+inline void grid_touch(lgs_grid* g)
+{
+    if (g) g->occ_valid.store(false, std::memory_order_release);
+}
+inline const unsigned* grid_occ(const lgs_grid* g)
+{
+    return g && g->occ && g->occ_valid.load(std::memory_order_acquire) ? g->occ : nullptr;
 }
 
 struct Upload {
diff --git a/my-lidar-graph-slam_amd/csrc/occupancy.hpp b/my-lidar-graph-slam_amd/csrc/occupancy.hpp
--- /dev/null
+++ b/my-lidar-graph-slam_amd/csrc/occupancy.hpp
@@ -0,0 +1,78 @@
+#pragma once
+
+#include <cstddef>
+#include <cstdint>
+#include <cstring>
+
+#if defined(__HIPCC__)
+#define LGS_OCC_HD __host__ __device__ __forceinline__
+#else
+#define LGS_OCC_HD inline
+#endif
+
+namespace lgs {
+namespace occ {
+
+constexpr int kShift = 4;
+constexpr int kBlock = 1 << kShift;
+
+LGS_OCC_HD int blocks(int n) { return (n + kBlock - 1) >> kShift; }
+LGS_OCC_HD int row_words(int w) { return (blocks(w) + 31) >> 5; }
+LGS_OCC_HD size_t words(int w, int h) { return (size_t)row_words(w) * (size_t)blocks(h); }
+
+LGS_OCC_HD unsigned word_mask(int wi, int c0, int c1)
+{
+    const int lo = c0 - (wi << 5), hi = c1 - (wi << 5);
+    if (hi < 0 || lo > 31) return 0u;
+    const unsigned from = lo <= 0 ? 0xFFFFFFFFu : 0xFFFFFFFFu << lo;
+    const unsigned upto = hi >= 31 ? 0xFFFFFFFFu : 0xFFFFFFFFu >> (31 - hi);
+    return from & upto;
+}
+
+LGS_OCC_HD bool any(const unsigned* bits, int ws, int x0, int x1, int y0, int y1)
+{
+    const int c0 = x0 >> kShift, c1 = (x1 - 1) >> kShift;
+    const int r0 = y0 >> kShift, r1 = (y1 - 1) >> kShift;
+    unsigned acc = 0u;
+    for (int r = r0; r <= r1; ++r)
+        for (int wi = c0 >> 5; wi <= c1 >> 5; ++wi) acc |= bits[(size_t)r * ws + wi] & word_mask(wi, c0, c1);
+    return acc != 0u;
+}
+
+struct Cols {
+    int w0, w1;
+    unsigned m0, m1;
+};
+LGS_OCC_HD Cols cols(int x0, int x1)
+{
+    const int c0 = x0 >> kShift, c1 = (x1 - 1) >> kShift;
+    Cols c;
+    c.w0 = c0 >> 5;
+    c.w1 = c1 >> 5;
+    c.m0 = word_mask(c.w0, c0, c1);
+    c.m1 = c.w1 != c.w0 ? word_mask(c.w1, c0, c1) : 0u;
+    return c;
+}
+LGS_OCC_HD bool any2(const unsigned* bits, int ws, const Cols& c, int y0, int y1)
+{
+    const unsigned* r0 = bits + (size_t)(y0 >> kShift) * ws;
+    const unsigned* r1 = bits + (size_t)((y1 - 1) >> kShift) * ws;
+    return (((r0[c.w0] | r1[c.w0]) & c.m0) | ((r0[c.w1] | r1[c.w1]) & c.m1)) != 0u;
+}
+
+#if !defined(__HIP_DEVICE_COMPILE__)
+inline void build_host(const double* cells, int w, int h, unsigned* bits)
+{
+    const int ws = row_words(w);
+    std::memset(bits, 0, sizeof(unsigned) * words(w, h));
+    for (int y = 0; y < h; ++y)
+        for (int x = 0; x < w; ++x) {
+            uint64_t b;
+            std::memcpy(&b, cells + (size_t)y * w + x, sizeof(b));
+            if (b) bits[(size_t)(y >> kShift) * ws + (x >> (kShift + 5))] |= 1u << ((x >> kShift) & 31);
+        }
+}
+#endif
+
+}
+}
diff --git a/my-lidar-graph-slam_amd/lgs_amd/abi.py b/my-lidar-graph-slam_amd/lgs_amd/abi.py
--- a/my-lidar-graph-slam_amd/lgs_amd/abi.py
+++ b/my-lidar-graph-slam_amd/lgs_amd/abi.py
@@ -41,6 +41,7 @@
 LGS_OPT_DEVICE_TIMING = 34
 LGS_OPT_LEAN_PROJECT = 35
 LGS_OPT_PGCG_GRID_NODES = 36
+LGS_OPT_GRID_OCCUPANCY = 38
 LGS_OPT_FAST_ROWS = 37
 KERNEL_IDS = ["k_project", "k_coarse", "k_seed", "k_select", "k_fine", "k_replay", "k_cost", "k_precompute",
               "k_linsolve", "k_ray_emit", "k_ray_apply", "k_super", "k_super_planes", "k_bb_score",
@@ -260,6 +261,9 @@
     ("lgs_grid_info", C.c_int, [_P, C.POINTER(C.c_int), C.POINTER(C.c_int), C.POINTER(C.c_double),
                                  C.POINTER(C.c_double), C.POINTER(C.c_double)]),
     ("lgs_grid_device_ptr", _P, [_P]),
+    ("lgs_grid_device_cells", _P, [_P]),
+    ("lgs_grid_occupancy_info", C.c_int, [_P, _P, C.POINTER(C.c_int), C.POINTER(C.c_int), C.POINTER(C.c_int),
+                                          C.POINTER(C.c_int64)]),
     ("lgs_grid_precompute_max", C.c_int, [_P, _P, C.c_int, _P]),
     ("lgs_scan_create", C.c_int, [_P, C.POINTER(ScanHost), C.POINTER(_P)]),
     ("lgs_scan_destroy", None, [_P]),
@@ -1088,8 +1092,22 @@
         self.ctx.check(self.ctx.lib.lgs_grid_download(self.ctx.h, self.h, dptr(out)), "grid_download")
         return out
 
+    def fill(self, value: float, ctx: "Context" = None):
+        ctx = ctx or self.ctx
+        ctx.check(ctx.lib.lgs_grid_fill(ctx.h, self.h, float(value)), "grid_fill")
+
     def device_ptr(self) -> int:
         return self.ctx.lib.lgs_grid_device_ptr(self.h)
+
+    def device_cells(self) -> int:
+        return self.ctx.lib.lgs_grid_device_cells(self.h)
+
+    def occupancy_info(self, ctx: "Context" = None) -> dict:
+        ctx = ctx or self.ctx
+        v, bw, bh, n = C.c_int(), C.c_int(), C.c_int(), C.c_int64()
+        ctx.check(ctx.lib.lgs_grid_occupancy_info(ctx.h, self.h, C.byref(v), C.byref(bw), C.byref(bh), C.byref(n)),
+                  "grid_occupancy_info")
+        return {"valid": v.value, "block_w": bw.value, "block_h": bh.value, "blocks_set": n.value}
 
     def close(self):
         if self.h:
```

New measurement: 100,800. 1.7% lower.
